# junyongeom/gru-mpi-cuda

Measured on AMD Instinct MI355X. Metric: char-tokens/sec (whole node) for GRU hidden=512 at 1/2/4/8 MI355X, higher is better.
Workload: dtype bf16; 1 GPU; model=GRU L=1 H=512 E=512 V=256, global_batch=256, seq_len=32, parallelism=dp1, impl=hip, optimizer=adam, overlap=False, plan=fwd=persistent bwd0=persistent+dWhh+dP head=fwd-tail serial dP=bwd-tail, dp_plan=replicated, dp_pipeline=0, collectives=0

## Files before the change

gru_mpi_cuda_amd/csrc/bindings.cpp:

```cpp
#include <pybind11/pybind11.h>
#include <pybind11/numpy.h>
#include <pybind11/stl.h>

#include "engine/trainer.h"
#include "engine/generator.h"
#include "comm/rccl_comm.h"
#include "comm/bootstrap.h"
#include "data/name_loader.h"

namespace py = pybind11;
using namespace gk;

static hipStream_t S(uintptr_t s) { return reinterpret_cast<hipStream_t>(s); }
template <class T> static T* Pp(uintptr_t p) { return reinterpret_cast<T*>(p); }

template <class T>
static T get(const py::dict& d, const char* k, T dflt) {
  if (!d.contains(k)) return dflt;
  return d[k].cast<T>();
}
#define GP(T, d, k) reinterpret_cast<T*>(get<uintptr_t>(d, k, 0))

static OptimArgs optim_from(const py::dict& d, const std::string& who) {
  OptimArgs a;
// ... 478 lines not shown
    a.s16 = GP(u16, d, "s16");
    a.Bp = get<int>(d, "Bp", 0); a.H = get<int>(d, "H", 0); a.algo = get<int>(d, "algo", 0);
    if (a.Bp % 32 || a.H % 64) throw std::runtime_error("fwd_step: Bp % 32 and H % 64 required");
    return a;
  };
  auto bwd_step_args = [](py::dict d) {
    BwdStepArgs a;
    a.dgh_next = GP(const u16, d, "dgh_next"); a.WhhT = GP(const u16, d, "WhhT");
    a.carry_in = GP(const float, d, "carry_in"); a.dy = GP(const float, d, "dy");
    a.r = GP(const float, d, "r"); a.z = GP(const float, d, "z"); a.n = GP(const float, d, "n");
    a.ghn = GP(const float, d, "ghn"); a.hprev = GP(const float, d, "hprev");
    a.carry_out = GP(float, d, "carry_out"); a.dgh = GP(u16, d, "dgh"); a.dghT = GP(u16, d, "dghT");
    a.dgiT = GP(u16, d, "dgiT"); a.dgi = GP(u16, d, "dgi");
    a.ldT = get<int>(d, "ldT", 0); a.colT = get<int>(d, "colT", 0);
    a.Bp = get<int>(d, "Bp", 0); a.H = get<int>(d, "H", 0); a.algo = get<int>(d, "algo", 0);
    a.sk_part = GP(float, d, "sk_part"); a.sk_part_floats = get<long>(d, "sk_part_floats", 0);
    a.sk_cnt = GP(unsigned, d, "sk_cnt"); a.sk_cnt_words = get<long>(d, "sk_cnt_words", 0);
    a.err = GP(unsigned, d, "err");
    a.dgiT_n_only = get<int>(d, "dgiT_n_only", 0);
    if (a.Bp % 32 || a.H % 64) throw std::runtime_error("bwd_step: Bp % 32 and H % 64 required");
    return a;
  };
  m.def("fwd_step", [fwd_step_args](py::dict d, uintptr_t s) {
    gru_fwd_step(fwd_step_args(d), S(s));
    HIP_LAUNCH_CHECK();
  });
  m.def("bwd_step", [bwd_step_args](py::dict d, uintptr_t s) {
    gru_bwd_step(bwd_step_args(d), S(s));
    HIP_LAUNCH_CHECK();
  });
  auto plan_dict = [](const StepPlan& p) {
    py::dict o;
    o["name"] = step_kernel_name(p.kernel);
    o["ks"] = p.ks; o["kb"] = p.kb; o["nks_i"] = p.nks_i; o["splits"] = p.splits; o["sk_map"] = p.sk_map;
    return o;
  };
  m.def("fwd_step_variant", [fwd_step_args, plan_dict](py::dict d) { return plan_dict(gru_fwd_step_plan(fwd_step_args(d))); });
  m.def("bwd_step_variant", [bwd_step_args, plan_dict](py::dict d) { return plan_dict(gru_bwd_step_plan(bwd_step_args(d))); });
  m.def("spin_delay", [](int us, uintptr_t s) { spin_delay(us, S(s)); HIP_LAUNCH_CHECK(); });
  m.def("copy_d2d", [](uintptr_t dst, uintptr_t src, size_t bytes) {
    HIP_CHECK(hipMemcpy(reinterpret_cast<void*>(dst), reinterpret_cast<const void*>(src), bytes, hipMemcpyDeviceToDevice));
  });
  m.def("graph_node_probe_detail", &graph_node_probe_detail);
  m.def("graph_node_probe", &graph_node_probe);
  m.def("block_cus", [](int nblocks, int us, uintptr_t s) { block_cus(nblocks, us, S(s)); });
  m.def("xcc_census", [](uintptr_t out, int nblocks, int threads, uintptr_t s) {
    xcc_census(Pp<unsigned>(out), nblocks, threads, S(s)); HIP_LAUNCH_CHECK(); });
  m.def("fwd_seq_supported", &gru_fwd_seq_supported);
  m.def("bwd_step_sk_splits", &gru_bwd_step_sk_splits);
  m.def("step_lds_variants", []() {
    const StepLdsVariants& v = step_lds_variants();
    py::dict d;
    d["fwd64"] = v.fwd64; d["bwd_sk_min_h"] = v.bwd_sk_min_h; d["dwfc_group"] = v.dwfc_group;
    d["bwd_big"] = v.bwd_big; d["bwd16"] = v.bwd16; d["bwd_xring"] = v.bwd_xring; d["fwd_xring"] = v.fwd_xring; d["fwd_fc"] = v.fwd_fc; d["fc_flash"] = v.fc_flash; d["fc_tail"] = v.fc_tail; d["bwd_tail"] = v.bwd_tail; d["save16"] = v.save16; d["big_dy"] = v.big_dy; d["ld_pad"] = v.ld_pad;
    return d;
  });
  m.def("set_step_lds_variants", [](py::dict d) {
    StepLdsVariants& v = step_lds_variants();
    for (auto kv : d) {
      const std::string k = py::str(kv.first);
      const int x = kv.second.cast<int>();
      if (k == "fwd64") v.fwd64 = x;
      else if (k == "bwd_sk_min_h") v.bwd_sk_min_h = x;
      else if (k == "dwfc_group") v.dwfc_group = x;
      else if (k == "bwd_big") v.bwd_big = x;
      else if (k == "bwd16") v.bwd16 = x;
      else if (k == "bwd_xring") v.bwd_xring = x;
      else if (k == "fwd_xring") v.fwd_xring = x;
      else if (k == "fwd_fc") v.fwd_fc = x;
      else if (k == "fc_flash") v.fc_flash = x;
      else if (k == "fc_tail") v.fc_tail = x;
      else if (k == "bwd_tail") v.bwd_tail = x;
      else if (k == "big_dy") v.big_dy = x;
      else if (k == "ld_pad") v.ld_pad = x;
      else if (k == "save16") v.save16 = x;
      else throw std::runtime_error("set_step_lds_variants: unknown field " + k);
    }
  });
  m.def("gemm_variants", []() {
    const GemmVariants& v = gemm_variants();
    py::dict d;
    d["mfma"] = v.mfma; d["phased"] = v.phased; d["sched"] = v.sched; d["groupm"] = v.groupm; d["onehot"] = v.onehot;
    d["small_ring"] = v.small_ring;
    return d;
  });
  m.def("set_gemm_variants", [](py::dict d) {
    GemmVariants& v = gemm_variants();
    for (auto kv : d) {
      const std::string k = py::str(kv.first);
      const int x = kv.second.cast<int>();
      if (k == "mfma") v.mfma = x;
      else if (k == "phased") v.phased = x;
      else if (k == "sched") v.sched = x;
      else if (k == "groupm") v.groupm = x;
      else if (k == "onehot") v.onehot = x;
      else if (k == "small_ring") {
        if (x != 0 && x != 3 && x != 4) throw std::runtime_error("set_gemm_variants: small_ring is 0, 3 or 4");
        v.small_ring = x;
      }
      else throw std::runtime_error("set_gemm_variants: unknown field " + k);
    }
  });
  m.def("bwd_seq_supported", &gru_bwd_seq_supported);
  m.def("fwd_seq2", [](py::dict lo, py::dict hi, uintptr_t Wih, uintptr_t bih, uintptr_t s) {
    auto parse = [](py::dict d) {
      SeqFwdArgs a;
      a.HSb = GP(u16, d, "HSb"); a.HSf = GP(float, d, "HSf"); a.HT = GP(u16, d, "HT"); a.ldT = get<int>(d, "ldT", 0);
      a.HF = GP(u16, d, "HF"); a.xch = GP(u16, d, "xch");
      a.sr = GP(float, d, "sr"); a.sz = GP(float, d, "sz"); a.sn = GP(float, d, "sn"); a.sghn = GP(float, d, "sghn");
      a.Whh = GP(const u16, d, "Whh"); a.bhh = GP(const float, d, "bhh");
      a.P = GP(const float, d, "P"); a.ids = GP(const int, d, "ids"); a.Gi = GP(const float, d, "Gi");
      a.h0 = GP(const float, d, "h0");
      a.cnt = GP(unsigned, d, "cnt"); a.err = GP(unsigned, d, "err");
      a.dbg = GP(unsigned long long, d, "dbg"); a.allow_local = get<int>(d, "allow_local", 1);
      a.xring = get<int>(d, "xring", 0);
      a.s16 = GP(u16, d, "s16");
      a.zero_next = GP(unsigned, d, "zero_next"); a.zero_words = get<long>(d, "zero_words", 0);
      a.T = get<int>(d, "T", 0); a.Bp = get<int>(d, "Bp", 0); a.H = get<int>(d, "H", 0);
      if (!a.xch || !a.cnt || !a.HSb || !a.HSf || !a.Whh || !a.bhh) throw std::runtime_error("fwd_seq2: HSb/HSf/xch/cnt/Whh/bhh required");
      return a;
    };
    SeqFwd2Args a;
    a.lo = parse(lo); a.hi = parse(hi);
    a.Wih = reinterpret_cast<const u16*>(Wih); a.bih = reinterpret_cast<const float*>(bih);
    if (!a.lo.ids == !a.lo.Gi) throw std::runtime_error("fwd_seq2: lo needs exactly one of P+ids / Gi");
// ... 464 lines not shown
```

gru_mpi_cuda_amd/csrc/engine/trainer.cpp:

```cpp
#include "trainer.h"
#include "../runtime/trace.h"
#include "../runtime/blaslt.h"

#include <cstring>
#include <algorithm>

namespace gk {

static int round_up(int x, int m) { return (x + m - 1) / m * m; }


Trainer::Trainer(const Dims& d, const OptCfg& o, float* params, float* grads, float* m, float* v, long nflat,
                 const std::map<std::string, long>& offsets)
    : d_(d), o_(o), params_(params), grads_(grads), m_(m), v_(v), nflat_(nflat), off_(offsets) {
  if (d_.V % 64 || d_.E % 64 || d_.H % 64)
    throw std::runtime_error("HIP engine needs vocab, embed and hidden to be multiples of 64");
  Bp_ = round_up(std::max(d_.B, 1), 64);
  blaslt_init(wgrad_prefers_library(3 * d_.H, d_.H, (long)d_.T * Bp_));
  C_ = std::max(1, d_.chunks);
  while (C_ > 1 && d_.T % C_) --C_;
  Tc_ = d_.T / C_;
  const int V = d_.V, E = d_.E, H = d_.H, T = d_.T, L = d_.L, B = Bp_;
  const size_t tok = (size_t)T * B;
  const int pad = step_lds_variants().ld_pad;
// ... 36 lines not shown
  persist_fwd_ = allow && gru_fwd_seq_supported(H, B);
  {
    const char* fw = std::getenv("GK_FWD_WAVE");
    fwd_wave_ = persist_fwd_ && L >= 2 && !(fw && fw[0] == '0') && gru_fwd_seq2_supported(H, B);
  }
  if (const char* sa = std::getenv("GK_STEP_ALGO")) step_algo_ = std::atoi(sa);
  if (const char* xl = std::getenv("GK_XCD_LOCAL")) xcd_local_ = std::atoi(xl) != 0;
  if (step_algo_ == 2 && !gru_step_lds_ok(H, B)) step_algo_ = 0;
  {
    const long tok = (long)d_.T * B, ctok = (long)Tc_ * B;
    dgiT_share_ = V % 128 == 0 && H % 128 == 0 && B % 8 == 0 && tok % 128 == 0 &&
                  ctok % 128 == 0;
  }
  seq_.resize(L);
  bool any_bwd = false;
  for (int l = 0; l < L; ++l) {
    SeqPlan& q = seq_[l];
    q.fuse_p = (l == 0) && V == 256 && allow && gru_bwd_seq_supported(H, B, H <= 512, true);
    q.fuse_w = allow && H <= 512 && gru_bwd_seq_supported(H, B, true, q.fuse_p);
    q.bwd = allow && gru_bwd_seq_supported(H, B, q.fuse_w, q.fuse_p);
    if (!q.bwd) q.fuse_w = q.fuse_p = false;
    q.big = allow && !q.bwd && step_lds_variants().bwd_big && gru_bwd_seq_big_supported(H, B) &&
            seq_flag_words(H, B) >= 8192;
    q.rows16 = q.bwd && !q.fuse_w && (B / 32) % 8 != 0 && (B / 16) % 8 == 0 && step_lds_variants().bwd16 &&
               gru_bwd_seq16_supported(H, B, q.fuse_p);
    q.nrb = q.rows16 ? B / 16 : B / 32;
    any_bwd |= q.bwd;
  }
  for (int l = 0; l < L; ++l) {
    SeqPlan& q = seq_[l];
    const bool fwd16 = persist_fwd_ || gru_step_picks_lds(step_algo_, H, B);
    q.s16 = step_lds_variants().save16 && d_.overlap == 0 && (q.big || q.bwd) && fwd16;
  }
  splits_ = 8;
  size_t o_cnt = R((size_t)2 * L * seq_flag_words(H, B) * 4 + 64), o_err = R(64), o_x = R((size_t)T * B * 3 * H * 2);
  constexpr int kSlots = 2 + 2 * kMaxGroup;
  size_t o_dst = R((size_t)kSlots * slot_ints() * 4);
  const size_t wmax = std::max({(size_t)V * H, (size_t)3 * H * H, (size_t)V * 3 * H, (size_t)3 * H * E});
  size_t o_sw = R((size_t)splits_ * wmax * 4);
  size_t o_rw = R((size_t)splits_ * std::max(V, 3 * H) * 4);
  size_t o_sfc2 = R((size_t)kFcSplitsMax * V * H * 4), o_rfc2 = R((size_t)kFcSplitsMax * V * 4);
  size_t o_se = R((size_t)splits_ * V * E * 4);
  std::vector<size_t> o_pw(L, 0), o_pbh(L, 0), o_pbi(L, 0), o_hf(L, 0), o_s16(L, 0);
  for (int l = 0; l < L; ++l) {
    if (seq_[l].s16) o_s16[l] = R(tok * H * 8);
    if (seq_[l].fuse_w) o_pw[l] = R((size_t)seq_[l].nrb * 3 * H * H * 4);
    if (seq_[l].fuse_w && persist_fwd_) o_hf[l] = R((tok + B) * H * 2);
    if (seq_[l].bwd || seq_[l].big) {
      o_pbh[l] = R((size_t)seq_[l].nrb * 3 * H * 4);
      o_pbi[l] = R((size_t)seq_[l].nrb * 3 * H * 4);
    }
  }
  size_t o_pP = seq_[0].fuse_p ? R((size_t)seq_[0].nrb * V * 3 * H * 4) : 0;
  int sk = 0;
  bool any_big = false;
  for (int l = 0; l < L; ++l) {
    if (!seq_[l].bwd && !seq_[l].big) sk = gru_bwd_step_sk_splits(H, B);
    any_big |= seq_[l].big;
  }
  size_t o_bp = any_big ? R((size_t)gru_bwd_seq_big_part_floats(H, B) * 4) : 0;
  sk_part_floats_ = sk ? (long)H * B * sk : 0;
  sk_cnt_words_ = sk ? (long)(H / 128) * (B / 64) * 16 : 0;
  size_t o_skp = sk ? R((size_t)sk_part_floats_ * 4) : 0, o_skc = sk ? R((size_t)sk_cnt_words_ * 4) : 0;
  (void)any_bwd;
  arena_.commit();
  d_stage_ = arena_.get<int>(o_dst);
  cnt_ = arena_.get<unsigned>(o_cnt); err_ = arena_.get<unsigned>(o_err); xbuf_ = arena_.get<u16>(o_x);
  slab_w_ = arena_.get<float>(o_sw); rs_w_ = arena_.get<float>(o_rw);
  slab_fc2_ = arena_.get<float>(o_sfc2); rs_fc2_ = arena_.get<float>(o_rfc2); slab_e_ = arena_.get<float>(o_se);
  for (int l = 0; l < L; ++l) {
    seq_[l].dWhh_part = seq_[l].fuse_w ? arena_.get<float>(o_pw[l]) : nullptr;
    seq_[l].HF = o_hf[l] ? arena_.get<u16>(o_hf[l]) : nullptr;
    seq_[l].dbhh_part = (seq_[l].bwd || seq_[l].big) ? arena_.get<float>(o_pbh[l]) : nullptr;
    seq_[l].dbih_part = (seq_[l].bwd || seq_[l].big) ? arena_.get<float>(o_pbi[l]) : nullptr;
  }
  dP_part_ = seq_[0].fuse_p ? arena_.get<float>(o_pP) : nullptr;
  bpart_ = any_big ? arena_.get<float>(o_bp) : nullptr;
  sk_part_ = sk ? arena_.get<float>(o_skp) : nullptr;
  sk_cnt_ = sk ? arena_.get<unsigned>(o_skc) : nullptr;

  ids_ = arena_.get<int>(o_ids); labels_ = arena_.get<int>(o_lab); inv_count_ = arena_.get<float>(o_inv);
  Ptab_ = arena_.get<float>(o_P); loss_part_ = arena_.get<float>(o_lp); loss_ = arena_.get<float>(o_loss);
  slab_fc_ = arena_.get<float>(o_sfc); rs_fc_ = arena_.get<float>(o_rfc); slab_P_ = arena_.get<float>(o_sP);
  dP_ = arena_.get<float>(o_dP); norm_parts_ = arena_.get<float>(o_np); gscale_ = arena_.get<float>(o_gs);
  step_ = arena_.get<int>(o_step);
  Emb = arena_.get<u16>(o_Emb); EmbT = arena_.get<u16>(o_EmbT); Wfc = arena_.get<u16>(o_Wfc); WfcT = arena_.get<u16>(o_WfcT);
  WfcF = arena_.get<u16>(o_WfcF); WfcTF = arena_.get<u16>(o_WfcTF);
  logits_ = fc_split_ ? arena_.get<float>(o_lg) : nullptr;
  dl_ = arena_.get<u16>(o_dl); dlT_ = arena_.get<u16>(o_dlT); dP_bf_ = arena_.get<u16>(o_dPb); dPT_bf_ = arena_.get<u16>(o_dPTb);
  Ls_.resize(L);
  for (int l = 0; l < L; ++l) {
    const LO& x = los[l];
    Layer& y = Ls_[l];
    y.HSf = arena_.get<float>(x.HSf); y.sr = arena_.get<float>(x.sr); y.sz = arena_.get<float>(x.sz);
    y.sn = arena_.get<float>(x.sn); y.sghn = arena_.get<float>(x.sghn); y.dy = arena_.get<float>(x.dy);
    y.Gi = l > 0 ? arena_.get<float>(x.Gi) : nullptr;
    y.carry[0] = arena_.get<float>(x.c0); y.carry[1] = arena_.get<float>(x.c1);
    y.HSb = arena_.get<u16>(x.HSb); y.HT = arena_.get<u16>(x.HT);
    y.dgh[0] = arena_.get<u16>(x.g0); y.dgh[1] = arena_.get<u16>(x.g1);
    y.dghT = arena_.get<u16>(x.dghT); y.dgiT = arena_.get<u16>(x.dgiT);
    y.dgi = l > 0 ? arena_.get<u16>(x.dgi) : nullptr;
    y.Whh = arena_.get<u16>(x.Whh); y.WhhT = arena_.get<u16>(x.WhhT);
    y.Wih = arena_.get<u16>(x.Wih); y.WihT = arena_.get<u16>(x.WihT);
    y.slab_hh = arena_.get<float>(x.shh); y.rs_hh = arena_.get<float>(x.rhh);
    y.slab_ih = l > 0 ? arena_.get<float>(x.sih) : nullptr; y.rs_ih = l > 0 ? arena_.get<float>(x.rih) : nullptr;
    y.s16 = o_s16[l] ? arena_.get<u16>(o_s16[l]) : nullptr;
  }

  HIP_CHECK(hipStreamCreateWithFlags(&s0_, hipStreamNonBlocking));
  HIP_CHECK(hipStreamCreateWithFlags(&s1_, hipStreamNonBlocking));
  {
    int lo = 0, hi = 0;
    HIP_CHECK(hipDeviceGetStreamPriorityRange(&lo, &hi));
    HIP_CHECK(hipStreamCreateWithPriority(&sc_, hipStreamNonBlocking, hi));
  }
  events_.resize(64 + 8 * C_ * L);
  for (auto& e : events_) HIP_CHECK(hipEventCreateWithFlags(&e, hipEventDisableTiming));
  HIP_CHECK(hipStreamCreateWithFlags(&sx_, hipStreamNonBlocking));
  HIP_CHECK(hipHostMalloc(&h_stage_, kSlots * (2 * tok + 16) * sizeof(int)));
  std::memset(h_stage_, 0, kSlots * (2 * tok + 16) * sizeof(int));
  const unsigned stage_flags = hipEventDisableTiming | (unsigned)hipEventDisableSystemFence;
  for (auto& e : stage_done_) {
    HIP_CHECK(hipEventCreateWithFlags(&e, stage_flags));
    HIP_CHECK(hipEventRecord(e, s0_));
  }
  for (auto& e : group_done_) {
    HIP_CHECK(hipEventCreateWithFlags(&e, stage_flags));
    HIP_CHECK(hipEventRecord(e, s0_));
  }
  for (auto* ev : {&copy_done_[0], &copy_done_[1], &group_copy_done_[0], &group_copy_done_[1]}) {
    HIP_CHECK(hipEventCreateWithFlags(ev, hipEventDisableTiming));
    HIP_CHECK(hipEventRecord(*ev, sx_));
  }
  HIP_CHECK(hipHostMalloc(reinterpret_cast<void**>(&err_host_), 64, hipHostMallocCoherent | hipHostMallocMapped));
  std::memset(err_host_, 0, 64);
  HIP_CHECK(hipHostGetDevicePointer(reinterpret_cast<void**>(&err_host_dev_), err_host_, 0));
  const char* ng = std::getenv("GK_NO_GRAPH");
  if (ng && ng[0] == '1') use_graph_ = false;
  overlap_ = d_.overlap != 0;
  dy_in_bwd_ = fc_split_ && !overlap_ && !seq_.empty() && seq_.back().big && seq_.back().s16 && d_.V == 256 &&
               step_lds_variants().big_dy;
  fc_in_fwd_ = persist_fwd_ && !fwd_wave_ && d_.L == 1 && !overlap_ && !fc_split_ && !seq_.empty() &&
               seq_[0].bwd && seq_[0].fuse_w && seq_[0].HF && step_lds_variants().fwd_fc &&
               Bp_ / 32 <= kFcSplitsMax && gru_fwd_seq_fc_supported(d_.H, Bp_, d_.V);
  fc_tail_ = persist_fwd_ && !fwd_wave_ && d_.L == 1 && !overlap_ && !fc_split_ && !fc_in_fwd_ && seq_[0].s16 &&
             d_.V % 128 == 0 && d_.H % (16 * (d_.V / 64)) == 0 && step_lds_variants().fc_tail &&
             step_lds_variants().fc_flash == 0 && gru_fwd_seq_tail_supported(d_.H, Bp_, d_.V);
  bwd_tail_ok_ = d_.L == 1 && !overlap_ && seq_[0].bwd && seq_[0].fuse_w && seq_[0].fuse_p && !seq_[0].rows16 &&
                 seq_[0].s16 && seq_[0].HF && step_lds_variants().bwd_tail && d_.V % seq_[0].nrb == 0 &&
                 (d_.V / seq_[0].nrb) % 8 == 0 && gru_bwd_seq_tail_supported(d_.H, Bp_, d_.V);
  bwd_tail_ = bwd_tail_ok_ && use_graph_ && o_.clip <= 0.f;
}

Trainer::~Trainer() {
  wd_.reset();
  if (pbf_) (void)hipFree(pbf_);
  if (bpack_) (void)hipFree(bpack_);
  for (auto& g : g_fb_) g.reset();
  for (auto& g : g_step_) g.reset();
  for (auto& g : g_group_) g.reset();
  g_opt_.reset();
  for (auto& e : events_) (void)hipEventDestroy(e);
  for (auto& g : g_group_) g.reset();
  for (auto& e : stage_done_) if (e) (void)hipEventDestroy(e);
  for (auto& e : group_done_) if (e) (void)hipEventDestroy(e);
  for (hipEvent_t e : {copy_done_[0], copy_done_[1], group_copy_done_[0], group_copy_done_[1]})
    if (e) (void)hipEventDestroy(e);
  if (h_stage_) (void)hipHostFree(h_stage_);
  if (err_host_) (void)hipHostFree(err_host_);
  if (s0_) (void)hipStreamDestroy(s0_);
  if (s1_) (void)hipStreamDestroy(s1_);
  if (sx_) (void)hipStreamDestroy(sx_);
  if (sc_) (void)hipStreamDestroy(sc_);
}

hipEvent_t Trainer::ev() {
  if (ev_next_ >= events_.size()) throw std::runtime_error("trainer: event pool exhausted");
  return events_[ev_next_++];
}


void Trainer::set_carry(bool on) {
  if (on == carry_) return;
  carry_ = on;
  for (auto& g : g_fb_) g.reset();
  for (auto& g : g_step_) g.reset();
  for (auto& g : g_group_) g.reset();
}

void Trainer::record_carry(hipStream_t s) {
  const int H = d_.H, T = d_.T, B = Bp_;
  const size_t n = (size_t)B * H, ldT = (size_t)(T + 1) * B;
  for (int l = 0; l < d_.L; ++l) {
    Layer& y = Ls_[l];
    HIP_CHECK(hipMemcpyAsync(y.HSf, y.HSf + (size_t)T * n, n * 4, hipMemcpyDeviceToDevice, s));
    HIP_CHECK(hipMemcpyAsync(y.HSb, y.HSb + (size_t)T * n, n * 2, hipMemcpyDeviceToDevice, s));
    HIP_CHECK(hipMemcpy2DAsync(y.HT, ldT * 2, y.HT + (size_t)T * B, ldT * 2, (size_t)B * 2, H,
                               hipMemcpyDeviceToDevice, s));
    if (seq_[l].HF)
      HIP_CHECK(hipMemcpyAsync(seq_[l].HF, seq_[l].HF + (size_t)T * n, n * 2, hipMemcpyDeviceToDevice, s));
  }
}

void Trainer::reset_hidden(hipStream_t s) {
// ... 393 lines not shown
        }
      }
      if (!used) rest.job[rest.n++] = D;
    }
    if (rest.n) reduce_slabs_multi(rest, s);
    adam_cast_multi(a, j, s);
  } else {
    if (part != 0) throw std::runtime_error("record_opt: split optimiser launches need V, E, H % 64 == 0");
    if (deferred_.n) reduce_slabs_multi(deferred_, s);
    adam_step(a, s);
    refresh_weights(s);
  }
  deferred_.n = 0;
  HIP_LAUNCH_CHECK();
}

void Trainer::forward_backward(hipStream_t s) {
  GK_TRACE("gk.forward_backward");
  const int slot = stage_slot_;
  stage_src_ = dev_slot(slot);
  HIP_CHECK(hipStreamWaitEvent(s, copy_done_[slot], 0));
  if (!use_graph_) {
    hipEvent_t a = events_.back();
    HIP_CHECK(hipEventRecord(a, s));
    HIP_CHECK(hipStreamWaitEvent(s0_, a, 0));
    if (overlap_) record_fb(s0_); else record_fb_seq(s0_);
    HIP_CHECK(hipEventRecord(a, s0_));
    HIP_CHECK(hipStreamWaitEvent(s, a, 0));
  } else {
    if (!g_fb_[slot].ready()) {
      g_fb_[slot].begin(s0_);
      if (overlap_) record_fb(s0_); else record_fb_seq(s0_);
      g_fb_[slot].end(s0_);
    }
    g_fb_[slot].launch(s);
  }
  HIP_CHECK(hipEventRecord(stage_done_[slot], s));
}

void Trainer::optimizer_step(hipStream_t s) {
  GK_TRACE("gk.optimizer_step");
  if (!use_graph_) { record_opt(s); return; }
  if (!g_opt_.ready()) {
    g_opt_.begin(s0_);
    record_opt(s0_);
    g_opt_.end(s0_);
  }
  g_opt_.launch(s);
}

void Trainer::set_comm(RcclComm* c, const std::vector<std::pair<long, long>>& buckets, long min_bucket_floats) {
  comm_ = c;
  if (!c) shard_opt_ = false;
  if (c) bwd_tail_ = false;
  buckets_ = buckets;
  min_bucket_ = std::max(1L, min_bucket_floats);
  const int L = d_.L;
  long prev = off_.at("fc.weight");
  bool ok = prev == 0 && off_.at("fc.bias") > prev;
  prev = off_.at("fc.bias");
  for (int l = L - 1; l >= 0; --l) {
    const std::string k = std::to_string(l);
    for (const char* n : {"weight_hh_l", "bias_hh_l", "bias_ih_l", "weight_ih_l"}) {
      const long o = off_.at(n + k);
      ok = ok && o > prev;
      prev = o;
    }
  }
  ok = ok && off_.at("embedding") > prev;
  if (!ok) throw std::runtime_error("set_comm: flat gradient layout is not in readiness order");
  dP_inplace_ = (long)d_.V * 3 * d_.H <= 3L * d_.H * d_.E;
  g_step_[0].reset();
  g_step_[1].reset();
  g_group_[0].reset();
  g_group_[1].reset();
}

void Trainer::set_dp_pipeline(int mode) {
  if (mode < -1 || mode > 1) throw std::runtime_error("set_dp_pipeline: -1 (auto), 0 or 1");
  dp_pipe_ = mode;
  g_step_[0].reset();
  g_step_[1].reset();
  g_group_[0].reset();
  g_group_[1].reset();
}

bool Trainer::dp_pipe_on() const {
  if (!comm_ || overlap_ || shard_opt_ || d_.L != 1 || o_.clip > 0.f) return false;
  const int V = d_.V, E = d_.E, H = d_.H;
  if (V % 64 || E % 64 || H % 64 || !dP_inplace_) return false;
  return dp_pipe_ == 1;
}

long Trainer::group_end(int l) const {
  if (l >= d_.L) return off_.at("weight_hh_l" + std::to_string(d_.L - 1));
  if (l > 0) return off_.at("weight_hh_l" + std::to_string(l - 1));
  return off_.at("weight_ih_l0") + (dP_inplace_ ? (long)d_.V * 3 * d_.H : 0L);
}

bool Trainer::ar_flush(hipStream_t s, bool force, bool with_err) {
  const long n = ar_ready_ - ar_launched_;
  if (n <= 0 || (!force && n < min_bucket_)) return false;
  auto reduce = [&](hipStream_t st) {
    if (with_err) comm_->allreduce_avg_f32_err(grads_ + ar_launched_, n, err_, st);
    else comm_->allreduce_avg_f32(grads_ + ar_launched_, n, st);
  };
  hipEvent_t e = ev();
// ... 188 lines not shown
```

gru_mpi_cuda_amd/csrc/engine/trainer.h:

```cpp
#pragma once
#include <map>
#include <cstdlib>
#include <string>
#include <vector>
#include "../runtime/runtime.h"
#include "../kernels/kernels.h"
#include "../comm/rccl_comm.h"
#include "../comm/watchdog.h"
#include <memory>

namespace gk {

struct Dims {
  int V = 256, E = 512, H = 512, L = 1, B = 256, T = 32, chunks = 4;
  int overlap = 1;
};
struct OptCfg {
  float lr = 1e-3f, b1 = 0.9f, b2 = 0.999f, eps = 1e-8f, wd = 0.f, clip = 0.f;
  int sgd = 0;
  int sched = 0, warmup = 0, total = 0;
  float lr_min = 0.f;
  int keep_grads = 1;
};

class Trainer {
 public:
  Trainer(const Dims& d, const OptCfg& o, float* params, float* grads, float* m, float* v, long nflat,
          const std::map<std::string, long>& offsets);
  ~Trainer();

  void refresh_weights(hipStream_t s);
  void set_batch(const int* x_bt, const int* y_bt, int B, hipStream_t s);
  void forward_backward(hipStream_t s);
  void optimizer_step(hipStream_t s);
  float read_loss();
  float read_grad_norm();
  int get_step();
  void set_step(int v);
  void set_lr(float lr);
  void set_use_graph(bool g) { use_graph_ = g; if (!g) bwd_tail_ = false; }
  void set_carry(bool on);
  bool carry() const { return carry_; }
  void reset_hidden(hipStream_t s);
  int padded_batch() const { return Bp_; }
  long workspace_bytes() const { return (long)arena_.bytes(); }
  uintptr_t buffer(const std::string& name) const;

 private:
  void record_fb(hipStream_t s0);
  bool defer_slabs_ = false;
  SlabJobs deferred_;
  void slab_job(SlabJobs& j, const float* src, int splits, long n, float* dst);
  void record_carry(hipStream_t s);
  bool carry_ = false;
  void record_opt(hipStream_t s0, int part = 0);
  void fwd_step(int l, int t, hipStream_t s);
  void bwd_step(int l, int t, hipStream_t s);
  hipEvent_t ev();
  float* P(const std::string& name) const { return params_ + off_.at(name); }
  float* G(const std::string& name) const { return grads_ + off_.at(name); }
  int in_dim(int l) const { return l == 0 ? d_.E : d_.H; }

  Dims d_;
  OptCfg o_;
  int Bp_ = 0, Tc_ = 0, C_ = 1;
  float* params_; float* grads_; float* m_; float* v_;
  long nflat_;
  std::map<std::string, long> off_;

  Arena arena_;
  hipStream_t s0_ = nullptr, s1_ = nullptr;
  std::vector<hipEvent_t> events_;
  size_t ev_next_ = 0;
  Graph g_fb_[2], g_opt_;
  bool use_graph_ = true;
  bool overlap_ = true;
  int* h_stage_ = nullptr;
  int* d_stage_ = nullptr;
  hipStream_t sx_ = nullptr;
  hipEvent_t stage_done_[2] = {nullptr, nullptr};
  hipEvent_t copy_done_[2] = {nullptr, nullptr};
  hipEvent_t group_copy_done_[2] = {nullptr, nullptr};
  int stage_slot_ = 0;
  const int* stage_src_ = nullptr;
  size_t slot_ints() const { return 16 + 2 * (size_t)Bp_ * d_.T; }
  const int* dev_slot(int slot) const { return d_stage_ + (size_t)slot * slot_ints(); }
  void fill_slot(int slot, const int* x, const int* y, int B);
  void copy_slots(int first, int n, hipEvent_t done);
  Graph g_step_[2];
  Graph g_group_[2];
  hipEvent_t group_done_[2] = {nullptr, nullptr};
  int group_ = 1, group_parity_ = 0;
  int group_slot(int parity, int j) const { return 2 + parity * kMaxGroup + j; }
// ... 29 lines not shown
  void set_comm(RcclComm* c, const std::vector<std::pair<long, long>>& buckets, long min_bucket_floats);
  const std::vector<std::pair<long, long>>& allreduce_log() const { return ar_log_; }
  void set_dp_pipeline(int mode);
  int dp_pipeline() const { return dp_pipe_on() ? 1 : 0; }
  bool dp_tail_recorded() const { return dp_tail_rec_; }
  void set_shard_optim(int mode);
  bool shard_optim() const { return shard_opt_; }
  int shard_mode() const { return shard_mode_; }
  void gather_params(hipStream_t s);
  long shard_chunk() const { return shard_chunk_; }
  void gather_opt_state(hipStream_t s);
  void step(hipStream_t s);
  static constexpr int kMaxGroup = 32;
  void set_graph_steps(int G);
  int graph_steps() const { return group_; }
  void set_batches(const int* x, const int* y, int B, int n);
  void step_group(hipStream_t s);
  void inject_error(unsigned bits) { HIP_CHECK(hipMemcpy(err_, &bits, 4, hipMemcpyHostToDevice)); }
  void enable_watchdog(int timeout_ms);
  int watchdog_status() const { return wd_ ? wd_->status() : 0; }
  std::string watchdog_message() { return wd_ ? wd_->message() : std::string(); }
 private:
  std::unique_ptr<Watchdog> wd_;

  struct Layer {
    float *HSf, *sr, *sz, *sn, *sghn, *dy, *Gi, *carry[2];
    u16* s16 = nullptr;
    u16 *HSb, *HT, *dgh[2], *dghT, *dgiT, *dgi;
    u16 *Whh, *WhhT, *Wih, *WihT;
    float *slab_hh, *rs_hh, *slab_ih, *rs_ih;
  };
  std::vector<Layer> Ls_;
  struct SeqPlan {
    bool bwd = false, fuse_w = false, fuse_p = false;
    bool big = false;
    bool rows16 = false;
    bool s16 = false;
    int nrb = 0;
    float *dWhh_part = nullptr, *dbhh_part = nullptr, *dbih_part = nullptr;
    u16* HF = nullptr;
  };
  void record_fb_seq(hipStream_t s0, bool dp = false);
  void record_emb_tail(hipStream_t s, const float* dP_fp32);
  static bool wgrad_prefers_library(int M, int N, long K) {
    const char* v = std::getenv("GK_WGRAD_GEMM");
    return v && std::string(v) == "lib" && (double)M * N >= 8e6 && 2.0 * M * N * (double)K >= 60e9;
  }
  void wgrad_gemm(const u16* A, int lda, const u16* Bm, int ldb, int M, int N, int K, float* slab,
                  float* rowsum, hipStream_t s);
  bool persist_fwd_ = false;
  bool fc_in_fwd_ = false;
  bool fc_tail_ = false;
  bool bwd_tail_ok_ = false, bwd_tail_ = false;
  bool in_step_ = false;
  bool dy_in_bwd_ = false;
  bool fwd_wave_ = false;
  float* bpart_ = nullptr;
  int step_algo_ = 0;
  std::vector<SeqPlan> seq_;
  int splits_ = 8;
  unsigned *cnt_ = nullptr, *err_ = nullptr;
  unsigned *err_host_ = nullptr, *err_host_dev_ = nullptr;
  float* sk_part_ = nullptr;
  unsigned* sk_cnt_ = nullptr;
  long sk_part_floats_ = 0, sk_cnt_words_ = 0;
  int xcd_local_ = 1;
  bool dgiT_share_ = false;
  u16* xbuf_ = nullptr;
  float *slab_w_ = nullptr, *rs_w_ = nullptr, *dP_part_ = nullptr;
  float *slab_fc2_ = nullptr, *rs_fc2_ = nullptr, *slab_e_ = nullptr;
  GemmArgs fc_held_;
  bool fc_held_on_ = false;
  int nloss_ = 0;
  long ldG_ = 0;
  static constexpr int kFcSplitsMax = 32;
 public:
  bool uses_persistent() const { return persist_fwd_ || (!seq_.empty() && seq_[0].bwd); }
  std::string plan() const;
  unsigned read_error();
 private:
  int *ids_, *labels_;
  float *inv_count_, *Ptab_, *loss_part_, *loss_, *slab_fc_, *rs_fc_, *slab_P_, *dP_;
  float *norm_parts_, *gscale_;
  int* step_;
  u16 *Emb, *EmbT, *Wfc, *WfcT, *dl_, *dlT_, *dP_bf_, *dPT_bf_;
  bool fc_split_ = false;
  float* logits_ = nullptr;
  u16 *WfcF, *WfcTF;
};

}
```

gru_mpi_cuda_amd/csrc/engine/trainer_seq.cpp:

```cpp
#include "trainer.h"
#include <algorithm>
#include <string>

namespace gk {

static bool ar_span() { return true; }

static int wgrad_engine() {
  const char* v = std::getenv("GK_WGRAD_GEMM");
  if (!v || !*v) return 0;
  if (std::string(v) == "lib") return 1;
  if (std::string(v) == "128") return 128;
  return 256;
}

static int gemm256_splits(int M, int N, int K) {
  int best = 0;
  double best_fill = 0.0;
  for (int sp = 1; sp <= 8; sp *= 2) {
    if (K % sp || (K / sp) % 64 || (sp > 1 && K / sp < 2048)) continue;
    const int bm = gemm256_tile_rows(M, N, K, sp);
    if (!bm) continue;
    const int wg = (M / bm) * (N / 256) * sp, rounds = (wg + 255) / 256;
    const double fill = (double)wg / (rounds * 256);
// ... 65 lines not shown

void Trainer::slab_job(SlabJobs& j, const float* src, int splits, long n, float* dst) {
  SlabJobs& t = (defer_slabs_ && splits <= kDeferMaxSplits) ? deferred_ : j;
  if (t.n >= 24) throw std::runtime_error("slab job list full");
  t.add(src, splits, n, dst);
}

void Trainer::record_fb_seq(hipStream_t s, bool dp) {
  const int V = d_.V, E = d_.E, H = d_.H, T = d_.T, L = d_.L, B = Bp_;
  const int H3 = 3 * H;
  const long tok = (long)T * B;
  const long fw = seq_flag_words(H, B);
  ev_next_ = 0;
  fc_held_on_ = false;
  if (dp) { ar_ready_ = ar_launched_ = 0; ar_busy_ = false; ar_log_.clear(); }
  dp_tail_rec_ = false;
  nloss_ = (int)(tok / 32);
  {
    GemmArgs g;
    g.A = Emb; g.lda = E; g.B = Ls_[0].Wih; g.ldb = E; g.C = Ptab_; g.ldc = H3;
    g.bias = P("bias_ih_l0"); g.M = V; g.N = H3; g.K = E;
    gemm_with_prep(g, PrepJob{stage_src_, Bp_, T, Bp_, ids_, labels_, inv_count_}, s);
  }
  if (carry_) record_carry(s);
  auto fwd_args = [&](int l) {
    Layer& y = Ls_[l];
    SeqFwdArgs a;
    a.HSb = y.HSb; a.HSf = y.HSf; a.HT = y.HT; a.ldT = (T + 1) * B; a.HF = seq_[l].HF;
    a.xch = xbuf_;
    if (y.s16) a.s16 = y.s16;
    else { a.sr = y.sr; a.sz = y.sz; a.sn = y.sn; a.sghn = y.sghn; }
    a.Whh = y.Whh; a.bhh = P("bias_hh_l" + std::to_string(l));
    if (l == 0) { a.P = Ptab_; a.ids = ids_; }
    else a.Gi = y.Gi;
    a.cnt = cnt_ + (size_t)l * fw; a.err = err_; a.allow_local = xcd_local_;
    a.xring = step_lds_variants().fwd_xring;
    if (seq_[l].bwd) { a.zero_next = cnt_ + (size_t)(L + l) * fw; a.zero_words = fw; }
    a.T = T; a.Bp = B; a.H = H;
    if (carry_) a.h0 = y.HSf;
    if (!seq_[l].bwd) fill_f32(reinterpret_cast<float*>(a.cnt), fw, 0.f, s);
    return a;
  };
  auto fc_args = [&]() {
    FcXentArgs f;
    f.X = Ls_[L - 1].HSb + (size_t)B * H; f.W = Wfc; f.b = P("fc.bias");
    f.labels = labels_; f.inv_count = inv_count_;
    f.dl = dl_; f.dlT = dlT_; f.ldT = (int)ldG_; f.colT = 0;
    f.loss_part = loss_part_; f.M = (int)tok; f.H = H; f.V = V;
    return f;
  };
  auto fc_fuse_dh = [&](FcXentArgs& f) {
    f.dl = nullptr; f.WT = WfcT; f.dy = Ls_[L - 1].dy; f.Wf = WfcF; f.WTf = WfcTF;
  };
  for (int l = 0; l < L; ++l) {
    Layer& y = Ls_[l];
    if (l > 0) {
      GemmArgs g;
      g.A = Ls_[l - 1].HSb + (size_t)B * H; g.lda = H; g.B = y.Wih; g.ldb = H;
      g.C = y.Gi; g.ldc = H3; g.bias = P("bias_ih_l" + std::to_string(l));
      g.M = (int)tok; g.N = H3; g.K = H;
      gemm_nt(g, s);
    }
    if (persist_fwd_ && fwd_wave_ && l + 1 < L) {
      SeqFwd2Args w2;
      w2.lo = fwd_args(l);
      w2.hi = fwd_args(l + 1);
      w2.hi.Gi = nullptr;
      w2.hi.xch = xbuf_ + (size_t)T * B * H;
      w2.lo.xring = w2.hi.xring = 0;
      w2.Wih = Ls_[l + 1].Wih; w2.bih = P("bias_ih_l" + std::to_string(l + 1));
      gru_fwd_seq2(w2, s);
      ++l;
    } else if (persist_fwd_ && fc_in_fwd_) {
      SeqFwdArgs a = fwd_args(l);
      a.HT = nullptr;
      SeqFcArgs f;
      f.Wf = WfcF; f.WTf = WfcTF; f.b = P("fc.bias"); f.labels = labels_; f.inv_count = inv_count_;
      f.dy = y.dy; f.dlF = dlT_; f.loss_part = loss_part_; f.dW = slab_fc2_; f.db = rs_fc2_; f.V = V;
      gru_fwd_seq_fc(a, f, s);
    } else if (persist_fwd_ && fc_tail_) {
      FcXentArgs f = fc_args();
      fc_fuse_dh(f);
      gru_fwd_seq_tail(fwd_args(l), f, s);
    } else if (persist_fwd_) {
      gru_fwd_seq(fwd_args(l), s);
    } else {
      for (int t = 0; t < T; ++t) fwd_step(l, t, s);
    }
  }
  Layer& top = Ls_[L - 1];
  SlabJobs tail;
  if (fc_in_fwd_) {
    tail.add(slab_fc2_, B / 32, (long)V * H, G("fc.weight"));
    tail.add(rs_fc2_, B / 32, V, G("fc.bias"));
  } else {
    FcXentArgs f = fc_args();
    if (fc_tail_) {
    } else if (fc_split_) {
      GemmArgs lg;
      lg.A = f.X; lg.lda = H; lg.B = Wfc; lg.ldb = H; lg.C = logits_; lg.ldc = V; lg.bias = f.b;
      lg.M = (int)tok; lg.N = V; lg.K = H;
      gemm_nt(lg, s);
      softmax_xent(logits_, f, s);
      if (!dy_in_bwd_) {
        GemmArgs g;
        g.A = dl_; g.lda = V; g.B = WfcT; g.ldb = V; g.C = top.dy; g.ldc = H;
        g.M = (int)tok; g.N = H; g.K = V;
        gemm_nt(g, s);
      }
    } else if (V % 128 == 0 && H % (16 * (V / 64)) == 0) {
      fc_fuse_dh(f);
      fc_xent(f, s);
    } else {
      fc_xent(f, s);
      GemmArgs g;
      g.A = dl_; g.lda = V; g.B = WfcT; g.ldb = V; g.C = top.dy; g.ldc = H;
      g.M = (int)tok; g.N = H; g.K = V;
      gemm_nt(g, s);
    }
    const int tiles = std::max(1, (V / 128) * (H / 128));
    int sp = 1;
    while (sp * 2 <= kFcSplitsMax && tiles * sp < 256 && tok % (sp * 2) == 0 && (tok / (sp * 2)) % 128 == 0)
      sp *= 2;
    if (sp * 2 <= kFcSplitsMax && tiles * sp < 512 && tok % (sp * 2) == 0 && tok / (sp * 2) >= 4096) sp *= 2;
    GemmArgs w;
    w.A = dlT_; w.lda = (int)ldG_; w.B = top.HT + B; w.ldb = (T + 1) * B;
    w.C = slab_fc2_; w.ldc = H; w.rowsumA = rs_fc2_;
    w.M = V; w.N = H; w.K = (int)tok; w.splits = sp;
    constexpr int kslice = 1024;
    if (kslice > 0 && tok % kslice == 0 && tok / kslice <= kFcSplitsMax && (V / 64) * (H / 64) * (tok / kslice) <= 256) {
      GemmArgs ws = w;
      ws.splits = (int)(tok / kslice); ws.algo = 3;
      if (gemm_small_kblocks(ws)) { w = ws; sp = ws.splits; }
    }
    fc_held_on_ = (dp && dp_pipe_on()) ||
                  (!dp && defer_slabs_ && sp <= 8 && w.algo == 3 && step_lds_variants().dwfc_group);
    if (fc_held_on_) fc_held_ = w;
    else gemm_nt(w, s);
    tail.add(slab_fc2_, sp, (long)V * H, G("fc.weight"));
    tail.add(rs_fc2_, sp, V, G("fc.bias"));
  }
  bool bwd_tail = bwd_tail_ok_ && !dp && defer_slabs_ && seq_[0].nrb <= kDeferMaxSplits;
  for (int k2 = 0; k2 < tail.n; ++k2) bwd_tail = bwd_tail && tail.job[k2].splits <= kDeferMaxSplits;
  if (in_step_) bwd_tail_ = bwd_tail;
  for (int l = L - 1; l >= 0; --l) {
    Layer& y = Ls_[l];
    const SeqPlan& q = seq_[l];
    const std::string k = std::to_string(l);
    if (q.bwd) {
      SeqBwdArgs a;
      a.dy = y.dy;
      if (q.s16) a.s16 = y.s16;
      else { a.sr = y.sr; a.sz = y.sz; a.sn = y.sn; a.sghn = y.sghn; }
      a.HSf = y.HSf; a.HT = y.HT; a.ldT = (T + 1) * B; a.HF = q.HF; a.WhhT = y.WhhT; a.xbuf = xbuf_;
      const bool need_T = !q.fuse_w || (l == 0 ? !q.fuse_p : true);
      a.dghT = need_T ? y.dghT : nullptr; a.dgiT = need_T ? y.dgiT : nullptr; a.ldG = (int)ldG_;
      a.dgi = y.dgi;
      a.dWhh_part = q.dWhh_part; a.dbhh_part = q.dbhh_part; a.dbih_part = q.dbih_part;
      if (q.fuse_p) { a.ids = ids_; a.dP_part = dP_part_; a.V = V; }
      a.cnt = cnt_ + (size_t)(L + l) * fw; a.err = err_; a.allow_local = xcd_local_;
      if (persist_fwd_) { a.zero_next = cnt_ + (size_t)l * fw; a.zero_words = fw; }
      a.T = T; a.Bp = B; a.H = H;
      if (!persist_fwd_) fill_f32(reinterpret_cast<float*>(a.cnt), fw, 0.f, s);
      a.xring = step_lds_variants().bwd_xring;
      if (bwd_tail && l == 0) {
        BwdTailArgs t;
        t.dP_bf = dP_bf_; t.dPT_bf = dPT_bf_; t.loss_part = loss_part_; t.nloss = nloss_; t.loss = loss_; t.step = step_;
        gru_bwd_seq_tail(a, t, s);
      } else if (q.rows16) gru_bwd_seq16(a, s);
      else gru_bwd_seq(a, s);
    } else if (q.big) {
      SeqBwdArgs a;
      a.dy = y.dy; a.HSf = y.HSf;
      if (q.s16) a.s16 = y.s16;
      else { a.sr = y.sr; a.sz = y.sz; a.sn = y.sn; a.sghn = y.sghn; }
      a.WhhT = y.WhhT; a.xbuf = xbuf_; a.part = bpart_;
      a.dghT = y.dghT; a.dgiT = y.dgiT; a.ldG = (int)ldG_; a.dgi = y.dgi;
      a.dgiT_n_only = l == 0 && dgiT_share_;
      a.dbhh_part = q.dbhh_part; a.dbih_part = l == 0 ? q.dbih_part : nullptr;
      if (dy_in_bwd_ && l == L - 1) { a.dl = dl_; a.WfcT = WfcT; a.V = V; a.dy = nullptr; }
      a.cnt = cnt_ + (size_t)(L + l) * fw; a.err = err_;
      a.T = T; a.Bp = B; a.H = H;
      a.xring = step_lds_variants().bwd_xring;
      fill_f32(reinterpret_cast<float*>(a.cnt), 8192, 0.f, s);
      gru_bwd_seq_big(a, s);
    } else {
      for (int t = T - 1; t >= 0; --t) bwd_step(l, t, s);
    }
    if (dp && q.bwd) ar_flush(s, false);
    SlabJobs j;
    if (q.fuse_w) slab_job(j, q.dWhh_part, q.nrb, (long)H3 * H, G("weight_hh_l" + k));
    if (q.bwd || q.big) slab_job(j, q.dbhh_part, q.nrb, H3, G("bias_hh_l" + k));
    if (l == 0 && q.fuse_p) {
      if (dp) j.add(dP_part_, q.nrb, (long)V * H3, dP_target());
      else if (!bwd_tail) j.add_cast(dP_part_, q.nrb, V, H3, nullptr, dP_bf_, dPT_bf_);
    }
    if (l == 0 && (q.bwd || q.big)) slab_job(j, q.dbih_part, q.nrb, H3, G("bias_ih_l0"));
    const bool pipe = dp && l == 0 && dp_pipe_on();
    if ((dp ? l == L - 1 : l == 0) && !pipe)
      for (int k2 = 0; k2 < tail.n; ++k2)
        slab_job(j, tail.job[k2].src, tail.job[k2].splits, tail.job[k2].n, tail.job[k2].dst);
    if (l == 0 && bwd_tail) {
      if (j.n) throw std::runtime_error("record_fb_seq: a slab job is left for the reduce launch the backward's tail replaced");
    } else if (l == 0) {
      j.add(loss_part_, nloss_, 1, loss_);
      j.bump = step_;
    }
    if (pipe) {
      if (!q.fuse_p || !q.fuse_w) throw std::runtime_error("pipelined data-parallel tail: needs the fused dW_hh / dP backward");
      record_dp_tail_l1(s, j, tail);
      HIP_LAUNCH_CHECK();
      return;
    }
    if (j.n) reduce_slabs_multi(j, s);
    if (!q.fuse_w)
      wgrad_gemm(y.dghT, (int)ldG_, y.HT, (T + 1) * B, H3, H, (int)tok, G("weight_hh_l" + k),
                 (q.bwd || q.big) ? nullptr : G("bias_hh_l" + k), s);
    if (l == 0) {
      if (!q.fuse_p) {
        GemmArgs p;
        int sp = splits_;
// ... 124 lines not shown
  e.A = dP_bf_; e.lda = H3; e.B = Ls_[0].WihT; e.ldb = H3; e.C = slab_e_; e.ldc = E;
  e.M = V; e.N = E; e.K = H3; e.splits = se;
  if (H3 % V == 0 && H3 / V <= splits_) {
    GemmArgs es = e;
    es.splits = H3 / V;
    const GemmArgs three[3] = {fc_held_, g, es};
    const bool with_fc = fc_held_on_ && gemm_small_group_depth(three, 3) == gemm_small_kblocks(g);
    const int nkb = gemm_small_kblocks(g);
    if (nkb && nkb == gemm_small_kblocks(es)) {
      const GemmArgs pair[2] = {g, es};
      if (fc_held_on_ && !with_fc) gemm_nt(fc_held_, s);
      if (with_fc) gemm_small_group(three, 3, s);
      else gemm_small_group(pair, 2, s);
      fc_held_on_ = false;
      SlabJobs r;
      slab_job(r, slab_e_, es.splits, (long)V * E, G("embedding"));
      if (r.n) reduce_slabs_multi(r, s);
      HIP_LAUNCH_CHECK();
      return;
    }
  }
  if (fc_held_on_) gemm_nt(fc_held_, s);
  fc_held_on_ = false;
  const GemmArgs both[2] = {g, e};
  const long wg = (long)(g.M / 128) * (g.N / 128) * g.splits + (long)(e.M / 128) * (e.N / 128) * e.splits;
  if (gemm_lds_ok(g) && gemm_lds_ok(e) && wg <= 512) {
    gemm_lds_group(both, 2, s);
  } else {
    gemm_nt(g, s);
    gemm_nt(e, s);
  }
  SlabJobs r;
  slab_job(r, slab_e_, se, (long)V * E, G("embedding"));
  if (r.n) reduce_slabs_multi(r, s);
  HIP_LAUNCH_CHECK();
}

std::string Trainer::plan() const {
  std::string p = std::string("fwd=") +
                  (persist_fwd_ ? (fwd_wave_ ? "persistent+wave" : fc_in_fwd_ ? "persistent+fc" : "persistent") : "per-step");
  for (size_t l = 0; l < seq_.size(); ++l) {
    p += " bwd" + std::to_string(l) + "=" +
         (seq_[l].bwd ? (seq_[l].rows16 ? "persistent16" : "persistent") : seq_[l].big ? "persistent-big" : "per-step");
    if (seq_[l].fuse_w) p += "+dWhh";
    if (seq_[l].fuse_p) p += "+dP";
    if (dy_in_bwd_ && l + 1 == seq_.size()) p += "+dy";
  }
  bool any_step = !persist_fwd_;
  for (const SeqPlan& q : seq_) any_step |= !q.bwd;
  if (any_step) p += std::string(" step=") + (gru_step_picks_lds(step_algo_, d_.H, Bp_) ? "lds" : "reg");
  if (fc_tail_) p += " head=fwd-tail";
  p += overlap_ ? " overlap(chunks=" + std::to_string(C_) + ")" : " serial";
  if (bwd_tail_) p += " dP=bwd-tail";
  return p;
}

unsigned Trainer::read_error() {
  unsigned e = 0;
  HIP_CHECK(hipDeviceSynchronize());
  HIP_CHECK(hipMemcpy(&e, err_, 4, hipMemcpyDeviceToHost));
  return e;
}

}
```

gru_mpi_cuda_amd/csrc/kernels/fc_block.h:

```cpp
#pragma once
#include "kernels.h"
#include "mma_tile.h"
#include "seq_sync.h"

namespace gk {

static constexpr int FROWS = 32;
static constexpr int kX2Pad = 8;

constexpr size_t fc_xent_v256_lds(int H) {
  return (size_t)FROWS * (H + kX2Pad) * 2 + (2 * 8 * 32 + 64) * 4 + 256 * 40 * 2 + (size_t)FROWS * (256 + 8) * 2 + FROWS * 4;
}

template <int NKC>
DEV void fc2_load_w(bf16x8 (&b)[NKC][2], const u16* Wf, int H, int v0, int ks, int lane) {
#pragma unroll
  for (int kk = 0; kk < NKC; ++kk)
#pragma unroll
    for (int c = 0; c < 2; ++c) b[kk][c] = ld8(Wf + ((size_t)((v0 / 16 + c) * (H / 32) + ks + kk) * 64 + lane) * 8);
}
template <int NKC>
DEV void fc2_mma(f32x4 (&acc)[2][2], const bf16x8 (&b)[NKC][2], const u16* xs, int ldx, int ks, int lane) {
  const int lr = lane & 15, lk = 8 * (lane >> 4);
#pragma unroll
  for (int kk = 0; kk < NKC; ++kk) {
    bf16x8 af[2];
#pragma unroll
    for (int r = 0; r < 2; ++r) af[r] = *reinterpret_cast<const bf16x8*>(xs + (r * 16 + lr) * ldx + (ks + kk) * 32 + lk);
#pragma unroll
    for (int r = 0; r < 2; ++r)
#pragma unroll
      for (int c = 0; c < 2; ++c) acc[r][c] = mfma16(af[r], b[kk][c], acc[r][c]);
  }
}
DEV void fc2_load_wt(bf16x8 (&bt)[8][4], const u16* WTf, int n0, int lane) {
#pragma unroll
  for (int kk = 0; kk < 8; ++kk)
#pragma unroll
    for (int c = 0; c < 4; ++c) bt[kk][c] = ld8(WTf + ((size_t)((n0 / 16 + c) * 8 + kk) * 64 + lane) * 8);
}

struct FcXPlain {
  static constexpr bool kWeightsFirst = false;
  DEV bool sc1() const { return false; }
  DEV void ready() const {}
  DEV int tid() const { return (int)threadIdx.x; }
};

template <int HH, bool DH, class XP>
DEV void fc_xent_v256_block(const FcXentArgs& a, float* smem, int block, const XP& xp) {
  int nst = 0;
  const int tid = xp.tid(), lane = tid & 63, w = tid >> 6;
  auto STAMP = [&]() {
    if (a.dbg && block == 0 && tid == 0) a.dbg[nst] = __builtin_amdgcn_s_memrealtime();
    ++nst;
  };
  STAMP();
  constexpr int V = 256, NW = 8, NKC = 8, LDR = V + 8;
  const int lr = lane & 15, lq = lane >> 4;
  constexpr int H = HH;
  const int ldx = H + kX2Pad, m0 = block * FROWS;
  u16* xs = reinterpret_cast<u16*>(smem);
  float* red = reinterpret_cast<float*>(xs + FROWS * ldx);
  float* lab = red + 2 * NW * 32;
  float* lrow = lab + 32;
  u16* st = reinterpret_cast<u16*>(lrow + 32);
  u16* dlr = st + V * 40;

  const int v0 = w * 32, nks = H / 32;
  const float inv = a.inv_count[0];
  float bias[2];
#pragma unroll
  for (int c = 0; c < 2; ++c) bias[c] = a.b[v0 + c * 16 + lr];
  bf16x8 b0[NKC][2], b1[NKC][2];
  constexpr int nxp = FROWS * H / 8 / 512;
  uint4 xv[nxp];
  auto load_x = [&]() {
    if (xp.sc1()) {
      const rsrc_t rX = make_rsrc(a.X, (unsigned)((size_t)a.M * H * 2));
#pragma unroll
      for (int e = 0; e < nxp; ++e) {
        const int q = tid + e * 512, row = q / (H / 8), c8 = q % (H / 8);
        const u32x4 v = __builtin_amdgcn_raw_buffer_load_b128(rX, (unsigned)(((size_t)(m0 + row) * H + c8 * 8) * 2), 0, 16);
        xv[e] = make_uint4(v.x, v.y, v.z, v.w);
      }
    } else {
#pragma unroll
      for (int e = 0; e < nxp; ++e) {
        const int q = tid + e * 512, row = q / (H / 8), c8 = q % (H / 8);
        xv[e] = *reinterpret_cast<const uint4*>(a.X + (size_t)(m0 + row) * H + c8 * 8);
      }
    }
  };
  int ylab;
  if constexpr (XP::kWeightsFirst) {
    ylab = tid < FROWS ? a.labels[m0 + tid] : 0;
    fc2_load_w<NKC>(b0, a.Wf, H, v0, 0, lane);
    if (nks > NKC) fc2_load_w<NKC>(b1, a.Wf, H, v0, NKC, lane);
    xp.ready();
// ... 81 lines not shown
        dlr[row * LDR + col] = db;
      }
    }
  lds_barrier();
  STAMP();
  if (tid < FROWS) {
    const int row = tid, y = ys[row];
    float m = red[row], sum = 0.f;
    for (int ww = 1; ww < NW; ++ww) m = fmaxf(m, red[ww * 32 + row]);
    for (int ww = 0; ww < NW; ++ww) sum += red[NW * 32 + ww * 32 + row];
    lrow[row] = (y >= 0) ? (logf(sum) + m - lab[row]) * inv : 0.f;
  }
  for (int q = tid; q < V * 4; q += 512) {
    const int col = q >> 2, seg = q & 3;
    uint4 v = *reinterpret_cast<const uint4*>(st + col * 40 + seg * 8);
    if ((col >> 3) & 1) v = make_uint4(v.y, v.x, v.w, v.z);
    *reinterpret_cast<uint4*>(a.dlT + (size_t)col * a.ldT + a.colT + m0 + seg * 8) = v;
  }
  STAMP();
  if constexpr (!DH) {
    for (int q = tid; q < FROWS * V / 8; q += 512) {
      const int r2 = q / (V / 8), c8 = q % (V / 8);
      *reinterpret_cast<uint4*>(a.dl + (size_t)(m0 + r2) * V + c8 * 8) =
          *reinterpret_cast<const uint4*>(dlr + r2 * LDR + c8 * 8);
    }
  }
  if constexpr (DH) for (int n0 = w * per; n0 < (w + 1) * per; n0 += 64) {
    if (n0 != w * per) fc2_load_wt(bt, a.WTf, n0, lane);
    f32x4 dacc[2][4];
    zero_acc(dacc);
#pragma unroll
    for (int kk = 0; kk < 8; ++kk) {
      bf16x8 af[2];
#pragma unroll
      for (int r = 0; r < 2; ++r) af[r] = *reinterpret_cast<const bf16x8*>(dlr + (r * 16 + lr) * LDR + kk * 32 + 8 * lq);
#pragma unroll
      for (int r = 0; r < 2; ++r)
#pragma unroll
        for (int c = 0; c < 4; ++c) dacc[r][c] = mfma16(af[r], bt[kk][c], dacc[r][c]);
    }
#pragma unroll
    for (int r = 0; r < 2; ++r)
#pragma unroll
      for (int c = 0; c < 4; ++c)
#pragma unroll
        for (int i = 0; i < 4; ++i)
          a.dy[(size_t)(m0 + r * 16 + lq * 4 + i) * H + n0 + c * 16 + lr] = dacc[r][c][i];
  }
  STAMP();
  __syncthreads();
  if (tid == 0) {
    float t = 0.f;
    for (int i = 0; i < FROWS; ++i) t += lrow[i];
    a.loss_part[block] = t;
  }
  STAMP();
}

}
```

gru_mpi_cuda_amd/csrc/kernels/gru_seq.hip:

```cpp
#include "kernels.h"
#include "mma_tile.h"
#include "seq_sync.h"
#include "fc_block.h"
#include "optim_dev.h"
#include <type_traits>

namespace gk {

static constexpr size_t kFwdRecLds = sizeof(float) * 8 * 6 * 256 + sizeof(u16) * 32 * 24 + sizeof(u16) * 16 * 40;
static constexpr size_t kFwdFcLds = sizeof(u16) * 32 * (512 + 8) + sizeof(u16) * 32 * (256 + 8) +
                                    sizeof(float) * (2 * 8 * 32 + 3 * 32);

template <int H>
DEV void fwd_fc_consumer(const SeqFwdArgs& a, const SeqFcArgs& f, unsigned char* smem, int ci) {
  constexpr int V = 256, NW = 8, LDX = H + 8, LDR = V + 8, NKS = H / 32, NKC = 4;
  static_assert((V / 64) * (H / 64) == kFcCons, "one 64 x 64 dW_fc tile per consumer");
  const int tid = threadIdx.x, lane = tid & 63, lr = lane & 15, lq = lane >> 4;
  const int w = __builtin_amdgcn_readfirstlane(tid >> 6);
  const int T = a.T, Bp = a.Bp, nrb = Bp / 32;
  constexpr int nunit = H / 16;
  const int rbk = ci % nrb, c = ci / nrb, b0 = rbk * 32;
  unsigned* const fl = a.cnt + (size_t)rbk * (nunit + kFcCons) * kFlagStride;
  unsigned* const cfl = fl + (size_t)nunit * kFlagStride;
  const int probe = f.probe & 7;
// ... 233 lines not shown
      for (;;) {
        bool ok = true;
        if (lane < n)
          ok = __hip_atomic_load(cfl + (size_t)((t0 + lane) % kFcCons) * kFlagStride, __ATOMIC_RELAXED,
                                 __HIP_MEMORY_SCOPE_AGENT) >= (unsigned)((t0 + lane) / kFcCons + 1);
        if (__all(ok)) break;
        __builtin_amdgcn_s_sleep(8);
        if (spin.expired()) {
          if (lane == 0) __hip_atomic_fetch_or(a.err, 1u, __ATOMIC_RELAXED, __HIP_MEMORY_SCOPE_AGENT);
          break;
        }
      }
      __builtin_amdgcn_fence(__ATOMIC_ACQUIRE, "wavefront");
    }
    bf16x8 A[DG], Bf[DG][2];
#pragma unroll
    for (int i = 0; i < DG; ++i) {
      if (i < n) {
        const int t = t0 + i;
        A[i] = ld8_sc1(rD, (unsigned)((((size_t)(t * nrb + rbk) * (V / 16) + tv) * 512 + lane * 8) * 2));
#pragma unroll
        for (int j = 0; j < 2; ++j)
          Bf[i][j] = ld8_sc1(rF, (unsigned)(((((size_t)(t + 1) * nunit + th + j) * nrb + rbk) * 512 + lane * 8) * 2));
      }
    }
#pragma unroll
    for (int i = 0; i < DG; ++i) {
      if (i < n) {
#pragma unroll
        for (int j = 0; j < 2; ++j) aw[j] = mfma16(A[i], Bf[i][j], aw[j]);
        if (rs_on) ab = mfma16(A[i], ones, ab);
      }
    }
  }
  float* W = f.dW + (size_t)rbk * V * H;
#pragma unroll
  for (int j = 0; j < 2; ++j)
#pragma unroll
    for (int i = 0; i < 4; ++i) W[(size_t)(tv * 16 + lq * 4 + i) * H + (th + j) * 16 + lr] = aw[j][i];
  if (rs_on && lr == 0) {
#pragma unroll
    for (int i = 0; i < 4; ++i) f.db[(size_t)rbk * V + tv * 16 + lq * 4 + i] = ab[i];
  }
}


struct FcXTail {
  static constexpr bool kWeightsFirst = true;
  const unsigned* fl;
  int nunit;
  unsigned epoch;
  unsigned* err;
  DEV bool sc1() const { return true; }
  DEV void ready() const { wait_flags_keep(fl, nunit, epoch, err); }
  DEV int tid() const {
    int t = (int)threadIdx.x;
    asm volatile("" : "+v"(t));
    return t;
  }
};

static_assert(std::is_trivially_copyable<SeqFwdArgs>::value && std::is_trivially_copyable<FcXentArgs>::value,
              "the tail reads both argument structs back from the kernel-argument segment byte for byte");
DEV void fwd_fc_tail(bool loc, unsigned char* smem) {
  typedef const __attribute__((address_space(4))) char* kptr_t;
  kptr_t kp = (kptr_t)__builtin_amdgcn_kernarg_segment_ptr();
  asm volatile("" : "+s"(kp));
  const SeqFwdArgs& a = *(const SeqFwdArgs*)kp;
  constexpr size_t fc_off = (sizeof(SeqFwdArgs) + alignof(FcXentArgs) - 1) / alignof(FcXentArgs) * alignof(FcXentArgs);
  const int T = a.T, nrb = a.Bp / 32, nunit = a.H / 16;
  const int ut = seq_unit_tile(nrb), rbk = seq_row_block(nrb);
  unsigned* const fl = a.cnt + (size_t)rbk * nunit * kFlagStride;
  const FcXTail xp{fl, nunit, (unsigned)(T + 1), a.err};
  const int tid = xp.tid();
  stamp(a.dbg, T + 1, 5);
  if (tid < 64) {
    asm volatile("s_waitcnt vmcnt(0)" ::: "memory");
    if (tid == 0) {
      if (loc) signal_flag_local(fl + (size_t)ut * kFlagStride, (unsigned)(T + 1));
      else signal_flag(fl + (size_t)ut * kFlagStride, (unsigned)(T + 1));
    }
  }
  for (int t = ut; t < T; t += nunit) {
    kptr_t kf = kp + fc_off;
    asm volatile("" : "+s"(kf));
    const FcXentArgs f = *(const FcXentArgs*)kf;
    fc_xent_v256_block<512, true>(f, reinterpret_cast<float*>(smem), t * nrb + rbk, xp);
  }
  stamp(a.dbg, T + 1, 6);
}

template <bool TAIL> struct FwdFcArg { typedef SeqFcArgs type; };
template <> struct FwdFcArg<true> { typedef FcXentArgs type; };
static constexpr size_t kFwdTailLds = fc_xent_v256_lds(512) > kFwdRecLds ? fc_xent_v256_lds(512) : kFwdRecLds;

template <int NKW, int RS, bool FC, int WPE = FC ? 4 : 1, bool TAIL = false>
__global__ void __launch_bounds__(512, WPE) gru_fwd_seq_kernel(SeqFwdArgs a, typename FwdFcArg<TAIL>::type fc) {
  static_assert(!(FC && TAIL), "the FC consumers and the FC tail exclude each other");
  static_assert(!TAIL || (NKW == 4 && RS == 2), "the tail is built for H = 512");
  static_assert(std::is_same<decltype(&gru_fwd_seq_kernel<NKW, RS, FC, WPE, TAIL>),
                             void (*)(SeqFwdArgs, typename FwdFcArg<TAIL>::type)>::value,
                "gru_fwd_seq_kernel takes (SeqFwdArgs, FC arguments) and nothing else");
  __shared__ __attribute__((aligned(16))) unsigned char smem[TAIL ? kFwdTailLds : FC ? (kFwdFcLds > kFwdRecLds ? kFwdFcLds : kFwdRecLds) : kFwdRecLds];
  auto& part = *reinterpret_cast<float(*)[8][6][256]>(smem);
  auto& stg = *reinterpret_cast<u16(*)[32][24]>(smem + sizeof(float) * 8 * 6 * 256);
  auto& stgT = *reinterpret_cast<u16(*)[16][40]>(smem + sizeof(float) * 8 * 6 * 256 + sizeof(u16) * 32 * 24);
  const int tid = threadIdx.x, lane = tid & 63, w = tid >> 6;
  const int H = a.H, Bp = a.Bp, T = a.T;
  const int nrb = Bp / 32;
  const unsigned nunit = (unsigned)(H / 16);
  if constexpr (FC) {
    const int nrec = (int)nunit * nrb;
    if ((int)blockIdx.x >= nrec) {
      zero_next_flags(a.zero_next, a.zero_words);
      if constexpr (NKW * 128 == 512 && RS == 2) fwd_fc_consumer<512>(a, fc, smem, (int)blockIdx.x - nrec);
      return;
    }
  }
  const size_t rb_lines = nunit + (FC ? kFcCons : 0);
  const int ut = FC ? seq_unit_tile_n(nrb, (int)nunit * nrb) : seq_unit_tile(nrb);
  const int j0 = ut * 16, rbk = FC ? seq_row_block_n(nrb, (int)nunit * nrb) : seq_row_block(nrb), b0 = rbk * 32;
  const int lr = lane & 15, lk = 8 * (lane >> 4);
  constexpr int NR = RS == 2 ? 1 : 2;
  const int rt = RS == 2 ? (w >> 2) : 0;
  const int k0 = (RS == 2 ? (w & 3) : w) * NKW * 32;

  bf16x8 bw[NKW][3];
#pragma unroll
  for (int kk = 0; kk < NKW; ++kk)
#pragma unroll
    for (int g = 0; g < 3; ++g) bw[kk][g] = ld8(a.Whh + (size_t)(g * H + j0 + lr) * H + k0 + kk * 32 + lk);

  const int rb = tid >> 8, reg = (tid >> 6) & 3, ln = tid & 63;
  const int row = rb * 16 + (ln >> 4) * 4 + reg, col = ln & 15;
  const int b = b0 + row, j = j0 + col;
  float bh[3];
#pragma unroll
  for (int g = 0; g < 3; ++g) bh[g] = a.bhh[g * H + j];
  float hp = a.h0 ? a.h0[(size_t)b * H + j] : 0.f;
  const rsrc_t rH = make_rsrc(a.HSb, (unsigned)((size_t)(T + 1) * Bp * H * 2));
  const rsrc_t rX = make_rsrc(a.xch, (unsigned)((size_t)T * Bp * H * 2));
  const int xr = a.xring >= 2 ? a.xring : T;
  const unsigned sv_bytes = (unsigned)((size_t)T * Bp * H * 4);
  const rsrc_t rHSf = make_rsrc(a.HSf, sv_bytes + (unsigned)(Bp * H * 4));
  const rsrc_t rSr = make_rsrc(a.sr, a.sr ? sv_bytes : 0u), rSz = make_rsrc(a.sz, a.sz ? sv_bytes : 0u);
  const rsrc_t rSn = make_rsrc(a.sn, a.sn ? sv_bytes : 0u), rSg = make_rsrc(a.sghn, a.sghn ? sv_bytes : 0u);
  const rsrc_t rS16 = make_rsrc(a.s16, a.s16 ? 2u * sv_bytes : 0u);
  const unsigned sv_lane = (unsigned)((b * H + j) * 4);
  stamp(a.dbg, T + 1, 0);
  zero_next_flags(a.zero_next, a.zero_words);
  int cens = (int)rb_lines;
  if constexpr (FC) {
    if ((fc.probe & 7) == 3) cens = (int)nunit;
    if (fc.probe & 8) __builtin_amdgcn_s_setprio(2);
  }
  const bool loc = a.allow_local && row_block_local(a.cnt + (size_t)rbk * rb_lines * kFlagStride, ut, cens, a.err);
  stamp(a.dbg, T + 1, 4);

  int idn = a.ids ? a.ids[b] : 0;
  auto load_gi = [&](int t, float (&gi)[3]) {
    if (t >= T) return;
    const float* src = a.ids ? a.P + (size_t)idn * 3 * H : a.Gi + ((size_t)t * Bp + b) * 3 * H;
#pragma unroll
    for (int g = 0; g < 3; ++g) gi[g] = src[g * H + j];
    if (a.ids && t + 1 < T) idn = a.ids[(size_t)(t + 1) * Bp + b];
  };
  float gin[3] = {0.f, 0.f, 0.f};
  load_gi(0, gin);
  for (int t = 0; t < T; ++t) {
    stamp(a.dbg, t, 0);
    const float gi[3] = {gin[0], gin[1], gin[2]};
    f32x4 acc[NR][3];
    zero_acc(acc);
    if (t > 0 || a.h0) {
      bf16x8 af[NKW][NR];
      if (t > 0) {
        const size_t slot = ((size_t)((t - 1) % xr) * nrb + rbk) * nunit;
        wave_wait_load<NKW>(a.cnt + (size_t)rbk * rb_lines * kFlagStride, lane < 2 * NKW, k0 / 16 + lane,
                            (unsigned)t, a.err, [&](int kk) {
          const int u = k0 + kk * 32 + lk;
          const unsigned tb = (unsigned)(((slot + u / 16) * 32 + lr) * 16 + (u & 15)) * 2;
#pragma unroll
          for (int r = 0; r < NR; ++r) af[kk][r] = ld8_sc1(rX, tb + (unsigned)((rt + r) * 16 * 16 * 2));
        });
      } else {
        const unsigned base = (unsigned)((((size_t)b0 + rt * 16 + lr) * H + k0 + lk) * 2);
#pragma unroll
        for (int kk = 0; kk < NKW; ++kk)
#pragma unroll
          for (int r = 0; r < NR; ++r) af[kk][r] = ld8_sc1(rH, base + (unsigned)(r * 16 * H * 2 + kk * 64));
      }
      stamp(a.dbg, t, 1);
#pragma unroll
      for (int kk = 0; kk < NKW; ++kk)
#pragma unroll
        for (int r = 0; r < NR; ++r)
#pragma unroll
          for (int g = 0; g < 3; ++g) acc[r][g] = mfma16(af[kk][r], bw[kk][g], acc[r][g]);
    }
#pragma unroll
    for (int r = 0; r < NR; ++r)
#pragma unroll
      for (int g = 0; g < 3; ++g)
#pragma unroll
        for (int i = 0; i < 4; ++i) part[w][r * 3 + g][i * 64 + lane] = acc[r][g][i];
    if constexpr (FC) {
      if (w == 2) asm volatile("s_waitcnt vmcnt(0)" ::: "memory");
    }
    __syncthreads();
    stamp(a.dbg, t, 2);
    float gh[3];
#pragma unroll
    for (int g = 0; g < 3; ++g) {
      float s = 0.f;
      if constexpr (RS == 2) {
#pragma unroll
        for (int ww = 0; ww < 4; ++ww) s += part[rb * 4 + ww][g][reg * 64 + ln];
      } else {
#pragma unroll
        for (int ww = 0; ww < 8; ++ww) s += part[ww][rb * 3 + g][reg * 64 + ln];
      }
      gh[g] = s + bh[g];
    }
    const float r = sigmoidf_(gi[0] + gh[0]);
    const float z = sigmoidf_(gi[1] + gh[1]);
    const float n = tanhf_(gi[2] + r * gh[2]);
    const float h = n + z * (hp - n);
    hp = h;
    const u16 hb = f2bf(h);
    stg[row][col] = hb;
    stgT[col][row] = hb;
    __syncthreads();
    stamp(a.dbg, t, 3);
    if (w == 0) {
      const u32x4 v = *reinterpret_cast<const u32x4*>(&stg[lane >> 1][(lane & 1) * 8]);
      const unsigned xo = (unsigned)((((size_t)(t % xr) * nrb + rbk) * nunit + ut) * 512 + lane * 8) * 2;
      unsigned* fl = a.cnt + ((size_t)rbk * rb_lines + ut) * kFlagStride;
      if (loc) {
        st16_plain(rX, xo, v);
        asm volatile("s_waitcnt vmcnt(0)" ::: "memory");
        if (lane == 0) signal_flag_local(fl, (unsigned)(t + 1));
      } else {
        st16_sc1(rX, xo, v);
        asm volatile("s_waitcnt vmcnt(0)" ::: "memory");
        if (lane == 0) signal_flag(fl, (unsigned)(t + 1));
      }
      stamp(a.dbg, t, 4);
      const size_t hs = ((size_t)(t + 1) * Bp + b0 + (lane >> 1)) * H + j0 + (lane & 1) * 8;
      if (FC && !loc) st16_sc1(rH, (unsigned)(hs * 2), v);
      else if (TAIL && !loc) {
        unsigned* hp = reinterpret_cast<unsigned*>(a.HSb + hs);
#pragma unroll
        for (int i = 0; i < 4; ++i) __hip_atomic_store(hp + i, v[i], __ATOMIC_RELAXED, __HIP_MEMORY_SCOPE_AGENT);
      } else *reinterpret_cast<u32x4*>(a.HSb + hs) = v;
      stamp(a.dbg, t, 5);
    } else if (w == 1 && a.HT) {
      const u32x4 v = *reinterpret_cast<const u32x4*>(&stgT[lane >> 2][(lane & 3) * 8]);
      *reinterpret_cast<u32x4*>(a.HT + (size_t)(j0 + (lane >> 2)) * a.ldT + (size_t)(t + 1) * Bp + b0 + (lane & 3) * 8) = v;
    } else if (w == 2 && a.HF) {
      const u32x4 v = *reinterpret_cast<const u32x4*>(&stgT[lane & 15][8 * (lane >> 4)]);
      const size_t hf = (((size_t)(t + 1) * nunit + ut) * nrb + rbk) * 512 + lane * 8;
      if (FC && !loc) st16_sc1(make_rsrc(a.HF, (unsigned)((size_t)(T + 1) * Bp * H * 2)), (unsigned)(hf * 2), v);
      else *reinterpret_cast<u32x4*>(a.HF + hf) = v;
    }
    load_gi(t + 1, gin);
    const int sstep = __builtin_amdgcn_readfirstlane(t * Bp * H * 4);
    __builtin_amdgcn_raw_buffer_store_b32(__float_as_uint(h), rHSf, sv_lane, sstep + Bp * H * 4, 0);
    if (TAIL || a.s16) {
      typedef unsigned u32x2_ __attribute__((ext_vector_type(2)));
      const u32x2_ pv = {(unsigned)f2bf(r) | ((unsigned)f2bf(z) << 16), (unsigned)f2bf(n) | ((unsigned)f2bf(gh[2]) << 16)};
      __builtin_amdgcn_raw_buffer_store_b64(pv, rS16, sv_lane * 2u, sstep * 2, 0);
    } else if (a.sr) {
      __builtin_amdgcn_raw_buffer_store_b32(__float_as_uint(r), rSr, sv_lane, sstep, 0);
      __builtin_amdgcn_raw_buffer_store_b32(__float_as_uint(z), rSz, sv_lane, sstep, 0);
      __builtin_amdgcn_raw_buffer_store_b32(__float_as_uint(n), rSn, sv_lane, sstep, 0);
      __builtin_amdgcn_raw_buffer_store_b32(__float_as_uint(gh[2]), rSg, sv_lane, sstep, 0);
    }
    stamp(a.dbg, t, 6);
  }
  if constexpr (FC) {
    asm volatile("s_waitcnt vmcnt(0)" ::: "memory");
    __syncthreads();
    if (tid == 0) {
      unsigned* fl = a.cnt + ((size_t)rbk * rb_lines + ut) * kFlagStride;
      if (loc) signal_flag_local(fl, (unsigned)(T + 1));
      else signal_flag(fl, (unsigned)(T + 1));
    }
  }
  if constexpr (TAIL) fwd_fc_tail(loc, smem);
}

template <int NKW>
__global__ void __launch_bounds__(512, 1) gru_fwd_seq2_kernel(SeqFwd2Args a) {
  constexpr int NKS = NKW < 4 ? 4 : NKW;
  __shared__ __attribute__((aligned(16))) bf16x8 stage[8][2][NKS][2][64];
  __shared__ __attribute__((aligned(16))) u16 stg[2][32][24];
  __shared__ __attribute__((aligned(16))) u16 stgT[2][16][40];
  typedef __attribute__((address_space(3))) void lds_void;
  const SeqFwdArgs& L0 = a.lo;
  const SeqFwdArgs& L1 = a.hi;
  const int tid = threadIdx.x, lane = tid & 63, w = __builtin_amdgcn_readfirstlane(tid >> 6);
  const int H = L0.H, Bp = L0.Bp, T = L0.T;
  const int nrb = Bp / 32, ut = seq_unit_tile(nrb);
  const int j0 = ut * 16, rbk = seq_row_block(nrb), b0 = rbk * 32;
  const int lr = lane & 15, lk = 8 * (lane >> 4);
  const int k0 = w * NKW * 32;
  const unsigned nunit = (unsigned)(H / 16);

  bf16x8 wh0[NKW][3], wi1[NKW][3], wh1[NKW][3];
#pragma unroll
  for (int kk = 0; kk < NKW; ++kk)
#pragma unroll
    for (int g = 0; g < 3; ++g) {
      const size_t o = (size_t)(g * H + j0 + lr) * H + k0 + kk * 32 + lk;
      wh0[kk][g] = ld8(L0.Whh + o);
      wi1[kk][g] = ld8(a.Wih + o);
      wh1[kk][g] = ld8(L1.Whh + o);
    }

  const int q = w >> 2, e = w & 3;
  const int row = q * 16 + 4 * (lane >> 4) + e, col = lane & 15;
  const int b = b0 + row, j = j0 + col, pidx = e * 64 + lane;
  float bh0[3], bh1[3], bi1[3];
#pragma unroll
  for (int g = 0; g < 3; ++g) {
    bh0[g] = L0.bhh[g * H + j];
    bh1[g] = L1.bhh[g * H + j];
    bi1[g] = a.bih[g * H + j];
  }
  float hp0 = L0.h0 ? L0.h0[(size_t)b * H + j] : 0.f;
  float hp1 = L1.h0 ? L1.h0[(size_t)b * H + j] : 0.f;
  const unsigned hs_bytes = (unsigned)((size_t)(T + 1) * Bp * H * 2), x_bytes = (unsigned)((size_t)T * Bp * H * 2);
  const rsrc_t rH0 = make_rsrc(L0.HSb, hs_bytes), rX0 = make_rsrc(L0.xch, x_bytes);
  const rsrc_t rH1 = make_rsrc(L1.HSb, hs_bytes), rX1 = make_rsrc(L1.xch, x_bytes);
  const int xr = L0.xring >= 2 ? L0.xring : T;
  zero_next_flags(L0.zero_next, L0.zero_words);
  zero_next_flags(L1.zero_next, L1.zero_words);
  unsigned* const fl0 = L0.cnt + (size_t)rbk * nunit * kFlagStride;
  unsigned* const fl1 = L1.cnt + (size_t)rbk * nunit * kFlagStride;
  const bool loc = L0.allow_local && row_block_local(fl0, ut, (int)nunit, L0.err);

  const unsigned xl = (unsigned)((((lk >> 4) * 32 + lr) * 16 + (lk & 15)) * 2);
// ... 139 lines not shown
      const int ly = w, t = s - ly;
      if (ly == 0 ? do0 : do1) {
        const SeqFwdArgs& Y = ly == 0 ? L0 : L1;
        const u32x4 v = *reinterpret_cast<const u32x4*>(&stg[ly][lane >> 1][(lane & 1) * 8]);
        const unsigned xo = (unsigned)((((size_t)(t % xr) * nrb + rbk) * nunit + ut) * 512 + lane * 8) * 2;
        unsigned* fl = (ly == 0 ? fl0 : fl1) + (size_t)ut * kFlagStride;
        const rsrc_t rX = ly == 0 ? rX0 : rX1;
        if (loc) {
          st16_plain(rX, xo, v);
          asm volatile("s_waitcnt vmcnt(0)" ::: "memory");
          if (lane == 0) signal_flag_local(fl, (unsigned)(t + 1));
        } else {
          st16_sc1(rX, xo, v);
          asm volatile("s_waitcnt vmcnt(0)" ::: "memory");
          if (lane == 0) signal_flag(fl, (unsigned)(t + 1));
        }
        if (ly == 0) stamp(L0.dbg, s, 4);
        *reinterpret_cast<u32x4*>(Y.HSb + ((size_t)(t + 1) * Bp + b0 + (lane >> 1)) * H + j0 + (lane & 1) * 8) = v;
      }
    } else if (w < 6) {
      const int ly = (w - 2) >> 1, t = s - ly;
      const SeqFwdArgs& Y = ly == 0 ? L0 : L1;
      if (ly == 0 ? do0 : do1) {
        if (((w - 2) & 1) == 0) {
          if (Y.HT) {
            const u32x4 v = *reinterpret_cast<const u32x4*>(&stgT[ly][lane >> 2][(lane & 3) * 8]);
            *reinterpret_cast<u32x4*>(Y.HT + (size_t)(j0 + (lane >> 2)) * Y.ldT + (size_t)(t + 1) * Bp + b0 + (lane & 3) * 8) = v;
          }
        } else if (Y.HF) {
          const u32x4 v = *reinterpret_cast<const u32x4*>(&stgT[ly][lane & 15][8 * (lane >> 4)]);
          *reinterpret_cast<u32x4*>(Y.HF + (((size_t)(t + 1) * nunit + ut) * nrb + rbk) * 512 + lane * 8) = v;
        }
      }
    }
    load_gi0(s + 1, gin);
    if (do0) {
      L0.HSf[((size_t)(s + 1) * Bp + b) * H + j] = h0v;
      const size_t so = ((size_t)s * Bp + b) * H + j;
      if (L0.s16) st_save16(L0.s16 + so * 4, r0, z0, n0, ghn0);
      else if (L0.sr) { L0.sr[so] = r0; L0.sz[so] = z0; L0.sn[so] = n0; L0.sghn[so] = ghn0; }
    }
    if (do1) {
      L1.HSf[((size_t)s * Bp + b) * H + j] = h1v;
      const size_t so = ((size_t)(s - 1) * Bp + b) * H + j;
      if (L1.s16) st_save16(L1.s16 + so * 4, r1, z1, n1, ghn1);
      else if (L1.sr) { L1.sr[so] = r1; L1.sz[so] = z1; L1.sn[so] = n1; L1.sghn[so] = ghn1; }
    }
  }
}

struct SeqBwdTailK : SeqBwdArgs { BwdTailArgs t; };
template <bool TAIL> struct BwdKArg { typedef SeqBwdArgs type; };
template <> struct BwdKArg<true> { typedef SeqBwdTailK type; };

static_assert(std::is_trivially_copyable<SeqBwdTailK>::value, "the tail reads its arguments back from the kernel-argument segment");
template <int NTW, int NTP>
DEV void bwd_dp_tail(const f32x4 (&accW)[3][NTW], const f32x4 (&accP)[3][NTP], const float (&dbh)[3], float dbi,
                     float (*red)[16][33], unsigned char* stage ) {
  typedef const __attribute__((address_space(4))) char* kptr_t;
  kptr_t kp = (kptr_t)__builtin_amdgcn_kernarg_segment_ptr();
  asm volatile("" : "+s"(kp));
  const SeqBwdTailK& k = *(const SeqBwdTailK*)kp;
  const SeqBwdArgs& a = k;
  int tid = (int)threadIdx.x;
  asm volatile("" : "+v"(tid));
  const int lane = tid & 63, w = tid >> 6, lr = lane & 15, lq = lane >> 4;
  const int H = a.H, H3 = 3 * H, V = a.V, T = a.T, nrb = a.Bp / 32;
  const int nunit = H / 16, ut = seq_unit_tile(nrb), rbk = seq_row_block(nrb), j0 = ut * 16;
  const unsigned slab_bytes = (unsigned)((size_t)V * H3 * 4);
  const rsrc_t rP = make_rsrc(a.dP_part, (unsigned)nrb * slab_bytes);
  stamp(a.dbg, T + 1, 0);
#pragma unroll
  for (int g = 0; g < 3; ++g)
#pragma unroll
    for (int nt = 0; nt < NTP; ++nt) {
      const unsigned o = (unsigned)rbk * slab_bytes +
                         (unsigned)((((w * NTP + nt) * 16 + lr) * H3 + g * H + j0 + lq * 4) * 4);
      st16_sc1(rP, o, __builtin_bit_cast(u32x4, accP[g][nt]));
    }
  {
    const int rb = tid >> 8, reg = (tid >> 6) & 3, ln = tid & 63;
    const int row = rb * 16 + (ln >> 4) * 4 + reg, col = ln & 15;
    red[0][col][row] = dbh[0]; red[1][col][row] = dbh[1]; red[2][col][row] = dbh[2];
    red[3][col][row] = dbh[0]; red[4][col][row] = dbh[1]; red[5][col][row] = dbi;
  }
  asm volatile("s_waitcnt vmcnt(0)" ::: "memory");
  lds_barrier();
  if (tid == 0) signal_flag(a.cnt + ((size_t)rbk * nunit + ut) * kFlagStride, (unsigned)(T + 1));
  stamp(a.dbg, T + 1, 1);
  if (tid < 96) {
    const int kk = tid >> 4, c = tid & 15;
    float sum = 0.f;
    for (int rr = 0; rr < 32; ++rr) sum += red[kk][c][rr];
    float* dst = (kk < 3 ? a.dbhh_part : a.dbih_part);
    if (dst) dst[(size_t)rbk * H3 + (kk % 3) * H + j0 + c] = sum;
  }
  {
    float* W = a.dWhh_part + (size_t)rbk * H3 * H;
#pragma unroll
    for (int g = 0; g < 3; ++g)
#pragma unroll
      for (int nt = 0; nt < NTW; ++nt)
#pragma unroll
        for (int i = 0; i < 4; ++i)
          W[(size_t)(g * H + j0 + lq * 4 + i) * H + (w * NTW + nt) * 16 + lr] = accW[g][nt][i];
  }
  if (tid < 64) {
    SpinBudget spin(a.err);
    for (;;) {
      bool ok = true;
      if (lane < nrb)
        ok = __hip_atomic_load(a.cnt + ((size_t)lane * nunit + ut) * kFlagStride, __ATOMIC_RELAXED,
                               __HIP_MEMORY_SCOPE_AGENT) >= (unsigned)(T + 1);
      if (__all(ok)) break;
      __builtin_amdgcn_s_sleep(GK_POLL_SLEEP);
      if (spin.expired()) {
        if (lane == 0) __hip_atomic_fetch_or(a.err, 1u, __ATOMIC_RELAXED, __HIP_MEMORY_SCOPE_AGENT);
        break;
      }
    }
  }
  lds_barrier();
  stamp(a.dbg, T + 1, 2);
  constexpr int LDS_P = 56;
  u16* const tile = reinterpret_cast<u16*>(stage);
  const int rows = V / nrb, v0 = rbk * rows;
  const int irow = tid / 6, ipc = tid % 6;
  const int icol = (ipc >> 1) * H + j0 + (ipc & 1) * 8;
  const int tcol = tid >> 2, tseg = tid & 3;
  for (int r0 = 0; r0 < rows; r0 += 32) {
    if (tid < 192 && r0 + irow < rows) {
      const size_t e = (size_t)(v0 + r0 + irow) * H3 + icol;
      f32x4 x[8][2];
#pragma unroll
      for (int s = 0; s < 8; ++s)
        if (s < nrb) {
          const unsigned o = (unsigned)s * slab_bytes + (unsigned)(e * 4);
          x[s][0] = __builtin_bit_cast(f32x4, __builtin_amdgcn_raw_buffer_load_b128(rP, o, 0, 16));
          x[s][1] = __builtin_bit_cast(f32x4, __builtin_amdgcn_raw_buffer_load_b128(rP, o + 16u, 0, 16));
        }
      f32x4 s0 = x[0][0], s1 = x[0][1];
#pragma unroll
      for (int s = 1; s < 8; ++s)
        if (s < nrb) {
#pragma unroll
          for (int i = 0; i < 4; ++i) { s0[i] += x[s][0][i]; s1[i] += x[s][1][i]; }
        }
      u32x4 pv;
      pv[0] = (unsigned)f2bf(s0[0]) | ((unsigned)f2bf(s0[1]) << 16);
      pv[1] = (unsigned)f2bf(s0[2]) | ((unsigned)f2bf(s0[3]) << 16);
      pv[2] = (unsigned)f2bf(s1[0]) | ((unsigned)f2bf(s1[1]) << 16);
      pv[3] = (unsigned)f2bf(s1[2]) | ((unsigned)f2bf(s1[3]) << 16);
      *reinterpret_cast<u32x4*>(k.t.dP_bf + e) = pv;
      *reinterpret_cast<u32x4*>(tile + irow * LDS_P + ipc * 8) = pv;
    }
    lds_barrier();
    if (tid < 192 && r0 + tseg * 8 < rows) {
      u16 v[8];
#pragma unroll
      for (int q = 0; q < 8; ++q) v[q] = tile[(tseg * 8 + q) * LDS_P + tcol];
      const int gcol = (tcol >> 4) * H + j0 + (tcol & 15);
      *reinterpret_cast<u32x4*>(k.t.dPT_bf + (size_t)gcol * V + v0 + r0 + tseg * 8) = *reinterpret_cast<const u32x4*>(v);
    }
    if (r0 + 32 < rows) lds_barrier();
  }
  if (blockIdx.x == 0 && tid < 64) {
    const float l = wave_strided_sum(k.t.loss_part, k.t.nloss, 1, 0, lane);
    if (tid == 0) {
      k.t.loss[0] = l;
      *k.t.step += 1;
    }
  }
  stamp(a.dbg, T + 1, 3);
}

template <int NKW3, int NTW, int NTP, bool TAIL = false>
__global__ void __launch_bounds__(512, 1) gru_bwd_seq_kernel(typename BwdKArg<TAIL>::type a) {
  static_assert(!TAIL || (NKW3 == 6 && NTW == 4 && NTP == 2), "the tail is built for H = 512, V = 256");
  static_assert(std::is_same<decltype(&gru_bwd_seq_kernel<NKW3, NTW, NTP, TAIL>), void (*)(typename BwdKArg<TAIL>::type)>::value,
                "gru_bwd_seq_kernel takes one argument struct and nothing else");
  __shared__ __attribute__((aligned(16))) float part[8][2][256];
  __shared__ __attribute__((aligned(16))) u16 srow[3][32][24];
  __shared__ __attribute__((aligned(16))) u16 sgT[4][16][40];
  __shared__ __attribute__((aligned(16))) float red[6][16][33];
  constexpr bool kScalarX = NKW3 >= 12;
  const int tid = threadIdx.x, lane = tid & 63, w = kScalarX ? __builtin_amdgcn_readfirstlane(tid >> 6) : tid >> 6;
  const int H = a.H, H3 = 3 * a.H, Bp = a.Bp, T = a.T;
  const int nrb = Bp / 32, ut = seq_unit_tile(nrb);
  const int j0 = ut * 16, rbk = seq_row_block(nrb), b0 = rbk * 32;
  const int lr = lane & 15, lk = 8 * (lane >> 4);
  const int k0 = w * NKW3 * 32;
  const unsigned nunit = (unsigned)(H / 16);

  constexpr bool kBwLds = NTW > 0 || NTP > 0 || NKW3 >= 12;
  __shared__ __attribute__((aligned(16))) bf16x8 bwL[kBwLds ? NKW3 : 1][kBwLds ? 512 : 1];
  bf16x8 bw[kBwLds ? 1 : NKW3];
#pragma unroll
  for (int kk = 0; kk < NKW3; ++kk) {
    const bf16x8 v = ld8(a.WhhT + (size_t)(j0 + lr) * H3 + k0 + kk * 32 + lk);
    if constexpr (kBwLds) bwL[kk][tid] = v; else bw[kk] = v;
  }

  const int rb = tid >> 8, reg = (tid >> 6) & 3, ln = tid & 63;
  const int row = rb * 16 + (ln >> 4) * 4 + reg, col = ln & 15;
  const int b = b0 + row, j = j0 + col;
  float carry = 0.f;
  float dbh[3] = {0.f, 0.f, 0.f}, dbi = 0.f;
  f32x4 accW[3][NTW > 0 ? NTW : 1];
  f32x4 accP[3][NTP > 0 ? NTP : 1];
  zero_acc(accW);
  zero_acc(accP);
  const int xr = a.xring >= 2 ? a.xring : T;
  const rsrc_t rX = make_rsrc(a.xbuf, (unsigned)((size_t)T * Bp * H3 * 2));
  const unsigned xlane = (unsigned)(((lk >> 4) * 3 * 512 + lr * 16 + (lk & 15)) * 2);
  zero_next_flags(a.zero_next, a.zero_words);
  const bool loc = a.allow_local && row_block_local(a.cnt + (size_t)rbk * nunit * kFlagStride, ut, (int)nunit, a.err);
  float sv[6];
  int svid = 0;
  __shared__ __attribute__((aligned(16))) int idsL[NTP > 0 ? 32 : 1];
  auto load_saves = [&](int t) {
    const size_t o = ((size_t)t * Bp + b) * H + j;
    sv[0] = a.dy[o];
    if (TAIL || a.s16) ld_save16_raw(a.s16 + o * 4, sv[1], sv[2]);
    else { sv[1] = a.sr[o]; sv[2] = a.sz[o]; sv[3] = a.sn[o]; sv[4] = a.sghn[o]; }
    sv[5] = a.HSf[o];
    if constexpr (NTP > 0) svid = a.ids[(size_t)t * Bp + b];
  };
  load_saves(T - 1);

  for (int t = T - 1; t >= 0; --t) {
    const int s = T - 1 - t;
    stamp(a.dbg, s, 0);
    f32x4 acc[2];
    acc[0] = f32x4{0.f, 0.f, 0.f, 0.f};
    acc[1] = acc[0];
    if (s > 0) {
      bf16x8 af[NKW3][2];
      const size_t slot = ((size_t)((t + 1) % xr) * nrb + rbk) * nunit;
      wave_wait_load<NKW3>(a.cnt + (size_t)rbk * nunit * kFlagStride, lane < 2 * NKW3,
                           ((k0 + 16 * lane) % H) / 16, (unsigned)s, a.err, [&](int kk) {
        if constexpr (kScalarX) {
          const int c0 = k0 + kk * 32;
          const int so = (int)((((slot + (size_t)((c0 % H) / 16)) * 3 + (size_t)(c0 / H)) * 512) * 2);
#pragma unroll
          for (int r = 0; r < 2; ++r) af[kk][r] = ld8_sc1s(rX, xlane + (unsigned)(r * 16 * 16 * 2), so);
        } else {
          const int c = k0 + kk * 32 + lk, u = c % H;
          const unsigned tb = (unsigned)(((slot + u / 16) * 3 + c / H) * 512 + lr * 16 + (u & 15)) * 2;
#pragma unroll
          for (int r = 0; r < 2; ++r) af[kk][r] = ld8_sc1(rX, tb + (unsigned)(r * 16 * 16 * 2));
        }
      });
      stamp(a.dbg, s, 1);
#pragma unroll
      for (int kk = 0; kk < NKW3; ++kk) {
        bf16x8 bk;
        if constexpr (kBwLds) bk = bwL[kk][tid]; else bk = bw[kk];
#pragma unroll
        for (int r = 0; r < 2; ++r) acc[r] = mfma16(af[kk][r], bk, acc[r]);
      }
    }
    const int idc = svid;
    float sr = sv[1], sz = sv[2], sn = sv[3], sghn = sv[4];
    const float dy = sv[0], hprev = sv[5];
    if (t > 0) load_saves(t - 1);
    if (TAIL || a.s16) unpack_save16(sr, sz, sr, sz, sn, sghn);
    bf16x8 hB[NTW > 0 ? NTW : 1];
    if constexpr (NTW > 0) {
      if (TAIL || a.HF) {
#pragma unroll
        for (int nt = 0; nt < NTW; ++nt)
          hB[nt] = ld8(a.HF + (((size_t)t * nunit + w * NTW + nt) * nrb + rbk) * 512 + lane * 8);
      } else {
#pragma unroll
        for (int nt = 0; nt < NTW; ++nt)
          hB[nt] = ld8(a.HT + (size_t)(w * NTW * 16 + nt * 16 + lr) * a.ldT + (size_t)t * Bp + b0 + lk);
      }
    }
#pragma unroll
    for (int r = 0; r < 2; ++r)
#pragma unroll
      for (int i = 0; i < 4; ++i) part[w][r][i * 64 + lane] = acc[r][i];
    __syncthreads();
    stamp(a.dbg, s, 2);
    float dh = dy + carry;
#pragma unroll
    for (int ww = 0; ww < 8; ++ww) dh += part[ww][rb][reg * 64 + ln];
    const float dn = dh * (1.f - sz);
    const float dz = dh * (hprev - sn);
    const float dan = dn * (1.f - sn * sn);
    const float dar = dan * sghn * sr * (1.f - sr);
    const float daz = dz * sz * (1.f - sz);
    const float dhn = dan * sr;
    carry = sz * dh;
    dbh[0] += dar; dbh[1] += daz; dbh[2] += dhn; dbi += dan;
    const u16 br = f2bf(dar), bz = f2bf(daz), bn = f2bf(dhn), bi = f2bf(dan);
    srow[0][row][col] = br; srow[1][row][col] = bz; srow[2][row][col] = bn;
    sgT[0][col][row] = br; sgT[1][col][row] = bz; sgT[2][col][row] = bn; sgT[3][col][row] = bi;
    if constexpr (NTP > 0) {
      if (col == 0) idsL[row] = idc;
    }
    __syncthreads();
    stamp(a.dbg, s, 3);
    auto fused_mma = [&]() {
      if constexpr (NTW > 0 || NTP > 0) {
        bf16x8 ga[3];
#pragma unroll
        for (int g = 0; g < 3; ++g) ga[g] = *reinterpret_cast<const bf16x8*>(&sgT[g][lr][lk]);
        if constexpr (NTW > 0) {
#pragma unroll
          for (int g = 0; g < 3; ++g)
#pragma unroll
            for (int nt = 0; nt < NTW; ++nt) accW[g][nt] = mfma16(ga[g], hB[nt], accW[g][nt]);
        }
        if constexpr (NTP > 0) {
          ga[2] = *reinterpret_cast<const bf16x8*>(&sgT[3][lr][lk]);
          int idv[8];
          const int4 i0 = *reinterpret_cast<const int4*>(&idsL[lk]), i1 = *reinterpret_cast<const int4*>(&idsL[lk + 4]);
          idv[0] = i0.x; idv[1] = i0.y; idv[2] = i0.z; idv[3] = i0.w;
          idv[4] = i1.x; idv[5] = i1.y; idv[6] = i1.z; idv[7] = i1.w;
#pragma unroll
          for (int nt = 0; nt < NTP; ++nt) {
            const int v = (w * NTP + nt) * 16 + lr;
            bf16x8 oh;
#pragma unroll
            for (int e = 0; e < 8; ++e) oh[e] = (__bf16)(idv[e] == v ? 1.0f : 0.0f);
#pragma unroll
            for (int g = 0; g < 3; ++g) accP[g][nt] = mfma16(ga[g], oh, accP[g][nt]);
          }
        }
      }
    };
    if (w == 0) {
      const size_t tile = (((size_t)(t % xr) * nrb + rbk) * nunit + ut) * (3 * 32 * 16);
#pragma unroll
      for (int g = 0; g < 3; ++g) {
        const u32x4 v = *reinterpret_cast<const u32x4*>(&srow[g][lane >> 1][(lane & 1) * 8]);
        if (loc) st16_plain(rX, (unsigned)((tile + g * 512 + lane * 8) * 2), v);
        else st16_sc1(rX, (unsigned)((tile + g * 512 + lane * 8) * 2), v);
      }
      asm volatile("s_waitcnt vmcnt(0)" ::: "memory");
      unsigned* fl = a.cnt + ((size_t)rbk * nunit + ut) * kFlagStride;
      if (lane == 0) {
        if (loc) signal_flag_local(fl, (unsigned)(s + 1));
        else signal_flag(fl, (unsigned)(s + 1));
      }
      stamp(a.dbg, s, 4);
    } else if (!TAIL && w <= 4 && a.dghT) {
      const int g = w - 1;
      const u32x4 v = *reinterpret_cast<const u32x4*>(&sgT[g][lane >> 2][(lane & 3) * 8]);
      const size_t c0 = (size_t)t * Bp + b0 + (lane & 3) * 8;
      const int gg = g < 3 ? g : 2;
      const size_t rowsel = (size_t)(gg * H + j0 + (lane >> 2)) * a.ldG + c0;
      if (g < 3) *reinterpret_cast<u32x4*>(a.dghT + rowsel) = v;
      if (g != 2) *reinterpret_cast<u32x4*>(a.dgiT + rowsel) = v;
    }
    if (!TAIL && a.dgi) {
      const size_t og = ((size_t)t * Bp + b) * H3 + j;
      a.dgi[og] = br; a.dgi[og + H] = bz; a.dgi[og + 2 * H] = bi;
    }
    stamp(a.dbg, s, 5);
    fused_mma();
    stamp(a.dbg, s, 6);
  }

  if constexpr (TAIL) {
    bwd_dp_tail<NTW, NTP>(accW, accP, dbh, dbi, red, reinterpret_cast<unsigned char*>(&part[0][0][0]));
    return;
  }
  if constexpr (NTW > 0) {
    float* W = a.dWhh_part + (size_t)rbk * H3 * H;
#pragma unroll
    for (int g = 0; g < 3; ++g)
#pragma unroll
      for (int nt = 0; nt < NTW; ++nt)
#pragma unroll
        for (int i = 0; i < 4; ++i)
          W[(size_t)(g * H + j0 + (lane >> 4) * 4 + i) * H + (w * NTW + nt) * 16 + lr] = accW[g][nt][i];
  }
  if constexpr (NTP > 0) {
    float* Pp = a.dP_part + (size_t)rbk * a.V * H3;
#pragma unroll
    for (int g = 0; g < 3; ++g)
#pragma unroll
      for (int nt = 0; nt < NTP; ++nt)
#pragma unroll
        for (int i = 0; i < 4; ++i)
          Pp[(size_t)((w * NTP + nt) * 16 + lr) * H3 + g * H + j0 + (lane >> 4) * 4 + i] = accP[g][nt][i];
  }
  red[0][col][row] = dbh[0]; red[1][col][row] = dbh[1]; red[2][col][row] = dbh[2];
  red[3][col][row] = dbh[0]; red[4][col][row] = dbh[1]; red[5][col][row] = dbi;
  __syncthreads();
  if (tid < 96) {
    const int k = tid >> 4, c = tid & 15;
    float sum = 0.f;
    for (int rr = 0; rr < 32; ++rr) sum += red[k][c][rr];
    float* dst = (k < 3 ? a.dbhh_part : a.dbih_part);
    if (dst) dst[(size_t)rbk * H3 + (k % 3) * H + j0 + c] = sum;
  }
}

template <class K>
static int resident_blocks(K kernel, int block = 512) {
  int dev = 0, ncu = 0, per = 0;
  if (hipGetDevice(&dev) != hipSuccess) return 0;
  if (hipDeviceGetAttribute(&ncu, hipDeviceAttributeMultiprocessorCount, dev) != hipSuccess) return 0;
  if (hipOccupancyMaxActiveBlocksPerMultiprocessor(&per, kernel, block, 0) != hipSuccess) return 0;
  return ncu * per;
}

static int fwd_rs(int H) { return H <= 512 ? 2 : 1; }

#define FWD_VARIANTS(X) X(256, 1, 1) X(256, 2, 2) X(512, 2, 1) X(512, 4, 2) X(1024, 4, 1) X(1024, 8, 2)

bool gru_fwd_seq_supported(int H, int Bp) {
  if (Bp % 32) return false;
  const int rs = fwd_rs(H);
  int cap = -1;
#define X(HH, NK, RS) if (H == HH && rs == RS) cap = resident_blocks(gru_fwd_seq_kernel<NK, RS, false>);
  FWD_VARIANTS(X)
#undef X
  return cap >= (H / 16) * (Bp / 32);
}

void gru_fwd_seq(const SeqFwdArgs& a, hipStream_t s) {
  if ((size_t)(a.T + 1) * a.Bp * a.H * (a.s16 ? 8 : 4) >= (1ull << 31))
    throw std::runtime_error("gru_fwd_seq: saves exceed the 2 GB buffer-offset range");
  dim3 grid((a.H / 16) * (a.Bp / 32)), block(512);
  const int rs = fwd_rs(a.H);
#define X(HH, NK, RS)                                                          \
  if (a.H == HH && rs == RS) {                                                \
    hipLaunchKernelGGL((gru_fwd_seq_kernel<NK, RS, false>), grid, block, 0, s, a, SeqFcArgs{});   \
    return;                                                                    \
  }
  FWD_VARIANTS(X)
#undef X
  throw std::runtime_error("gru_fwd_seq: no kernel variant for this shape");
}

bool gru_fwd_seq_fc_supported(int H, int Bp, int V) {
  if (H != 512 || V != 256 || Bp % 32 || fwd_rs(H) != 2) return false;
  if (H / 16 + kFcCons > 64) return false;
  const int cap = resident_blocks(gru_fwd_seq_kernel<4, 2, true>);
  return cap >= (H / 16 + kFcCons) * (Bp / 32);
}

void gru_fwd_seq_fc(const SeqFwdArgs& a, const SeqFcArgs& f, hipStream_t s) {
  if (a.H != 512 || f.V != 256 || !a.HF || !f.Wf || !f.WTf || !f.dlF || !f.dy || !f.dW || !f.db || !f.loss_part ||
      !f.labels || !f.inv_count || !f.b)
    throw std::runtime_error("gru_fwd_seq_fc: needs H = 512, V = 256, the HF copy and every FC buffer");
  if ((size_t)(a.T + 1) * a.Bp * a.H * (a.s16 ? 8 : 4) >= (1ull << 31))
    throw std::runtime_error("gru_fwd_seq_fc: saves exceed the 2 GB buffer-offset range");
  const int nrb = a.Bp / 32;
  dim3 grid((a.H / 16) * nrb + kFcCons * nrb), block(512);
  if (f.probe & 16)
    hipLaunchKernelGGL((gru_fwd_seq_kernel<4, 2, true, 1>), grid, block, 0, s, a, f);
  else
    hipLaunchKernelGGL((gru_fwd_seq_kernel<4, 2, true>), grid, block, 0, s, a, f);
}

bool gru_fwd_seq_tail_supported(int H, int Bp, int V) {
  if (H != 512 || V != 256 || Bp % 32 || fwd_rs(H) != 2) return false;
  const int cap = resident_blocks(gru_fwd_seq_kernel<4, 2, false, 1, true>);
  return cap >= (H / 16) * (Bp / 32);
}

void gru_fwd_seq_tail(const SeqFwdArgs& a, const FcXentArgs& f, hipStream_t s) {
  if (a.H != 512 || f.H != 512 || f.V != 256 || f.M != a.T * a.Bp || f.X != a.HSb + (size_t)a.Bp * a.H || !f.Wf || !f.WTf ||
      !f.dy || f.dl || !f.dlT || !f.loss_part || !f.labels || !f.inv_count || !f.b || !a.s16)
    throw std::runtime_error("gru_fwd_seq_tail: needs H = 512, V = 256, the packed saves (s16), X = HSb + Bp * H and the "
                             "fused-dH FC arguments");
  if ((size_t)(a.T + 1) * a.Bp * a.H * (a.s16 ? 8 : 4) >= (1ull << 31))
    throw std::runtime_error("gru_fwd_seq_tail: saves exceed the 2 GB buffer-offset range");
  dim3 grid((a.H / 16) * (a.Bp / 32)), block(512);
  hipLaunchKernelGGL((gru_fwd_seq_kernel<4, 2, false, 1, true>), grid, block, 0, s, a, f);
}

#define FWD2_VARIANTS(X) X(256, 1) X(512, 2) X(1024, 4)

bool gru_fwd_seq2_supported(int H, int Bp) {
  if (Bp % 32) return false;
  int cap = -1;
#define X(HH, NK) if (H == HH) cap = resident_blocks(gru_fwd_seq2_kernel<NK>);
  FWD2_VARIANTS(X)
#undef X
  return cap >= (H / 16) * (Bp / 32);
}

void gru_fwd_seq2(const SeqFwd2Args& a, hipStream_t s) {
  const SeqFwdArgs& l0 = a.lo;
  const SeqFwdArgs& l1 = a.hi;
  if (l1.H != l0.H || l1.Bp != l0.Bp || l1.T != l0.T || !a.Wih || !a.bih || !l1.HSf || !l1.HSb || !l1.xch ||
      !l1.cnt || l1.xch == l0.xch || l1.cnt == l0.cnt)
    throw std::runtime_error("gru_fwd_seq2: inconsistent layer arguments");
  dim3 grid((l0.H / 16) * (l0.Bp / 32)), block(512);
#define X(HH, NK)                                                           \
  if (l0.H == HH) {                                                         \
    hipLaunchKernelGGL((gru_fwd_seq2_kernel<NK>), grid, block, 0, s, a);    \
    return;                                                                 \
  }
  FWD2_VARIANTS(X)
#undef X
  throw std::runtime_error("gru_fwd_seq2: no kernel variant for H=" + std::to_string(l0.H));
}

#define BWD_VARIANTS(X)               \
  X(256, 3, 2, 2) X(256, 3, 2, 0) X(256, 3, 0, 0) \
  X(512, 6, 4, 2) X(512, 6, 4, 0) X(512, 6, 0, 0) \
  X(1024, 12, 0, 2) X(1024, 12, 0, 0)

bool gru_bwd_seq_supported(int H, int Bp, bool fuse_w, bool fuse_p) {
  if (Bp % 32) return false;
  int cap = -1;
#define X(HH, NK, NW, NP) \
  if (H == HH && (NW > 0) == fuse_w && (NP > 0) == fuse_p) cap = resident_blocks(gru_bwd_seq_kernel<NK, NW, NP>);
  BWD_VARIANTS(X)
#undef X
  return cap >= (H / 16) * (Bp / 32);
}

void gru_bwd_seq(const SeqBwdArgs& a, hipStream_t s) {
  dim3 grid((a.H / 16) * (a.Bp / 32)), block(512);
  const bool fw = a.dWhh_part != nullptr, fp = a.dP_part != nullptr;
#define X(HH, NK, NW, NP)                                                              \
  if (a.H == HH && (NW > 0) == fw && (NP > 0) == fp) {                                \
    hipLaunchKernelGGL((gru_bwd_seq_kernel<NK, NW, NP>), grid, block, 0, s, a);       \
    return;                                                                            \
  }
  BWD_VARIANTS(X)
#undef X
  throw std::runtime_error("gru_bwd_seq: no kernel variant for H=" + std::to_string(a.H) +
                           " fuse_w=" + std::to_string(fw) + " fuse_p=" + std::to_string(fp));
}

bool gru_bwd_seq_tail_supported(int H, int Bp, int V) {
  if (H != 512 || V != 256 || Bp < 32 || Bp % 32 || Bp / 32 > 8) return false;
  const int nrb = Bp / 32;
  if (V % nrb || (V / nrb) % 8) return false;
  const int cap = resident_blocks(gru_bwd_seq_kernel<6, 4, 2, true>);
  return cap >= (H / 16) * nrb;
}

void gru_bwd_seq_tail(const SeqBwdArgs& a, const BwdTailArgs& t, hipStream_t s) {
  const int nrb = a.Bp / 32;
  if (a.H != 512 || a.V != 256 || a.Bp < 32 || a.Bp % 32 || nrb > 8 || a.V % nrb || (a.V / nrb) % 8 || !a.dWhh_part || !a.dP_part ||
      !a.s16 || !a.HF || a.dghT || a.dgiT || a.dgi || !a.ids || !a.cnt || !a.err || !t.dP_bf || !t.dPT_bf || !t.loss_part || !t.loss || !t.step || t.nloss <= 0)
    throw std::runtime_error("gru_bwd_seq_tail: needs H = 512, V = 256, at most 8 row blocks dividing V into multiples "
                             "of 8 rows, the packed saves (s16), the HF copy, no dG copies, the fused dW_hh / dP "
                             "partials and every tail buffer");
  dim3 grid((a.H / 16) * nrb), block(512);
  SeqBwdTailK k{a, t};
  hipLaunchKernelGGL((gru_bwd_seq_kernel<6, 4, 2, true>), grid, block, 0, s, k);
}

}
```

gru_mpi_cuda_amd/csrc/kernels/kernels.h:

```cpp
#pragma once
#include <vector>
#include <hip/hip_runtime.h>
#include <stdint.h>

typedef unsigned short u16;
#define DEV_HOST_INLINE __host__ __device__ __forceinline__

namespace gk {

struct FwdStepArgs {
  const u16* hprev_bf = nullptr;
  const float* hprev_f = nullptr;
  const u16* Whh = nullptr;
  const float* bhh = nullptr;
  const float* P = nullptr;
  const int* ids = nullptr;
  const float* Gi = nullptr;
  const u16* x_bf = nullptr;
  const u16* Wih = nullptr;
  const float* bih = nullptr;
  int Kin = 0;
  float* h_f = nullptr;
  u16* h_bf = nullptr;
  u16* hT = nullptr;
  int ldT = 0, colT = 0;
  float* sr = nullptr; float* sz = nullptr; float* sn = nullptr; float* sghn = nullptr;
  u16* s16 = nullptr;
  int Bp = 0, H = 0;
  int algo = 0;
};
void gru_fwd_step(const FwdStepArgs& a, hipStream_t s);

struct BwdStepArgs {
  int dgiT_n_only = 0;
  const u16* dgh_next = nullptr;
  const u16* WhhT = nullptr;
  const float* carry_in = nullptr;
  const float* dy = nullptr;
  const float *r = nullptr, *z = nullptr, *n = nullptr, *ghn = nullptr;
  const float* hprev = nullptr;
  float* carry_out = nullptr;
  u16* dgh = nullptr;
  u16* dghT = nullptr;
  u16* dgiT = nullptr;
  u16* dgi = nullptr;
  int ldT = 0, colT = 0, Bp = 0, H = 0;
  int algo = 0;
  float* sk_part = nullptr;
  long sk_part_floats = 0;
  unsigned* sk_cnt = nullptr;
  long sk_cnt_words = 0;
  int sk_map = 0;
  unsigned* err = nullptr;
};
void gru_bwd_step(const BwdStepArgs& a, hipStream_t s);
int gru_bwd_step_sk_splits(int H, int Bp);
struct StepLdsVariants {
  int fwd64 = 1;
  int bwd_sk_min_h = 1024;
  int dwfc_group = 1;
  int bwd_big = 1;
  int bwd16 = 1;
  int bwd_xring = 2;
  int fwd_xring = 4;
  int save16 = 1;
  int fc_flash = 0;
  int fwd_fc = 0;
  int fc_tail = 1;
  int bwd_tail = 1;
  int big_dy = 1;
  int ld_pad = -1;
};
StepLdsVariants& step_lds_variants();
struct GemmVariants {
  int mfma = 0;
  int phased = -1;
  int sched = -1;
  int groupm = 4;
  int onehot = 1;
  int small_ring = 4;
};
GemmVariants& gemm_variants();
bool gru_step_lds_ok(int H, int Bp);
bool gru_step_picks_lds(int algo, int H, int Bp);
void gru_fwd_step_lds(const FwdStepArgs& a, hipStream_t s);
void gru_bwd_step_lds(const BwdStepArgs& a, hipStream_t s);
enum StepKernel { kStepReg = 0, kStepLds128, kStepLds64, kStepBig, kStepLds8, kStepSk2, kStepSk4 };
struct StepPlan { int kernel = kStepReg; int ks = 0, kb = 0, nks_i = 0; int splits = 0, sk_map = 0; };
const char* step_kernel_name(int kernel);
StepPlan gru_fwd_step_plan(const FwdStepArgs& a);
StepPlan gru_bwd_step_plan(const BwdStepArgs& a);
StepPlan gru_fwd_step_lds_plan(const FwdStepArgs& a);
StepPlan gru_bwd_step_lds_plan(const BwdStepArgs& a);

struct PrepJob { const int* in = nullptr; int Bmax = 0, T = 0, Bp = 0; int* ids = nullptr; int* labels = nullptr; float* inv_count = nullptr; };
struct SeqFwdArgs {
  u16* HSb = nullptr;
  u16* xch = nullptr;
  float* HSf = nullptr;
  u16* HT = nullptr; int ldT = 0;
  u16* HF = nullptr;
  float *sr = nullptr, *sz = nullptr, *sn = nullptr, *sghn = nullptr;
  u16* s16 = nullptr;
  const u16* Whh = nullptr; const float* bhh = nullptr;
  const float* P = nullptr; const int* ids = nullptr;
  const float* Gi = nullptr;
  const float* h0 = nullptr;
  unsigned* cnt = nullptr;
  unsigned* zero_next = nullptr;
  long zero_words = 0;
  unsigned* err = nullptr;
  unsigned long long* dbg = nullptr;
  int allow_local = 1;
  int xring = 0;
  int T = 0, Bp = 0, H = 0;
};
static constexpr int kFcCons = 32;
inline long seq_flag_words(int H, int Bp) { return (long)(Bp / 32) * (H / 16 + kFcCons) * 16; }
bool gru_fwd_seq_supported(int H, int Bp);
void gru_fwd_seq(const SeqFwdArgs& a, hipStream_t s);
struct SeqFcArgs {
  const u16* Wf = nullptr;
// ... 14 lines not shown
struct FcXentArgs;
bool gru_fwd_seq_tail_supported(int H, int Bp, int V);
void gru_fwd_seq_tail(const SeqFwdArgs& a, const FcXentArgs& f, hipStream_t s);


struct SeqFwd2Args {
  SeqFwdArgs lo, hi;
  const u16* Wih = nullptr;
  const float* bih = nullptr;
};
bool gru_fwd_seq2_supported(int H, int Bp);
void gru_fwd_seq2(const SeqFwd2Args& a, hipStream_t s);

struct SeqBwdArgs {
  const float* dy = nullptr;
  const float *sr = nullptr, *sz = nullptr, *sn = nullptr, *sghn = nullptr;
  const u16* s16 = nullptr;
  const float* HSf = nullptr;
  const u16* HT = nullptr; int ldT = 0;
  const u16* HF = nullptr;
  const u16* WhhT = nullptr;
  u16* xbuf = nullptr;
  u16* dghT = nullptr; u16* dgiT = nullptr; int ldG = 0;
  u16* dgi = nullptr;
  float* dWhh_part = nullptr;
  float* dbhh_part = nullptr;
  float* dbih_part = nullptr;
  const int* ids = nullptr;
  float* dP_part = nullptr; int V = 0;
  unsigned* cnt = nullptr;
  unsigned* zero_next = nullptr;
  long zero_words = 0;
  unsigned* err = nullptr;
  unsigned long long* dbg = nullptr;
  int allow_local = 1;
  float* part = nullptr;
  int dgiT_n_only = 0;
  const u16* dl = nullptr;
  const u16* WfcT = nullptr;
  int xring = 0;
  int T = 0, Bp = 0, H = 0;
};
bool gru_bwd_seq_supported(int H, int Bp, bool fuse_w, bool fuse_p);
void gru_bwd_seq(const SeqBwdArgs& a, hipStream_t s);
struct BwdTailArgs {
  u16* dP_bf = nullptr;
  u16* dPT_bf = nullptr;
  const float* loss_part = nullptr; int nloss = 0;
  float* loss = nullptr;
  int* step = nullptr;
};
bool gru_bwd_seq_tail_supported(int H, int Bp, int V);
void gru_bwd_seq_tail(const SeqBwdArgs& a, const BwdTailArgs& t, hipStream_t s);
bool gru_bwd_seq16_supported(int H, int Bp, bool fuse_p);
void gru_bwd_seq16(const SeqBwdArgs& a, hipStream_t s);
bool gru_bwd_seq_big_supported(int H, int Bp);
long gru_bwd_seq_big_part_floats(int H, int Bp);
void gru_bwd_seq_big(const SeqBwdArgs& a, hipStream_t s);

struct FcXentArgs {
  const u16* X = nullptr;
  const u16* W = nullptr;
  const float* b = nullptr;
  const int* labels = nullptr;
  const float* inv_count = nullptr;
  u16* dl = nullptr;
  u16* dlT = nullptr;
  float* loss_part = nullptr;
  const u16* WT = nullptr;
  float* dy = nullptr;
  int M = 0, H = 0, V = 0, ldT = 0, colT = 0;
  const u16* Wf = nullptr;
  const u16* WTf = nullptr;
  unsigned long long* dbg = nullptr;
};
void fc_xent(const FcXentArgs& a, hipStream_t s);
void softmax_xent(const float* logits, const FcXentArgs& a, hipStream_t s);
bool fc_xent_fused_ok(int V, int H, int M);

struct FcSampleArgs {
  const u16* X = nullptr;
  const u16* W = nullptr;
  const u16* Wf = nullptr;
  const float* b = nullptr;
  const float* rf = nullptr;
  int* ids = nullptr;
  unsigned char* out = nullptr;
  int* alive = nullptr;
  float* probs = nullptr;
  int N = 0, Bp = 0, H = 0, V = 0, step = 0, max_len = 0, eos = 0;
};
void fc_sample(const FcSampleArgs& a, hipStream_t s);

struct GemmF32Args {
  const float* A = nullptr; int lda = 0;
  const float* B = nullptr; int ldb = 0;
  float* C = nullptr; int ldc = 0;
  const float* bias = nullptr;
  int M = 0, N = 0, K = 0;
  int splits = 1;
  long slab = 0;
};
void gemm_f32_nt(const GemmF32Args& g, hipStream_t s);
struct GruGatesF32Args {
  const float* P = nullptr; const int* ids = nullptr;
  const float* Gi = nullptr;
// ... 350 lines not shown
```

Before: 43.26 million char-tokens/s.

## Fuse persistent forward-with-FC-tail and backward-with-tail into one launch

```diff
diff --git a/gru_mpi_cuda_amd/csrc/bindings.cpp b/gru_mpi_cuda_amd/csrc/bindings.cpp
--- a/gru_mpi_cuda_amd/csrc/bindings.cpp
+++ b/gru_mpi_cuda_amd/csrc/bindings.cpp
@@ -554,7 +554,7 @@
     const StepLdsVariants& v = step_lds_variants();
     py::dict d;
     d["fwd64"] = v.fwd64; d["bwd_sk_min_h"] = v.bwd_sk_min_h; d["dwfc_group"] = v.dwfc_group;
-    d["bwd_big"] = v.bwd_big; d["bwd16"] = v.bwd16; d["bwd_xring"] = v.bwd_xring; d["fwd_xring"] = v.fwd_xring; d["fwd_fc"] = v.fwd_fc; d["fc_flash"] = v.fc_flash; d["fc_tail"] = v.fc_tail; d["bwd_tail"] = v.bwd_tail; d["save16"] = v.save16; d["big_dy"] = v.big_dy; d["ld_pad"] = v.ld_pad;
+    d["bwd_big"] = v.bwd_big; d["bwd16"] = v.bwd16; d["bwd_xring"] = v.bwd_xring; d["fwd_xring"] = v.fwd_xring; d["fwd_fc"] = v.fwd_fc; d["fc_flash"] = v.fc_flash; d["fc_tail"] = v.fc_tail; d["bwd_tail"] = v.bwd_tail; d["fb_one"] = v.fb_one; d["save16"] = v.save16; d["big_dy"] = v.big_dy; d["ld_pad"] = v.ld_pad;
     return d;
   });
   m.def("set_step_lds_variants", [](py::dict d) {
@@ -573,6 +573,7 @@
       else if (k == "fc_flash") v.fc_flash = x;
       else if (k == "fc_tail") v.fc_tail = x;
       else if (k == "bwd_tail") v.bwd_tail = x;
+      else if (k == "fb_one") v.fb_one = x;
       else if (k == "big_dy") v.big_dy = x;
       else if (k == "ld_pad") v.ld_pad = x;
       else if (k == "save16") v.save16 = x;
diff --git a/gru_mpi_cuda_amd/csrc/engine/trainer.cpp b/gru_mpi_cuda_amd/csrc/engine/trainer.cpp
--- a/gru_mpi_cuda_amd/csrc/engine/trainer.cpp
+++ b/gru_mpi_cuda_amd/csrc/engine/trainer.cpp
@@ -112,6 +112,9 @@
     }
   }
   size_t o_pP = seq_[0].fuse_p ? R((size_t)seq_[0].nrb * V * 3 * H * 4) : 0;
+  const bool fb_mem = L == 1 && persist_fwd_ && seq_[0].bwd;
+  size_t o_fbf = fb_mem ? R((size_t)4 * seq_flag_words(H, B) * 4) : 0, o_fbl = fb_mem ? R(64) : 0;
+  size_t o_xf = fb_mem ? R((size_t)T * B * H * 2) : 0;
   int sk = 0;
   bool any_big = false;
   for (int l = 0; l < L; ++l) {
@@ -135,6 +138,9 @@
     seq_[l].dbih_part = (seq_[l].bwd || seq_[l].big) ? arena_.get<float>(o_pbi[l]) : nullptr;
   }
   dP_part_ = seq_[0].fuse_p ? arena_.get<float>(o_pP) : nullptr;
+  fb_flags_ = fb_mem ? arena_.get<unsigned>(o_fbf) : nullptr;
+  fb_launches_ = fb_mem ? arena_.get<unsigned>(o_fbl) : nullptr;
+  xbuf_fwd_ = fb_mem ? arena_.get<u16>(o_xf) : nullptr;
   bpart_ = any_big ? arena_.get<float>(o_bp) : nullptr;
   sk_part_ = sk ? arena_.get<float>(o_skp) : nullptr;
   sk_cnt_ = sk ? arena_.get<unsigned>(o_skc) : nullptr;
@@ -210,6 +216,9 @@
                  seq_[0].s16 && seq_[0].HF && step_lds_variants().bwd_tail && d_.V % seq_[0].nrb == 0 &&
                  (d_.V / seq_[0].nrb) % 8 == 0 && gru_bwd_seq_tail_supported(d_.H, Bp_, d_.V);
   bwd_tail_ = bwd_tail_ok_ && use_graph_ && o_.clip <= 0.f;
+  fb_one_ok_ = fc_tail_ && bwd_tail_ok_ && fb_flags_ && d_.T >= 2 && step_lds_variants().fb_one &&
+               gru_fb_one_supported(d_.H, Bp_, d_.V);
+  fb_one_ = fb_one_ok_ && bwd_tail_;
 }
 
 Trainer::~Trainer() {
@@ -709,7 +718,7 @@
 void Trainer::set_comm(RcclComm* c, const std::vector<std::pair<long, long>>& buckets, long min_bucket_floats) {
   comm_ = c;
   if (!c) shard_opt_ = false;
-  if (c) bwd_tail_ = false;
+  if (c) bwd_tail_ = fb_one_ = false;
   buckets_ = buckets;
   min_bucket_ = std::max(1L, min_bucket_floats);
   const int L = d_.L;
diff --git a/gru_mpi_cuda_amd/csrc/engine/trainer.h b/gru_mpi_cuda_amd/csrc/engine/trainer.h
--- a/gru_mpi_cuda_amd/csrc/engine/trainer.h
+++ b/gru_mpi_cuda_amd/csrc/engine/trainer.h
@@ -38,7 +38,7 @@
   int get_step();
   void set_step(int v);
   void set_lr(float lr);
-  void set_use_graph(bool g) { use_graph_ = g; if (!g) bwd_tail_ = false; }
+  void set_use_graph(bool g) { use_graph_ = g; if (!g) bwd_tail_ = fb_one_ = false; }
   void set_carry(bool on);
   bool carry() const { return carry_; }
   void reset_hidden(hipStream_t s);
@@ -174,6 +174,9 @@
   bool fc_in_fwd_ = false;
   bool fc_tail_ = false;
   bool bwd_tail_ok_ = false, bwd_tail_ = false;
+  bool fb_one_ok_ = false, fb_one_ = false;
+  unsigned *fb_flags_ = nullptr, *fb_launches_ = nullptr;
+  u16* xbuf_fwd_ = nullptr;
   bool in_step_ = false;
   bool dy_in_bwd_ = false;
   bool fwd_wave_ = false;
diff --git a/gru_mpi_cuda_amd/csrc/engine/trainer_seq.cpp b/gru_mpi_cuda_amd/csrc/engine/trainer_seq.cpp
--- a/gru_mpi_cuda_amd/csrc/engine/trainer_seq.cpp
+++ b/gru_mpi_cuda_amd/csrc/engine/trainer_seq.cpp
@@ -141,6 +141,18 @@
   auto fc_fuse_dh = [&](FcXentArgs& f) {
     f.dl = nullptr; f.WT = WfcT; f.dy = Ls_[L - 1].dy; f.Wf = WfcF; f.WTf = WfcTF;
   };
+  const bool fb_cand = fb_one_ok_ && in_step_ && !dp && !carry_ && L == 1 && T >= 2 && step_lds_variants().fb_one;
+  bool fwd_held = false;
+  SeqFwdArgs held_a;
+  FcXentArgs held_f;
+  bool wfc_held = false;
+  GemmArgs held_w;
+  auto flush_held_fwd = [&]() {
+    if (fwd_held) gru_fwd_seq_tail(held_a, held_f, s);
+    if (wfc_held) gemm_nt(held_w, s);
+    fwd_held = wfc_held = false;
+  };
+  bool fb_one = false;
   for (int l = 0; l < L; ++l) {
     Layer& y = Ls_[l];
     if (l > 0) {
@@ -170,7 +182,8 @@
     } else if (persist_fwd_ && fc_tail_) {
       FcXentArgs f = fc_args();
       fc_fuse_dh(f);
-      gru_fwd_seq_tail(fwd_args(l), f, s);
+      if (fb_cand) { held_a = fwd_args(l); held_f = f; fwd_held = true; }
+      else gru_fwd_seq_tail(fwd_args(l), f, s);
     } else if (persist_fwd_) {
       gru_fwd_seq(fwd_args(l), s);
     } else {
@@ -225,6 +238,7 @@
     fc_held_on_ = (dp && dp_pipe_on()) ||
                   (!dp && defer_slabs_ && sp <= 8 && w.algo == 3 && step_lds_variants().dwfc_group);
     if (fc_held_on_) fc_held_ = w;
+    else if (fwd_held) { held_w = w; wfc_held = true; }
     else gemm_nt(w, s);
     tail.add(slab_fc2_, sp, (long)V * H, G("fc.weight"));
     tail.add(rs_fc2_, sp, V, G("fc.bias"));
@@ -232,6 +246,9 @@
   bool bwd_tail = bwd_tail_ok_ && !dp && defer_slabs_ && seq_[0].nrb <= kDeferMaxSplits;
   for (int k2 = 0; k2 < tail.n; ++k2) bwd_tail = bwd_tail && tail.job[k2].splits <= kDeferMaxSplits;
   if (in_step_) bwd_tail_ = bwd_tail;
+  if (!bwd_tail || !seq_[0].bwd) flush_held_fwd();
+  fb_one = fwd_held;
+  if (in_step_) fb_one_ = fb_one;
   for (int l = L - 1; l >= 0; --l) {
     Layer& y = Ls_[l];
     const SeqPlan& q = seq_[l];
@@ -255,7 +272,15 @@
       if (bwd_tail && l == 0) {
         BwdTailArgs t;
         t.dP_bf = dP_bf_; t.dPT_bf = dPT_bf_; t.loss_part = loss_part_; t.nloss = nloss_; t.loss = loss_; t.step = step_;
-        gru_bwd_seq_tail(a, t, s);
+        if (fb_one) {
+          FbOneX x;
+          x.set_words = 2 * fw; x.launches = fb_launches_;
+          held_a.cnt = fb_flags_; held_a.zero_next = nullptr; held_a.zero_words = 0; held_a.xch = xbuf_fwd_;
+          a.cnt = fb_flags_ + fw; a.zero_next = nullptr; a.zero_words = 0;
+          gru_fb_one(held_a, held_f, a, t, x, s);
+          if (wfc_held) gemm_nt(held_w, s);
+          fwd_held = wfc_held = false;
+        } else gru_bwd_seq_tail(a, t, s);
       } else if (q.rows16) gru_bwd_seq16(a, s);
       else gru_bwd_seq(a, s);
     } else if (q.big) {
@@ -486,6 +511,7 @@
   if (fc_tail_) p += " head=fwd-tail";
   p += overlap_ ? " overlap(chunks=" + std::to_string(C_) + ")" : " serial";
   if (bwd_tail_) p += " dP=bwd-tail";
+  if (fb_one_ && fc_tail_ && bwd_tail_) p += " fb=one-launch";
   return p;
 }
 
diff --git a/gru_mpi_cuda_amd/csrc/kernels/fc_block.h b/gru_mpi_cuda_amd/csrc/kernels/fc_block.h
--- a/gru_mpi_cuda_amd/csrc/kernels/fc_block.h
+++ b/gru_mpi_cuda_amd/csrc/kernels/fc_block.h
@@ -45,6 +45,7 @@
   DEV bool sc1() const { return false; }
   DEV void ready() const {}
   DEV int tid() const { return (int)threadIdx.x; }
+  DEV void store_loss(float* p, float v) const { *p = v; }
 };
 
 template <int HH, bool DH, class XP>
@@ -232,9 +233,9 @@
   if (tid == 0) {
     float t = 0.f;
     for (int i = 0; i < FROWS; ++i) t += lrow[i];
-    a.loss_part[block] = t;
-  }
-  STAMP();
-}
-
-}
+    xp.store_loss(a.loss_part + block, t);
+  }
+  STAMP();
+}
+
+}
diff --git a/gru_mpi_cuda_amd/csrc/kernels/gru_seq.hip b/gru_mpi_cuda_amd/csrc/kernels/gru_seq.hip
--- a/gru_mpi_cuda_amd/csrc/kernels/gru_seq.hip
+++ b/gru_mpi_cuda_amd/csrc/kernels/gru_seq.hip
@@ -309,6 +309,7 @@
   unsigned epoch;
   unsigned* err;
   DEV bool sc1() const { return true; }
+  DEV void store_loss(float* p, float v) const { *p = v; }
   DEV void ready() const { wait_flags_keep(fl, nunit, epoch, err); }
   DEV int tid() const {
     int t = (int)threadIdx.x;
@@ -319,7 +320,12 @@
 
 static_assert(std::is_trivially_copyable<SeqFwdArgs>::value && std::is_trivially_copyable<FcXentArgs>::value,
               "the tail reads both argument structs back from the kernel-argument segment byte for byte");
-DEV void fwd_fc_tail(bool loc, unsigned char* smem) {
+struct FcXTailOne : FcXTail {
+  DEV void store_loss(float* p, float v) const { __hip_atomic_store(p, v, __ATOMIC_RELAXED, __HIP_MEMORY_SCOPE_AGENT); }
+};
+
+template <bool ONE>
+DEV void fwd_fc_tail(bool loc, unsigned char* smem, unsigned foff) {
   typedef const __attribute__((address_space(4))) char* kptr_t;
   kptr_t kp = (kptr_t)__builtin_amdgcn_kernarg_segment_ptr();
   asm volatile("" : "+s"(kp));
@@ -327,8 +333,9 @@
   constexpr size_t fc_off = (sizeof(SeqFwdArgs) + alignof(FcXentArgs) - 1) / alignof(FcXentArgs) * alignof(FcXentArgs);
   const int T = a.T, nrb = a.Bp / 32, nunit = a.H / 16;
   const int ut = seq_unit_tile(nrb), rbk = seq_row_block(nrb);
-  unsigned* const fl = a.cnt + (size_t)rbk * nunit * kFlagStride;
-  const FcXTail xp{fl, nunit, (unsigned)(T + 1), a.err};
+  unsigned* const fl = a.cnt + (ONE ? (size_t)foff : (size_t)0) + (size_t)rbk * nunit * kFlagStride;
+  const FcXTail xb{fl, nunit, (unsigned)(T + 1), a.err};
+  const typename std::conditional<ONE, FcXTailOne, FcXTail>::type xp{xb};
   const int tid = xp.tid();
   stamp(a.dbg, T + 1, 5);
   if (tid < 64) {
@@ -359,192 +366,8 @@
                              void (*)(SeqFwdArgs, typename FwdFcArg<TAIL>::type)>::value,
                 "gru_fwd_seq_kernel takes (SeqFwdArgs, FC arguments) and nothing else");
   __shared__ __attribute__((aligned(16))) unsigned char smem[TAIL ? kFwdTailLds : FC ? (kFwdFcLds > kFwdRecLds ? kFwdFcLds : kFwdRecLds) : kFwdRecLds];
-  auto& part = *reinterpret_cast<float(*)[8][6][256]>(smem);
-  auto& stg = *reinterpret_cast<u16(*)[32][24]>(smem + sizeof(float) * 8 * 6 * 256);
-  auto& stgT = *reinterpret_cast<u16(*)[16][40]>(smem + sizeof(float) * 8 * 6 * 256 + sizeof(u16) * 32 * 24);
-  const int tid = threadIdx.x, lane = tid & 63, w = tid >> 6;
-  const int H = a.H, Bp = a.Bp, T = a.T;
-  const int nrb = Bp / 32;
-  const unsigned nunit = (unsigned)(H / 16);
-  if constexpr (FC) {
-    const int nrec = (int)nunit * nrb;
-    if ((int)blockIdx.x >= nrec) {
-      zero_next_flags(a.zero_next, a.zero_words);
-      if constexpr (NKW * 128 == 512 && RS == 2) fwd_fc_consumer<512>(a, fc, smem, (int)blockIdx.x - nrec);
-      return;
-    }
-  }
-  const size_t rb_lines = nunit + (FC ? kFcCons : 0);
-  const int ut = FC ? seq_unit_tile_n(nrb, (int)nunit * nrb) : seq_unit_tile(nrb);
-  const int j0 = ut * 16, rbk = FC ? seq_row_block_n(nrb, (int)nunit * nrb) : seq_row_block(nrb), b0 = rbk * 32;
-  const int lr = lane & 15, lk = 8 * (lane >> 4);
-  constexpr int NR = RS == 2 ? 1 : 2;
-  const int rt = RS == 2 ? (w >> 2) : 0;
-  const int k0 = (RS == 2 ? (w & 3) : w) * NKW * 32;
-
-  bf16x8 bw[NKW][3];
-#pragma unroll
-  for (int kk = 0; kk < NKW; ++kk)
-#pragma unroll
-    for (int g = 0; g < 3; ++g) bw[kk][g] = ld8(a.Whh + (size_t)(g * H + j0 + lr) * H + k0 + kk * 32 + lk);
-
-  const int rb = tid >> 8, reg = (tid >> 6) & 3, ln = tid & 63;
-  const int row = rb * 16 + (ln >> 4) * 4 + reg, col = ln & 15;
-  const int b = b0 + row, j = j0 + col;
-  float bh[3];
-#pragma unroll
-  for (int g = 0; g < 3; ++g) bh[g] = a.bhh[g * H + j];
-  float hp = a.h0 ? a.h0[(size_t)b * H + j] : 0.f;
-  const rsrc_t rH = make_rsrc(a.HSb, (unsigned)((size_t)(T + 1) * Bp * H * 2));
-  const rsrc_t rX = make_rsrc(a.xch, (unsigned)((size_t)T * Bp * H * 2));
-  const int xr = a.xring >= 2 ? a.xring : T;
-  const unsigned sv_bytes = (unsigned)((size_t)T * Bp * H * 4);
-  const rsrc_t rHSf = make_rsrc(a.HSf, sv_bytes + (unsigned)(Bp * H * 4));
-  const rsrc_t rSr = make_rsrc(a.sr, a.sr ? sv_bytes : 0u), rSz = make_rsrc(a.sz, a.sz ? sv_bytes : 0u);
-  const rsrc_t rSn = make_rsrc(a.sn, a.sn ? sv_bytes : 0u), rSg = make_rsrc(a.sghn, a.sghn ? sv_bytes : 0u);
-  const rsrc_t rS16 = make_rsrc(a.s16, a.s16 ? 2u * sv_bytes : 0u);
-  const unsigned sv_lane = (unsigned)((b * H + j) * 4);
-  stamp(a.dbg, T + 1, 0);
-  zero_next_flags(a.zero_next, a.zero_words);
-  int cens = (int)rb_lines;
-  if constexpr (FC) {
-    if ((fc.probe & 7) == 3) cens = (int)nunit;
-    if (fc.probe & 8) __builtin_amdgcn_s_setprio(2);
-  }
-  const bool loc = a.allow_local && row_block_local(a.cnt + (size_t)rbk * rb_lines * kFlagStride, ut, cens, a.err);
-  stamp(a.dbg, T + 1, 4);
-
-  int idn = a.ids ? a.ids[b] : 0;
-  auto load_gi = [&](int t, float (&gi)[3]) {
-    if (t >= T) return;
-    const float* src = a.ids ? a.P + (size_t)idn * 3 * H : a.Gi + ((size_t)t * Bp + b) * 3 * H;
-#pragma unroll
-    for (int g = 0; g < 3; ++g) gi[g] = src[g * H + j];
-    if (a.ids && t + 1 < T) idn = a.ids[(size_t)(t + 1) * Bp + b];
-  };
-  float gin[3] = {0.f, 0.f, 0.f};
-  load_gi(0, gin);
-  for (int t = 0; t < T; ++t) {
-    stamp(a.dbg, t, 0);
-    const float gi[3] = {gin[0], gin[1], gin[2]};
-    f32x4 acc[NR][3];
-    zero_acc(acc);
-    if (t > 0 || a.h0) {
-      bf16x8 af[NKW][NR];
-      if (t > 0) {
-        const size_t slot = ((size_t)((t - 1) % xr) * nrb + rbk) * nunit;
-        wave_wait_load<NKW>(a.cnt + (size_t)rbk * rb_lines * kFlagStride, lane < 2 * NKW, k0 / 16 + lane,
-                            (unsigned)t, a.err, [&](int kk) {
-          const int u = k0 + kk * 32 + lk;
-          const unsigned tb = (unsigned)(((slot + u / 16) * 32 + lr) * 16 + (u & 15)) * 2;
-#pragma unroll
-          for (int r = 0; r < NR; ++r) af[kk][r] = ld8_sc1(rX, tb + (unsigned)((rt + r) * 16 * 16 * 2));
-        });
-      } else {
-        const unsigned base = (unsigned)((((size_t)b0 + rt * 16 + lr) * H + k0 + lk) * 2);
-#pragma unroll
-        for (int kk = 0; kk < NKW; ++kk)
-#pragma unroll
-          for (int r = 0; r < NR; ++r) af[kk][r] = ld8_sc1(rH, base + (unsigned)(r * 16 * H * 2 + kk * 64));
-      }
-      stamp(a.dbg, t, 1);
-#pragma unroll
-      for (int kk = 0; kk < NKW; ++kk)
-#pragma unroll
-        for (int r = 0; r < NR; ++r)
-#pragma unroll
-          for (int g = 0; g < 3; ++g) acc[r][g] = mfma16(af[kk][r], bw[kk][g], acc[r][g]);
-    }
-#pragma unroll
-    for (int r = 0; r < NR; ++r)
-#pragma unroll
-      for (int g = 0; g < 3; ++g)
-#pragma unroll
-        for (int i = 0; i < 4; ++i) part[w][r * 3 + g][i * 64 + lane] = acc[r][g][i];
-    if constexpr (FC) {
-      if (w == 2) asm volatile("s_waitcnt vmcnt(0)" ::: "memory");
-    }
-    __syncthreads();
-    stamp(a.dbg, t, 2);
-    float gh[3];
-#pragma unroll
-    for (int g = 0; g < 3; ++g) {
-      float s = 0.f;
-      if constexpr (RS == 2) {
-#pragma unroll
-        for (int ww = 0; ww < 4; ++ww) s += part[rb * 4 + ww][g][reg * 64 + ln];
-      } else {
-#pragma unroll
-        for (int ww = 0; ww < 8; ++ww) s += part[ww][rb * 3 + g][reg * 64 + ln];
-      }
-      gh[g] = s + bh[g];
-    }
-    const float r = sigmoidf_(gi[0] + gh[0]);
-    const float z = sigmoidf_(gi[1] + gh[1]);
-    const float n = tanhf_(gi[2] + r * gh[2]);
-    const float h = n + z * (hp - n);
-    hp = h;
-    const u16 hb = f2bf(h);
-    stg[row][col] = hb;
-    stgT[col][row] = hb;
-    __syncthreads();
-    stamp(a.dbg, t, 3);
-    if (w == 0) {
-      const u32x4 v = *reinterpret_cast<const u32x4*>(&stg[lane >> 1][(lane & 1) * 8]);
-      const unsigned xo = (unsigned)((((size_t)(t % xr) * nrb + rbk) * nunit + ut) * 512 + lane * 8) * 2;
-      unsigned* fl = a.cnt + ((size_t)rbk * rb_lines + ut) * kFlagStride;
-      if (loc) {
-        st16_plain(rX, xo, v);
-        asm volatile("s_waitcnt vmcnt(0)" ::: "memory");
-        if (lane == 0) signal_flag_local(fl, (unsigned)(t + 1));
-      } else {
-        st16_sc1(rX, xo, v);
-        asm volatile("s_waitcnt vmcnt(0)" ::: "memory");
-        if (lane == 0) signal_flag(fl, (unsigned)(t + 1));
-      }
-      stamp(a.dbg, t, 4);
-      const size_t hs = ((size_t)(t + 1) * Bp + b0 + (lane >> 1)) * H + j0 + (lane & 1) * 8;
-      if (FC && !loc) st16_sc1(rH, (unsigned)(hs * 2), v);
-      else if (TAIL && !loc) {
-        unsigned* hp = reinterpret_cast<unsigned*>(a.HSb + hs);
-#pragma unroll
-        for (int i = 0; i < 4; ++i) __hip_atomic_store(hp + i, v[i], __ATOMIC_RELAXED, __HIP_MEMORY_SCOPE_AGENT);
-      } else *reinterpret_cast<u32x4*>(a.HSb + hs) = v;
-      stamp(a.dbg, t, 5);
-    } else if (w == 1 && a.HT) {
-      const u32x4 v = *reinterpret_cast<const u32x4*>(&stgT[lane >> 2][(lane & 3) * 8]);
-      *reinterpret_cast<u32x4*>(a.HT + (size_t)(j0 + (lane >> 2)) * a.ldT + (size_t)(t + 1) * Bp + b0 + (lane & 3) * 8) = v;
-    } else if (w == 2 && a.HF) {
-      const u32x4 v = *reinterpret_cast<const u32x4*>(&stgT[lane & 15][8 * (lane >> 4)]);
-      const size_t hf = (((size_t)(t + 1) * nunit + ut) * nrb + rbk) * 512 + lane * 8;
-      if (FC && !loc) st16_sc1(make_rsrc(a.HF, (unsigned)((size_t)(T + 1) * Bp * H * 2)), (unsigned)(hf * 2), v);
-      else *reinterpret_cast<u32x4*>(a.HF + hf) = v;
-    }
-    load_gi(t + 1, gin);
-    const int sstep = __builtin_amdgcn_readfirstlane(t * Bp * H * 4);
-    __builtin_amdgcn_raw_buffer_store_b32(__float_as_uint(h), rHSf, sv_lane, sstep + Bp * H * 4, 0);
-    if (TAIL || a.s16) {
-      typedef unsigned u32x2_ __attribute__((ext_vector_type(2)));
-      const u32x2_ pv = {(unsigned)f2bf(r) | ((unsigned)f2bf(z) << 16), (unsigned)f2bf(n) | ((unsigned)f2bf(gh[2]) << 16)};
-      __builtin_amdgcn_raw_buffer_store_b64(pv, rS16, sv_lane * 2u, sstep * 2, 0);
-    } else if (a.sr) {
-      __builtin_amdgcn_raw_buffer_store_b32(__float_as_uint(r), rSr, sv_lane, sstep, 0);
-      __builtin_amdgcn_raw_buffer_store_b32(__float_as_uint(z), rSz, sv_lane, sstep, 0);
-      __builtin_amdgcn_raw_buffer_store_b32(__float_as_uint(n), rSn, sv_lane, sstep, 0);
-      __builtin_amdgcn_raw_buffer_store_b32(__float_as_uint(gh[2]), rSg, sv_lane, sstep, 0);
-    }
-    stamp(a.dbg, t, 6);
-  }
-  if constexpr (FC) {
-    asm volatile("s_waitcnt vmcnt(0)" ::: "memory");
-    __syncthreads();
-    if (tid == 0) {
-      unsigned* fl = a.cnt + ((size_t)rbk * rb_lines + ut) * kFlagStride;
-      if (loc) signal_flag_local(fl, (unsigned)(T + 1));
-      else signal_flag(fl, (unsigned)(T + 1));
-    }
-  }
-  if constexpr (TAIL) fwd_fc_tail(loc, smem);
+#include "gru_seq_fwd_body.h"
+  if constexpr (TAIL) fwd_fc_tail<false>(loc, smem, 0u);
 }
 
 template <int NKW>
@@ -790,16 +613,25 @@
 struct SeqBwdTailK : SeqBwdArgs { BwdTailArgs t; };
 template <bool TAIL> struct BwdKArg { typedef SeqBwdArgs type; };
 template <> struct BwdKArg<true> { typedef SeqBwdTailK type; };
+struct FbOneArgs { SeqFwdArgs f; FcXentArgs fc; SeqBwdTailK b; FbOneX x; };
+static_assert(std::is_trivially_copyable<FbOneArgs>::value, "the phases read their arguments back byte for byte");
+constexpr size_t karg_align(size_t off, size_t al) { return (off + al - 1) / al * al; }
+static constexpr size_t kFbOneFcOff = karg_align(sizeof(SeqFwdArgs), alignof(FcXentArgs));
+static constexpr size_t kFbOneBOff = karg_align(kFbOneFcOff + sizeof(FcXentArgs), alignof(SeqBwdTailK));
+static constexpr size_t kFbOneXOff = karg_align(kFbOneBOff + sizeof(SeqBwdTailK), alignof(FbOneX));
+static_assert(sizeof(FbOneArgs) == karg_align(kFbOneXOff + sizeof(FbOneX), alignof(FbOneArgs)),
+              "members in declaration order at their natural alignment");
 
 static_assert(std::is_trivially_copyable<SeqBwdTailK>::value, "the tail reads its arguments back from the kernel-argument segment");
-template <int NTW, int NTP>
+template <int NTW, int NTP, bool ONE = false>
 DEV void bwd_dp_tail(const f32x4 (&accW)[3][NTW], const f32x4 (&accP)[3][NTP], const float (&dbh)[3], float dbi,
-                     float (*red)[16][33], unsigned char* stage ) {
+                     float (*red)[16][33], unsigned char* stage , unsigned foff = 0u) {
   typedef const __attribute__((address_space(4))) char* kptr_t;
   kptr_t kp = (kptr_t)__builtin_amdgcn_kernarg_segment_ptr();
   asm volatile("" : "+s"(kp));
-  const SeqBwdTailK& k = *(const SeqBwdTailK*)kp;
+  const SeqBwdTailK& k = *(const SeqBwdTailK*)(kp + (ONE ? kFbOneBOff : 0));
   const SeqBwdArgs& a = k;
+  unsigned* const cnt = a.cnt + (ONE ? (size_t)foff : (size_t)0);
   int tid = (int)threadIdx.x;
   asm volatile("" : "+v"(tid));
   const int lane = tid & 63, w = tid >> 6, lr = lane & 15, lq = lane >> 4;
@@ -824,7 +656,7 @@
   }
   asm volatile("s_waitcnt vmcnt(0)" ::: "memory");
   lds_barrier();
-  if (tid == 0) signal_flag(a.cnt + ((size_t)rbk * nunit + ut) * kFlagStride, (unsigned)(T + 1));
+  if (tid == 0) signal_flag(cnt + ((size_t)rbk * nunit + ut) * kFlagStride, (unsigned)(T + 1));
   stamp(a.dbg, T + 1, 1);
   if (tid < 96) {
     const int kk = tid >> 4, c = tid & 15;
@@ -848,7 +680,7 @@
     for (;;) {
       bool ok = true;
       if (lane < nrb)
-        ok = __hip_atomic_load(a.cnt + ((size_t)lane * nunit + ut) * kFlagStride, __ATOMIC_RELAXED,
+        ok = __hip_atomic_load(cnt + ((size_t)lane * nunit + ut) * kFlagStride, __ATOMIC_RELAXED,
                                __HIP_MEMORY_SCOPE_AGENT) >= (unsigned)(T + 1);
       if (__all(ok)) break;
       __builtin_amdgcn_s_sleep(GK_POLL_SLEEP);
@@ -903,10 +735,21 @@
     if (r0 + 32 < rows) lds_barrier();
   }
   if (blockIdx.x == 0 && tid < 64) {
-    const float l = wave_strided_sum(k.t.loss_part, k.t.nloss, 1, 0, lane);
+    float l;
+    if constexpr (ONE) {
+      float acc = 0.f;
+      for (int s = lane; s < k.t.nloss; s += 64)
+        acc += __hip_atomic_load(k.t.loss_part + s, __ATOMIC_RELAXED, __HIP_MEMORY_SCOPE_AGENT);
+      l = wave_sum(acc);
+    } else l = wave_strided_sum(k.t.loss_part, k.t.nloss, 1, 0, lane);
     if (tid == 0) {
       k.t.loss[0] = l;
       *k.t.step += 1;
+      if constexpr (ONE) {
+        kptr_t kx = kp + kFbOneXOff;
+        asm volatile("" : "+s"(kx));
+        *((const FbOneX*)kx)->launches += 1u;
+      }
     }
   }
   stamp(a.dbg, T + 1, 3);
@@ -921,186 +764,10 @@
   __shared__ __attribute__((aligned(16))) u16 srow[3][32][24];
   __shared__ __attribute__((aligned(16))) u16 sgT[4][16][40];
   __shared__ __attribute__((aligned(16))) float red[6][16][33];
-  constexpr bool kScalarX = NKW3 >= 12;
-  const int tid = threadIdx.x, lane = tid & 63, w = kScalarX ? __builtin_amdgcn_readfirstlane(tid >> 6) : tid >> 6;
-  const int H = a.H, H3 = 3 * a.H, Bp = a.Bp, T = a.T;
-  const int nrb = Bp / 32, ut = seq_unit_tile(nrb);
-  const int j0 = ut * 16, rbk = seq_row_block(nrb), b0 = rbk * 32;
-  const int lr = lane & 15, lk = 8 * (lane >> 4);
-  const int k0 = w * NKW3 * 32;
-  const unsigned nunit = (unsigned)(H / 16);
-
-  constexpr bool kBwLds = NTW > 0 || NTP > 0 || NKW3 >= 12;
-  __shared__ __attribute__((aligned(16))) bf16x8 bwL[kBwLds ? NKW3 : 1][kBwLds ? 512 : 1];
-  bf16x8 bw[kBwLds ? 1 : NKW3];
-#pragma unroll
-  for (int kk = 0; kk < NKW3; ++kk) {
-    const bf16x8 v = ld8(a.WhhT + (size_t)(j0 + lr) * H3 + k0 + kk * 32 + lk);
-    if constexpr (kBwLds) bwL[kk][tid] = v; else bw[kk] = v;
-  }
-
-  const int rb = tid >> 8, reg = (tid >> 6) & 3, ln = tid & 63;
-  const int row = rb * 16 + (ln >> 4) * 4 + reg, col = ln & 15;
-  const int b = b0 + row, j = j0 + col;
-  float carry = 0.f;
-  float dbh[3] = {0.f, 0.f, 0.f}, dbi = 0.f;
-  f32x4 accW[3][NTW > 0 ? NTW : 1];
-  f32x4 accP[3][NTP > 0 ? NTP : 1];
-  zero_acc(accW);
-  zero_acc(accP);
-  const int xr = a.xring >= 2 ? a.xring : T;
-  const rsrc_t rX = make_rsrc(a.xbuf, (unsigned)((size_t)T * Bp * H3 * 2));
-  const unsigned xlane = (unsigned)(((lk >> 4) * 3 * 512 + lr * 16 + (lk & 15)) * 2);
-  zero_next_flags(a.zero_next, a.zero_words);
-  const bool loc = a.allow_local && row_block_local(a.cnt + (size_t)rbk * nunit * kFlagStride, ut, (int)nunit, a.err);
-  float sv[6];
-  int svid = 0;
+  constexpr bool kBwL = NTW > 0 || NTP > 0 || NKW3 >= 12;
+  __shared__ __attribute__((aligned(16))) bf16x8 bwL[kBwL ? NKW3 : 1][kBwL ? 512 : 1];
   __shared__ __attribute__((aligned(16))) int idsL[NTP > 0 ? 32 : 1];
-  auto load_saves = [&](int t) {
-    const size_t o = ((size_t)t * Bp + b) * H + j;
-    sv[0] = a.dy[o];
-    if (TAIL || a.s16) ld_save16_raw(a.s16 + o * 4, sv[1], sv[2]);
-    else { sv[1] = a.sr[o]; sv[2] = a.sz[o]; sv[3] = a.sn[o]; sv[4] = a.sghn[o]; }
-    sv[5] = a.HSf[o];
-    if constexpr (NTP > 0) svid = a.ids[(size_t)t * Bp + b];
-  };
-  load_saves(T - 1);
-
-  for (int t = T - 1; t >= 0; --t) {
-    const int s = T - 1 - t;
-    stamp(a.dbg, s, 0);
-    f32x4 acc[2];
-    acc[0] = f32x4{0.f, 0.f, 0.f, 0.f};
-    acc[1] = acc[0];
-    if (s > 0) {
-      bf16x8 af[NKW3][2];
-      const size_t slot = ((size_t)((t + 1) % xr) * nrb + rbk) * nunit;
-      wave_wait_load<NKW3>(a.cnt + (size_t)rbk * nunit * kFlagStride, lane < 2 * NKW3,
-                           ((k0 + 16 * lane) % H) / 16, (unsigned)s, a.err, [&](int kk) {
-        if constexpr (kScalarX) {
-          const int c0 = k0 + kk * 32;
-          const int so = (int)((((slot + (size_t)((c0 % H) / 16)) * 3 + (size_t)(c0 / H)) * 512) * 2);
-#pragma unroll
-          for (int r = 0; r < 2; ++r) af[kk][r] = ld8_sc1s(rX, xlane + (unsigned)(r * 16 * 16 * 2), so);
-        } else {
-          const int c = k0 + kk * 32 + lk, u = c % H;
-          const unsigned tb = (unsigned)(((slot + u / 16) * 3 + c / H) * 512 + lr * 16 + (u & 15)) * 2;
-#pragma unroll
-          for (int r = 0; r < 2; ++r) af[kk][r] = ld8_sc1(rX, tb + (unsigned)(r * 16 * 16 * 2));
-        }
-      });
-      stamp(a.dbg, s, 1);
-#pragma unroll
-      for (int kk = 0; kk < NKW3; ++kk) {
-        bf16x8 bk;
-        if constexpr (kBwLds) bk = bwL[kk][tid]; else bk = bw[kk];
-#pragma unroll
-        for (int r = 0; r < 2; ++r) acc[r] = mfma16(af[kk][r], bk, acc[r]);
-      }
-    }
-    const int idc = svid;
-    float sr = sv[1], sz = sv[2], sn = sv[3], sghn = sv[4];
-    const float dy = sv[0], hprev = sv[5];
-    if (t > 0) load_saves(t - 1);
-    if (TAIL || a.s16) unpack_save16(sr, sz, sr, sz, sn, sghn);
-    bf16x8 hB[NTW > 0 ? NTW : 1];
-    if constexpr (NTW > 0) {
-      if (TAIL || a.HF) {
-#pragma unroll
-        for (int nt = 0; nt < NTW; ++nt)
-          hB[nt] = ld8(a.HF + (((size_t)t * nunit + w * NTW + nt) * nrb + rbk) * 512 + lane * 8);
-      } else {
-#pragma unroll
-        for (int nt = 0; nt < NTW; ++nt)
-          hB[nt] = ld8(a.HT + (size_t)(w * NTW * 16 + nt * 16 + lr) * a.ldT + (size_t)t * Bp + b0 + lk);
-      }
-    }
-#pragma unroll
-    for (int r = 0; r < 2; ++r)
-#pragma unroll
-      for (int i = 0; i < 4; ++i) part[w][r][i * 64 + lane] = acc[r][i];
-    __syncthreads();
-    stamp(a.dbg, s, 2);
-    float dh = dy + carry;
-#pragma unroll
-    for (int ww = 0; ww < 8; ++ww) dh += part[ww][rb][reg * 64 + ln];
-    const float dn = dh * (1.f - sz);
-    const float dz = dh * (hprev - sn);
-    const float dan = dn * (1.f - sn * sn);
-    const float dar = dan * sghn * sr * (1.f - sr);
-    const float daz = dz * sz * (1.f - sz);
-    const float dhn = dan * sr;
-    carry = sz * dh;
-    dbh[0] += dar; dbh[1] += daz; dbh[2] += dhn; dbi += dan;
-    const u16 br = f2bf(dar), bz = f2bf(daz), bn = f2bf(dhn), bi = f2bf(dan);
-    srow[0][row][col] = br; srow[1][row][col] = bz; srow[2][row][col] = bn;
-    sgT[0][col][row] = br; sgT[1][col][row] = bz; sgT[2][col][row] = bn; sgT[3][col][row] = bi;
-    if constexpr (NTP > 0) {
-      if (col == 0) idsL[row] = idc;
-    }
-    __syncthreads();
-    stamp(a.dbg, s, 3);
-    auto fused_mma = [&]() {
-      if constexpr (NTW > 0 || NTP > 0) {
-        bf16x8 ga[3];
-#pragma unroll
-        for (int g = 0; g < 3; ++g) ga[g] = *reinterpret_cast<const bf16x8*>(&sgT[g][lr][lk]);
-        if constexpr (NTW > 0) {
-#pragma unroll
-          for (int g = 0; g < 3; ++g)
-#pragma unroll
-            for (int nt = 0; nt < NTW; ++nt) accW[g][nt] = mfma16(ga[g], hB[nt], accW[g][nt]);
-        }
-        if constexpr (NTP > 0) {
-          ga[2] = *reinterpret_cast<const bf16x8*>(&sgT[3][lr][lk]);
-          int idv[8];
-          const int4 i0 = *reinterpret_cast<const int4*>(&idsL[lk]), i1 = *reinterpret_cast<const int4*>(&idsL[lk + 4]);
-          idv[0] = i0.x; idv[1] = i0.y; idv[2] = i0.z; idv[3] = i0.w;
-          idv[4] = i1.x; idv[5] = i1.y; idv[6] = i1.z; idv[7] = i1.w;
-#pragma unroll
-          for (int nt = 0; nt < NTP; ++nt) {
-            const int v = (w * NTP + nt) * 16 + lr;
-            bf16x8 oh;
-#pragma unroll
-            for (int e = 0; e < 8; ++e) oh[e] = (__bf16)(idv[e] == v ? 1.0f : 0.0f);
-#pragma unroll
-            for (int g = 0; g < 3; ++g) accP[g][nt] = mfma16(ga[g], oh, accP[g][nt]);
-          }
-        }
-      }
-    };
-    if (w == 0) {
-      const size_t tile = (((size_t)(t % xr) * nrb + rbk) * nunit + ut) * (3 * 32 * 16);
-#pragma unroll
-      for (int g = 0; g < 3; ++g) {
-        const u32x4 v = *reinterpret_cast<const u32x4*>(&srow[g][lane >> 1][(lane & 1) * 8]);
-        if (loc) st16_plain(rX, (unsigned)((tile + g * 512 + lane * 8) * 2), v);
-        else st16_sc1(rX, (unsigned)((tile + g * 512 + lane * 8) * 2), v);
-      }
-      asm volatile("s_waitcnt vmcnt(0)" ::: "memory");
-      unsigned* fl = a.cnt + ((size_t)rbk * nunit + ut) * kFlagStride;
-      if (lane == 0) {
-        if (loc) signal_flag_local(fl, (unsigned)(s + 1));
-        else signal_flag(fl, (unsigned)(s + 1));
-      }
-      stamp(a.dbg, s, 4);
-    } else if (!TAIL && w <= 4 && a.dghT) {
-      const int g = w - 1;
-      const u32x4 v = *reinterpret_cast<const u32x4*>(&sgT[g][lane >> 2][(lane & 3) * 8]);
-      const size_t c0 = (size_t)t * Bp + b0 + (lane & 3) * 8;
-      const int gg = g < 3 ? g : 2;
-      const size_t rowsel = (size_t)(gg * H + j0 + (lane >> 2)) * a.ldG + c0;
-      if (g < 3) *reinterpret_cast<u32x4*>(a.dghT + rowsel) = v;
-      if (g != 2) *reinterpret_cast<u32x4*>(a.dgiT + rowsel) = v;
-    }
-    if (!TAIL && a.dgi) {
-      const size_t og = ((size_t)t * Bp + b) * H3 + j;
-      a.dgi[og] = br; a.dgi[og + H] = bz; a.dgi[og + 2 * H] = bi;
-    }
-    stamp(a.dbg, s, 5);
-    fused_mma();
-    stamp(a.dbg, s, 6);
-  }
+#include "gru_seq_bwd_body.h"
 
   if constexpr (TAIL) {
     bwd_dp_tail<NTW, NTP>(accW, accP, dbh, dbi, red, reinterpret_cast<unsigned char*>(&part[0][0][0]));
@@ -1136,6 +803,93 @@
     float* dst = (k < 3 ? a.dbhh_part : a.dbih_part);
     if (dst) dst[(size_t)rbk * H3 + (k % 3) * H + j0 + c] = sum;
   }
+}
+
+struct FbOneBwdLds {
+  float part[8][2][256];
+  u16 srow[3][32][24];
+  u16 sgT[4][16][40];
+  float red[6][16][33];
+  bf16x8 bwL[6][512];
+  int idsL[32];
+};
+static constexpr size_t kFbOneLds = sizeof(FbOneBwdLds) > kFwdTailLds ? sizeof(FbOneBwdLds) : kFwdTailLds;
+
+template <int NKW, int RS, int NKW3, int NTW, int NTP, bool FC = false>
+__global__ void __launch_bounds__(512, 1) gru_fb_one_kernel(FbOneArgs k) {
+  static_assert(NKW == 4 && RS == 2 && NKW3 == 6 && NTW == 4 && NTP == 2 && !FC, "built for H = 512, V = 256");
+  static_assert(std::is_same<decltype(&gru_fb_one_kernel<NKW, RS, NKW3, NTW, NTP, FC>), void (*)(FbOneArgs)>::value,
+                "one argument struct and nothing else");
+  static_assert(kFbOneFcOff == (sizeof(SeqFwdArgs) + alignof(FcXentArgs) - 1) / alignof(FcXentArgs) * alignof(FcXentArgs),
+                "fwd_fc_tail finds the head's arguments where the two-argument forward has them");
+  __shared__ __attribute__((aligned(16))) unsigned char smem[kFbOneLds];
+  typedef const __attribute__((address_space(4))) char* kptr_t;
+  constexpr bool TAIL = true;
+  unsigned foff;
+  {
+    const unsigned par = __builtin_amdgcn_readfirstlane(__hip_atomic_load(k.x.launches, __ATOMIC_RELAXED, __HIP_MEMORY_SCOPE_AGENT)) & 1u;
+    foff = par * (unsigned)k.x.set_words;
+    zero_next_flags(k.f.cnt + (size_t)(par ^ 1u) * k.x.set_words, k.x.set_words);
+  }
+#define GK_FB_ONE 1
+  bool loc_f;
+  {
+    const SeqFwdArgs& a = k.f;
+    const typename FwdFcArg<!FC>::type& fc = k.fc;
+    (void)fc;
+#include "gru_seq_fwd_body.h"
+    loc_f = loc;
+  }
+  fwd_fc_tail<true>(loc_f, smem, foff);
+  bf16x8 wpre[NKW3];
+  {
+    kptr_t kp = (kptr_t)__builtin_amdgcn_kernarg_segment_ptr();
+    asm volatile("" : "+s"(kp));
+    const SeqFwdArgs& a = *(const SeqFwdArgs*)kp;
+    const SeqBwdArgs& b = *(const SeqBwdTailK*)(kp + kFbOneBOff);
+    int tid = (int)threadIdx.x;
+    asm volatile("" : "+v"(tid));
+    const int lane = tid & 63, w = tid >> 6, lr = lane & 15, lk = 8 * (lane >> 4);
+    const int T = a.T, nrb = a.Bp / 32, nunit = a.H / 16;
+    const int ut = seq_unit_tile(nrb), rbk = seq_row_block(nrb);
+#pragma unroll
+    for (int kk = 0; kk < NKW3; ++kk)
+      wpre[kk] = ld8(b.WhhT + (size_t)(ut * 16 + lr) * (3 * 512) + w * NKW3 * 32 + kk * 32 + lk);
+    unsigned* const fl = a.cnt + (size_t)foff + (size_t)rbk * nunit * kFlagStride;
+    stamp(a.dbg, T + 1, 7);
+    asm volatile("s_waitcnt vmcnt(0)" ::: "memory");
+    __syncthreads();
+    if (tid == 0) {
+      if (loc_f) signal_flag_local(fl + (size_t)ut * kFlagStride, (unsigned)(T + 2));
+      else {
+        __builtin_amdgcn_fence(__ATOMIC_RELEASE, "agent");
+        asm volatile("s_waitcnt vmcnt(0)" ::: "memory");
+        signal_flag(fl + (size_t)ut * kFlagStride, (unsigned)(T + 2));
+      }
+    }
+    sweep_flags(fl, nunit, (unsigned)(T + 2), a.err);
+    if (tid < 64) {
+      __builtin_amdgcn_fence(__ATOMIC_ACQUIRE, "agent");
+      asm volatile("s_waitcnt vmcnt(0)" ::: "memory");
+    }
+    __syncthreads();
+    stamp(a.dbg, T + 2, 0);
+  }
+  {
+    kptr_t kp = (kptr_t)__builtin_amdgcn_kernarg_segment_ptr();
+    asm volatile("" : "+s"(kp));
+    const SeqBwdTailK& a = *(const SeqBwdTailK*)(kp + kFbOneBOff);
+    FbOneBwdLds& L = *reinterpret_cast<FbOneBwdLds*>(smem);
+    auto& part = L.part;
+    auto& srow = L.srow;
+    auto& sgT = L.sgT;
+    auto& red = L.red;
+    auto& bwL = L.bwL;
+    auto& idsL = L.idsL;
+#include "gru_seq_bwd_body.h"
+    bwd_dp_tail<NTW, NTP, true>(accW, accP, dbh, dbi, red, reinterpret_cast<unsigned char*>(&part[0][0][0]), foff);
+  }
+#undef GK_FB_ONE
 }
 
 template <class K>
@@ -1203,13 +957,17 @@
   return cap >= (H / 16) * (Bp / 32);
 }
 
-void gru_fwd_seq_tail(const SeqFwdArgs& a, const FcXentArgs& f, hipStream_t s) {
+static void check_fwd_tail_args(const SeqFwdArgs& a, const FcXentArgs& f) {
   if (a.H != 512 || f.H != 512 || f.V != 256 || f.M != a.T * a.Bp || f.X != a.HSb + (size_t)a.Bp * a.H || !f.Wf || !f.WTf ||
       !f.dy || f.dl || !f.dlT || !f.loss_part || !f.labels || !f.inv_count || !f.b || !a.s16)
     throw std::runtime_error("gru_fwd_seq_tail: needs H = 512, V = 256, the packed saves (s16), X = HSb + Bp * H and the "
                              "fused-dH FC arguments");
   if ((size_t)(a.T + 1) * a.Bp * a.H * (a.s16 ? 8 : 4) >= (1ull << 31))
     throw std::runtime_error("gru_fwd_seq_tail: saves exceed the 2 GB buffer-offset range");
+}
+
+void gru_fwd_seq_tail(const SeqFwdArgs& a, const FcXentArgs& f, hipStream_t s) {
+  check_fwd_tail_args(a, f);
   dim3 grid((a.H / 16) * (a.Bp / 32)), block(512);
   hipLaunchKernelGGL((gru_fwd_seq_kernel<4, 2, false, 1, true>), grid, block, 0, s, a, f);
 }
@@ -1279,16 +1037,40 @@
   return cap >= (H / 16) * nrb;
 }
 
-void gru_bwd_seq_tail(const SeqBwdArgs& a, const BwdTailArgs& t, hipStream_t s) {
+static void check_bwd_tail_args(const SeqBwdArgs& a, const BwdTailArgs& t) {
   const int nrb = a.Bp / 32;
   if (a.H != 512 || a.V != 256 || a.Bp < 32 || a.Bp % 32 || nrb > 8 || a.V % nrb || (a.V / nrb) % 8 || !a.dWhh_part || !a.dP_part ||
       !a.s16 || !a.HF || a.dghT || a.dgiT || a.dgi || !a.ids || !a.cnt || !a.err || !t.dP_bf || !t.dPT_bf || !t.loss_part || !t.loss || !t.step || t.nloss <= 0)
     throw std::runtime_error("gru_bwd_seq_tail: needs H = 512, V = 256, at most 8 row blocks dividing V into multiples "
                              "of 8 rows, the packed saves (s16), the HF copy, no dG copies, the fused dW_hh / dP "
                              "partials and every tail buffer");
-  dim3 grid((a.H / 16) * nrb), block(512);
+}
+
+void gru_bwd_seq_tail(const SeqBwdArgs& a, const BwdTailArgs& t, hipStream_t s) {
+  check_bwd_tail_args(a, t);
+  dim3 grid((a.H / 16) * (a.Bp / 32)), block(512);
   SeqBwdTailK k{a, t};
   hipLaunchKernelGGL((gru_bwd_seq_kernel<6, 4, 2, true>), grid, block, 0, s, k);
 }
 
-}
+bool gru_fb_one_supported(int H, int Bp, int V) {
+  if (!gru_fwd_seq_tail_supported(H, Bp, V) || !gru_bwd_seq_tail_supported(H, Bp, V)) return false;
+  return resident_blocks(gru_fb_one_kernel<4, 2, 6, 4, 2>) >= (H / 16) * (Bp / 32);
+}
+
+void gru_fb_one(const SeqFwdArgs& a, const FcXentArgs& f, const SeqBwdArgs& b, const BwdTailArgs& t, const FbOneX& x, hipStream_t s) {
+  check_fwd_tail_args(a, f);
+  check_bwd_tail_args(b, t);
+  const long fw = (long)(a.Bp / 32) * (a.H / 16) * kFlagStride;
+  if (a.T < 2 || b.T != a.T || b.Bp != a.Bp || a.h0 || !x.launches || x.set_words < 2 * fw || b.cnt < a.cnt + fw ||
+      b.cnt + fw > a.cnt + x.set_words || (const void*)b.xbuf == (const void*)a.xch || b.dy != f.dy || b.HF != a.HF ||
+      b.HSf != a.HSf || b.s16 != a.s16 || t.loss_part != f.loss_part)
+    throw std::runtime_error("gru_fb_one: needs T >= 2, no carried state, one set of buffers for both phases, the "
+                             "backward's flag block behind the forward's inside each of the two flag sets, an "
+                             "exchange region per phase and the launch counter");
+  dim3 grid((a.H / 16) * (a.Bp / 32)), block(512);
+  FbOneArgs k{a, f, SeqBwdTailK{b, t}, x};
+  hipLaunchKernelGGL((gru_fb_one_kernel<4, 2, 6, 4, 2>), grid, block, 0, s, k);
+}
+
+}
diff --git a/gru_mpi_cuda_amd/csrc/kernels/gru_seq_bwd_body.h b/gru_mpi_cuda_amd/csrc/kernels/gru_seq_bwd_body.h
--- /dev/null
+++ b/gru_mpi_cuda_amd/csrc/kernels/gru_seq_bwd_body.h
@@ -0,0 +1,191 @@
+#ifdef GK_FB_ONE
+  unsigned* const cnt0 = a.cnt + (size_t)foff;
+#else
+  unsigned* const cnt0 = a.cnt;
+#endif
+  constexpr bool kScalarX = NKW3 >= 12;
+  const int tid = threadIdx.x, lane = tid & 63, w = kScalarX ? __builtin_amdgcn_readfirstlane(tid >> 6) : tid >> 6;
+  const int H = a.H, H3 = 3 * a.H, Bp = a.Bp, T = a.T;
+  const int nrb = Bp / 32, ut = seq_unit_tile(nrb);
+  const int j0 = ut * 16, rbk = seq_row_block(nrb), b0 = rbk * 32;
+  const int lr = lane & 15, lk = 8 * (lane >> 4);
+  const int k0 = w * NKW3 * 32;
+  const unsigned nunit = (unsigned)(H / 16);
+
+  constexpr bool kBwLds = NTW > 0 || NTP > 0 || NKW3 >= 12;
+  bf16x8 bw[kBwLds ? 1 : NKW3];
+#pragma unroll
+  for (int kk = 0; kk < NKW3; ++kk) {
+#ifdef GK_FB_ONE
+    const bf16x8 v = wpre[kk];
+#else
+    const bf16x8 v = ld8(a.WhhT + (size_t)(j0 + lr) * H3 + k0 + kk * 32 + lk);
+#endif
+    if constexpr (kBwLds) bwL[kk][tid] = v; else bw[kk] = v;
+  }
+
+  const int rb = tid >> 8, reg = (tid >> 6) & 3, ln = tid & 63;
+  const int row = rb * 16 + (ln >> 4) * 4 + reg, col = ln & 15;
+  const int b = b0 + row, j = j0 + col;
+  float carry = 0.f;
+  float dbh[3] = {0.f, 0.f, 0.f}, dbi = 0.f;
+  f32x4 accW[3][NTW > 0 ? NTW : 1];
+  f32x4 accP[3][NTP > 0 ? NTP : 1];
+  zero_acc(accW);
+  zero_acc(accP);
+  const int xr = a.xring >= 2 ? a.xring : T;
+  const rsrc_t rX = make_rsrc(a.xbuf, (unsigned)((size_t)T * Bp * H3 * 2));
+  const unsigned xlane = (unsigned)(((lk >> 4) * 3 * 512 + lr * 16 + (lk & 15)) * 2);
+#ifdef GK_FB_ONE
+  const bool loc = loc_f;
+#else
+  zero_next_flags(a.zero_next, a.zero_words);
+  const bool loc = a.allow_local && row_block_local(cnt0 + (size_t)rbk * nunit * kFlagStride, ut, (int)nunit, a.err);
+#endif
+  float sv[6];
+  int svid = 0;
+  auto load_saves = [&](int t) {
+    const size_t o = ((size_t)t * Bp + b) * H + j;
+    sv[0] = a.dy[o];
+    if (TAIL || a.s16) ld_save16_raw(a.s16 + o * 4, sv[1], sv[2]);
+    else { sv[1] = a.sr[o]; sv[2] = a.sz[o]; sv[3] = a.sn[o]; sv[4] = a.sghn[o]; }
+    sv[5] = a.HSf[o];
+    if constexpr (NTP > 0) svid = a.ids[(size_t)t * Bp + b];
+  };
+  load_saves(T - 1);
+
+  for (int t = T - 1; t >= 0; --t) {
+    const int s = T - 1 - t;
+    stamp(a.dbg, s, 0);
+    f32x4 acc[2];
+    acc[0] = f32x4{0.f, 0.f, 0.f, 0.f};
+    acc[1] = acc[0];
+    if (s > 0) {
+      bf16x8 af[NKW3][2];
+      const size_t slot = ((size_t)((t + 1) % xr) * nrb + rbk) * nunit;
+      wave_wait_load<NKW3>(cnt0 + (size_t)rbk * nunit * kFlagStride, lane < 2 * NKW3,
+                           ((k0 + 16 * lane) % H) / 16, (unsigned)s, a.err, [&](int kk) {
+        if constexpr (kScalarX) {
+          const int c0 = k0 + kk * 32;
+          const int so = (int)((((slot + (size_t)((c0 % H) / 16)) * 3 + (size_t)(c0 / H)) * 512) * 2);
+#pragma unroll
+          for (int r = 0; r < 2; ++r) af[kk][r] = ld8_sc1s(rX, xlane + (unsigned)(r * 16 * 16 * 2), so);
+        } else {
+          const int c = k0 + kk * 32 + lk, u = c % H;
+          const unsigned tb = (unsigned)(((slot + u / 16) * 3 + c / H) * 512 + lr * 16 + (u & 15)) * 2;
+#pragma unroll
+          for (int r = 0; r < 2; ++r) af[kk][r] = ld8_sc1(rX, tb + (unsigned)(r * 16 * 16 * 2));
+        }
+      });
+      stamp(a.dbg, s, 1);
+#pragma unroll
+      for (int kk = 0; kk < NKW3; ++kk) {
+        bf16x8 bk;
+        if constexpr (kBwLds) bk = bwL[kk][tid]; else bk = bw[kk];
+#pragma unroll
+        for (int r = 0; r < 2; ++r) acc[r] = mfma16(af[kk][r], bk, acc[r]);
+      }
+    }
+    const int idc = svid;
+    float sr = sv[1], sz = sv[2], sn = sv[3], sghn = sv[4];
+    const float dy = sv[0], hprev = sv[5];
+    if (t > 0) load_saves(t - 1);
+    if (TAIL || a.s16) unpack_save16(sr, sz, sr, sz, sn, sghn);
+    bf16x8 hB[NTW > 0 ? NTW : 1];
+    if constexpr (NTW > 0) {
+      if (TAIL || a.HF) {
+#pragma unroll
+        for (int nt = 0; nt < NTW; ++nt)
+          hB[nt] = ld8(a.HF + (((size_t)t * nunit + w * NTW + nt) * nrb + rbk) * 512 + lane * 8);
+      } else {
+#pragma unroll
+        for (int nt = 0; nt < NTW; ++nt)
+          hB[nt] = ld8(a.HT + (size_t)(w * NTW * 16 + nt * 16 + lr) * a.ldT + (size_t)t * Bp + b0 + lk);
+      }
+    }
+#pragma unroll
+    for (int r = 0; r < 2; ++r)
+#pragma unroll
+      for (int i = 0; i < 4; ++i) part[w][r][i * 64 + lane] = acc[r][i];
+    __syncthreads();
+    stamp(a.dbg, s, 2);
+    float dh = dy + carry;
+#pragma unroll
+    for (int ww = 0; ww < 8; ++ww) dh += part[ww][rb][reg * 64 + ln];
+    const float dn = dh * (1.f - sz);
+    const float dz = dh * (hprev - sn);
+    const float dan = dn * (1.f - sn * sn);
+    const float dar = dan * sghn * sr * (1.f - sr);
+    const float daz = dz * sz * (1.f - sz);
+    const float dhn = dan * sr;
+    carry = sz * dh;
+    dbh[0] += dar; dbh[1] += daz; dbh[2] += dhn; dbi += dan;
+    const u16 br = f2bf(dar), bz = f2bf(daz), bn = f2bf(dhn), bi = f2bf(dan);
+    srow[0][row][col] = br; srow[1][row][col] = bz; srow[2][row][col] = bn;
+    sgT[0][col][row] = br; sgT[1][col][row] = bz; sgT[2][col][row] = bn; sgT[3][col][row] = bi;
+    if constexpr (NTP > 0) {
+      if (col == 0) idsL[row] = idc;
+    }
+    __syncthreads();
+    stamp(a.dbg, s, 3);
+    auto fused_mma = [&]() {
+      if constexpr (NTW > 0 || NTP > 0) {
+        bf16x8 ga[3];
+#pragma unroll
+        for (int g = 0; g < 3; ++g) ga[g] = *reinterpret_cast<const bf16x8*>(&sgT[g][lr][lk]);
+        if constexpr (NTW > 0) {
+#pragma unroll
+          for (int g = 0; g < 3; ++g)
+#pragma unroll
+            for (int nt = 0; nt < NTW; ++nt) accW[g][nt] = mfma16(ga[g], hB[nt], accW[g][nt]);
+        }
+        if constexpr (NTP > 0) {
+          ga[2] = *reinterpret_cast<const bf16x8*>(&sgT[3][lr][lk]);
+          int idv[8];
+          const int4 i0 = *reinterpret_cast<const int4*>(&idsL[lk]), i1 = *reinterpret_cast<const int4*>(&idsL[lk + 4]);
+          idv[0] = i0.x; idv[1] = i0.y; idv[2] = i0.z; idv[3] = i0.w;
+          idv[4] = i1.x; idv[5] = i1.y; idv[6] = i1.z; idv[7] = i1.w;
+#pragma unroll
+          for (int nt = 0; nt < NTP; ++nt) {
+            const int v = (w * NTP + nt) * 16 + lr;
+            bf16x8 oh;
+#pragma unroll
+            for (int e = 0; e < 8; ++e) oh[e] = (__bf16)(idv[e] == v ? 1.0f : 0.0f);
+#pragma unroll
+            for (int g = 0; g < 3; ++g) accP[g][nt] = mfma16(ga[g], oh, accP[g][nt]);
+          }
+        }
+      }
+    };
+    if (w == 0) {
+      const size_t tile = (((size_t)(t % xr) * nrb + rbk) * nunit + ut) * (3 * 32 * 16);
+#pragma unroll
+      for (int g = 0; g < 3; ++g) {
+        const u32x4 v = *reinterpret_cast<const u32x4*>(&srow[g][lane >> 1][(lane & 1) * 8]);
+        if (loc) st16_plain(rX, (unsigned)((tile + g * 512 + lane * 8) * 2), v);
+        else st16_sc1(rX, (unsigned)((tile + g * 512 + lane * 8) * 2), v);
+      }
+      asm volatile("s_waitcnt vmcnt(0)" ::: "memory");
+      unsigned* fl = cnt0 + ((size_t)rbk * nunit + ut) * kFlagStride;
+      if (lane == 0) {
+        if (loc) signal_flag_local(fl, (unsigned)(s + 1));
+        else signal_flag(fl, (unsigned)(s + 1));
+      }
+      stamp(a.dbg, s, 4);
+    } else if (!TAIL && w <= 4 && a.dghT) {
+      const int g = w - 1;
+      const u32x4 v = *reinterpret_cast<const u32x4*>(&sgT[g][lane >> 2][(lane & 3) * 8]);
+      const size_t c0 = (size_t)t * Bp + b0 + (lane & 3) * 8;
+      const int gg = g < 3 ? g : 2;
+      const size_t rowsel = (size_t)(gg * H + j0 + (lane >> 2)) * a.ldG + c0;
+      if (g < 3) *reinterpret_cast<u32x4*>(a.dghT + rowsel) = v;
+      if (g != 2) *reinterpret_cast<u32x4*>(a.dgiT + rowsel) = v;
+    }
+    if (!TAIL && a.dgi) {
+      const size_t og = ((size_t)t * Bp + b) * H3 + j;
+      a.dgi[og] = br; a.dgi[og + H] = bz; a.dgi[og + 2 * H] = bi;
+    }
+    stamp(a.dbg, s, 5);
+    fused_mma();
+    stamp(a.dbg, s, 6);
+  }
diff --git a/gru_mpi_cuda_amd/csrc/kernels/gru_seq_fwd_body.h b/gru_mpi_cuda_amd/csrc/kernels/gru_seq_fwd_body.h
--- /dev/null
+++ b/gru_mpi_cuda_amd/csrc/kernels/gru_seq_fwd_body.h
@@ -0,0 +1,192 @@
+#ifdef GK_FB_ONE
+  unsigned* const cnt0 = a.cnt + (size_t)foff;
+#else
+  unsigned* const cnt0 = a.cnt;
+#endif
+  auto& part = *reinterpret_cast<float(*)[8][6][256]>(smem);
+  auto& stg = *reinterpret_cast<u16(*)[32][24]>(smem + sizeof(float) * 8 * 6 * 256);
+  auto& stgT = *reinterpret_cast<u16(*)[16][40]>(smem + sizeof(float) * 8 * 6 * 256 + sizeof(u16) * 32 * 24);
+  const int tid = threadIdx.x, lane = tid & 63, w = tid >> 6;
+  const int H = a.H, Bp = a.Bp, T = a.T;
+  const int nrb = Bp / 32;
+  const unsigned nunit = (unsigned)(H / 16);
+  if constexpr (FC) {
+    const int nrec = (int)nunit * nrb;
+    if ((int)blockIdx.x >= nrec) {
+      zero_next_flags(a.zero_next, a.zero_words);
+      if constexpr (NKW * 128 == 512 && RS == 2) fwd_fc_consumer<512>(a, fc, smem, (int)blockIdx.x - nrec);
+      return;
+    }
+  }
+  const size_t rb_lines = nunit + (FC ? kFcCons : 0);
+  const int ut = FC ? seq_unit_tile_n(nrb, (int)nunit * nrb) : seq_unit_tile(nrb);
+  const int j0 = ut * 16, rbk = FC ? seq_row_block_n(nrb, (int)nunit * nrb) : seq_row_block(nrb), b0 = rbk * 32;
+  const int lr = lane & 15, lk = 8 * (lane >> 4);
+  constexpr int NR = RS == 2 ? 1 : 2;
+  const int rt = RS == 2 ? (w >> 2) : 0;
+  const int k0 = (RS == 2 ? (w & 3) : w) * NKW * 32;
+
+  bf16x8 bw[NKW][3];
+#pragma unroll
+  for (int kk = 0; kk < NKW; ++kk)
+#pragma unroll
+    for (int g = 0; g < 3; ++g) bw[kk][g] = ld8(a.Whh + (size_t)(g * H + j0 + lr) * H + k0 + kk * 32 + lk);
+
+  const int rb = tid >> 8, reg = (tid >> 6) & 3, ln = tid & 63;
+  const int row = rb * 16 + (ln >> 4) * 4 + reg, col = ln & 15;
+  const int b = b0 + row, j = j0 + col;
+  float bh[3];
+#pragma unroll
+  for (int g = 0; g < 3; ++g) bh[g] = a.bhh[g * H + j];
+  float hp = a.h0 ? a.h0[(size_t)b * H + j] : 0.f;
+  const rsrc_t rH = make_rsrc(a.HSb, (unsigned)((size_t)(T + 1) * Bp * H * 2));
+  const rsrc_t rX = make_rsrc(a.xch, (unsigned)((size_t)T * Bp * H * 2));
+  const int xr = a.xring >= 2 ? a.xring : T;
+  const unsigned sv_bytes = (unsigned)((size_t)T * Bp * H * 4);
+  const rsrc_t rHSf = make_rsrc(a.HSf, sv_bytes + (unsigned)(Bp * H * 4));
+  const rsrc_t rSr = make_rsrc(a.sr, a.sr ? sv_bytes : 0u), rSz = make_rsrc(a.sz, a.sz ? sv_bytes : 0u);
+  const rsrc_t rSn = make_rsrc(a.sn, a.sn ? sv_bytes : 0u), rSg = make_rsrc(a.sghn, a.sghn ? sv_bytes : 0u);
+  const rsrc_t rS16 = make_rsrc(a.s16, a.s16 ? 2u * sv_bytes : 0u);
+  const unsigned sv_lane = (unsigned)((b * H + j) * 4);
+  stamp(a.dbg, T + 1, 0);
+#ifndef GK_FB_ONE
+  zero_next_flags(a.zero_next, a.zero_words);
+#endif
+  int cens = (int)rb_lines;
+  if constexpr (FC) {
+    if ((fc.probe & 7) == 3) cens = (int)nunit;
+    if (fc.probe & 8) __builtin_amdgcn_s_setprio(2);
+  }
+  const bool loc = a.allow_local && row_block_local(cnt0 + (size_t)rbk * rb_lines * kFlagStride, ut, cens, a.err);
+  stamp(a.dbg, T + 1, 4);
+
+  int idn = a.ids ? a.ids[b] : 0;
+  auto load_gi = [&](int t, float (&gi)[3]) {
+    if (t >= T) return;
+    const float* src = a.ids ? a.P + (size_t)idn * 3 * H : a.Gi + ((size_t)t * Bp + b) * 3 * H;
+#pragma unroll
+    for (int g = 0; g < 3; ++g) gi[g] = src[g * H + j];
+    if (a.ids && t + 1 < T) idn = a.ids[(size_t)(t + 1) * Bp + b];
+  };
+  float gin[3] = {0.f, 0.f, 0.f};
+  load_gi(0, gin);
+  for (int t = 0; t < T; ++t) {
+    stamp(a.dbg, t, 0);
+    const float gi[3] = {gin[0], gin[1], gin[2]};
+    f32x4 acc[NR][3];
+    zero_acc(acc);
+    if (t > 0 || a.h0) {
+      bf16x8 af[NKW][NR];
+      if (t > 0) {
+        const size_t slot = ((size_t)((t - 1) % xr) * nrb + rbk) * nunit;
+        wave_wait_load<NKW>(cnt0 + (size_t)rbk * rb_lines * kFlagStride, lane < 2 * NKW, k0 / 16 + lane,
+                            (unsigned)t, a.err, [&](int kk) {
+          const int u = k0 + kk * 32 + lk;
+          const unsigned tb = (unsigned)(((slot + u / 16) * 32 + lr) * 16 + (u & 15)) * 2;
+#pragma unroll
+          for (int r = 0; r < NR; ++r) af[kk][r] = ld8_sc1(rX, tb + (unsigned)((rt + r) * 16 * 16 * 2));
+        });
+      } else {
+        const unsigned base = (unsigned)((((size_t)b0 + rt * 16 + lr) * H + k0 + lk) * 2);
+#pragma unroll
+        for (int kk = 0; kk < NKW; ++kk)
+#pragma unroll
+          for (int r = 0; r < NR; ++r) af[kk][r] = ld8_sc1(rH, base + (unsigned)(r * 16 * H * 2 + kk * 64));
+      }
+      stamp(a.dbg, t, 1);
+#pragma unroll
+      for (int kk = 0; kk < NKW; ++kk)
+#pragma unroll
+        for (int r = 0; r < NR; ++r)
+#pragma unroll
+          for (int g = 0; g < 3; ++g) acc[r][g] = mfma16(af[kk][r], bw[kk][g], acc[r][g]);
+    }
+#pragma unroll
+    for (int r = 0; r < NR; ++r)
+#pragma unroll
+      for (int g = 0; g < 3; ++g)
+#pragma unroll
+        for (int i = 0; i < 4; ++i) part[w][r * 3 + g][i * 64 + lane] = acc[r][g][i];
+    if constexpr (FC) {
+      if (w == 2) asm volatile("s_waitcnt vmcnt(0)" ::: "memory");
+    }
+    __syncthreads();
+    stamp(a.dbg, t, 2);
+    float gh[3];
+#pragma unroll
+    for (int g = 0; g < 3; ++g) {
+      float s = 0.f;
+      if constexpr (RS == 2) {
+#pragma unroll
+        for (int ww = 0; ww < 4; ++ww) s += part[rb * 4 + ww][g][reg * 64 + ln];
+      } else {
+#pragma unroll
+        for (int ww = 0; ww < 8; ++ww) s += part[ww][rb * 3 + g][reg * 64 + ln];
+      }
+      gh[g] = s + bh[g];
+    }
+    const float r = sigmoidf_(gi[0] + gh[0]);
+    const float z = sigmoidf_(gi[1] + gh[1]);
+    const float n = tanhf_(gi[2] + r * gh[2]);
+    const float h = n + z * (hp - n);
+    hp = h;
+    const u16 hb = f2bf(h);
+    stg[row][col] = hb;
+    stgT[col][row] = hb;
+    __syncthreads();
+    stamp(a.dbg, t, 3);
+    if (w == 0) {
+      const u32x4 v = *reinterpret_cast<const u32x4*>(&stg[lane >> 1][(lane & 1) * 8]);
+      const unsigned xo = (unsigned)((((size_t)(t % xr) * nrb + rbk) * nunit + ut) * 512 + lane * 8) * 2;
+      unsigned* fl = cnt0 + ((size_t)rbk * rb_lines + ut) * kFlagStride;
+      if (loc) {
+        st16_plain(rX, xo, v);
+        asm volatile("s_waitcnt vmcnt(0)" ::: "memory");
+        if (lane == 0) signal_flag_local(fl, (unsigned)(t + 1));
+      } else {
+        st16_sc1(rX, xo, v);
+        asm volatile("s_waitcnt vmcnt(0)" ::: "memory");
+        if (lane == 0) signal_flag(fl, (unsigned)(t + 1));
+      }
+      stamp(a.dbg, t, 4);
+      const size_t hs = ((size_t)(t + 1) * Bp + b0 + (lane >> 1)) * H + j0 + (lane & 1) * 8;
+      if (FC && !loc) st16_sc1(rH, (unsigned)(hs * 2), v);
+      else if (TAIL && !loc) {
+        unsigned* hp = reinterpret_cast<unsigned*>(a.HSb + hs);
+#pragma unroll
+        for (int i = 0; i < 4; ++i) __hip_atomic_store(hp + i, v[i], __ATOMIC_RELAXED, __HIP_MEMORY_SCOPE_AGENT);
+      } else *reinterpret_cast<u32x4*>(a.HSb + hs) = v;
+      stamp(a.dbg, t, 5);
+    } else if (w == 1 && a.HT) {
+      const u32x4 v = *reinterpret_cast<const u32x4*>(&stgT[lane >> 2][(lane & 3) * 8]);
+      *reinterpret_cast<u32x4*>(a.HT + (size_t)(j0 + (lane >> 2)) * a.ldT + (size_t)(t + 1) * Bp + b0 + (lane & 3) * 8) = v;
+    } else if (w == 2 && a.HF) {
+      const u32x4 v = *reinterpret_cast<const u32x4*>(&stgT[lane & 15][8 * (lane >> 4)]);
+      const size_t hf = (((size_t)(t + 1) * nunit + ut) * nrb + rbk) * 512 + lane * 8;
+      if (FC && !loc) st16_sc1(make_rsrc(a.HF, (unsigned)((size_t)(T + 1) * Bp * H * 2)), (unsigned)(hf * 2), v);
+      else *reinterpret_cast<u32x4*>(a.HF + hf) = v;
+    }
+    load_gi(t + 1, gin);
+    const int sstep = __builtin_amdgcn_readfirstlane(t * Bp * H * 4);
+    __builtin_amdgcn_raw_buffer_store_b32(__float_as_uint(h), rHSf, sv_lane, sstep + Bp * H * 4, 0);
+    if (TAIL || a.s16) {
+      typedef unsigned u32x2_ __attribute__((ext_vector_type(2)));
+      const u32x2_ pv = {(unsigned)f2bf(r) | ((unsigned)f2bf(z) << 16), (unsigned)f2bf(n) | ((unsigned)f2bf(gh[2]) << 16)};
+      __builtin_amdgcn_raw_buffer_store_b64(pv, rS16, sv_lane * 2u, sstep * 2, 0);
+    } else if (a.sr) {
+      __builtin_amdgcn_raw_buffer_store_b32(__float_as_uint(r), rSr, sv_lane, sstep, 0);
+      __builtin_amdgcn_raw_buffer_store_b32(__float_as_uint(z), rSz, sv_lane, sstep, 0);
+      __builtin_amdgcn_raw_buffer_store_b32(__float_as_uint(n), rSn, sv_lane, sstep, 0);
+      __builtin_amdgcn_raw_buffer_store_b32(__float_as_uint(gh[2]), rSg, sv_lane, sstep, 0);
+    }
+    stamp(a.dbg, t, 6);
+  }
+  if constexpr (FC) {
+    asm volatile("s_waitcnt vmcnt(0)" ::: "memory");
+    __syncthreads();
+    if (tid == 0) {
+      unsigned* fl = cnt0 + ((size_t)rbk * rb_lines + ut) * kFlagStride;
+      if (loc) signal_flag_local(fl, (unsigned)(T + 1));
+      else signal_flag(fl, (unsigned)(T + 1));
+    }
+  }
diff --git a/gru_mpi_cuda_amd/csrc/kernels/kernels.h b/gru_mpi_cuda_amd/csrc/kernels/kernels.h
--- a/gru_mpi_cuda_amd/csrc/kernels/kernels.h
+++ b/gru_mpi_cuda_amd/csrc/kernels/kernels.h
@@ -68,6 +68,7 @@
   int fwd_fc = 0;
   int fc_tail = 1;
   int bwd_tail = 1;
+  int fb_one = 1;
   int big_dy = 1;
   int ld_pad = -1;
 };
@@ -188,6 +189,12 @@
 };
 bool gru_bwd_seq_tail_supported(int H, int Bp, int V);
 void gru_bwd_seq_tail(const SeqBwdArgs& a, const BwdTailArgs& t, hipStream_t s);
+struct FbOneX {
+  long set_words = 0;
+  unsigned* launches = nullptr;
+};
+bool gru_fb_one_supported(int H, int Bp, int V);
+void gru_fb_one(const SeqFwdArgs& a, const FcXentArgs& f, const SeqBwdArgs& b, const BwdTailArgs& t, const FbOneX& x, hipStream_t s);
 bool gru_bwd_seq16_supported(int H, int Bp, bool fuse_p);
 void gru_bwd_seq16(const SeqBwdArgs& a, hipStream_t s);
 bool gru_bwd_seq_big_supported(int H, int Bp);
```

Measured after the change: 43.71 million char-tokens/s (median of 6 runs). 1.01x the previous value.
